# Biblbrox/ViT-Spectre-Experiments

Measured on AMD Instinct MI355X. Metric: images/sec training, Spectre-ViT-S CIFAR-100 bs512, higher is better.
Workload: dtype bf16; 1 GPU; Spectre-ViT-Small (E512 H16 F768 L4 P4 N65, 100 classes, dropout 0.001), fft mixer, train step fwd+CE+bwd+AdamW, bs 512/GPU; mixer=fft, global_batch=512, parallelism=dp1

## Files before the change

include/spv.h:

```cpp
#ifndef SPV_H
#define SPV_H

#include <stddef.h>
#include <stdint.h>

#ifdef __cplusplus
extern "C" {
#endif

#define SPV_F32 0
#define SPV_BF16 1

#define SPV_ABI_VERSION 1

int spv_version(void);
enum {
    SPV_PATH_GEMM_STRIP = 0,
    SPV_PATH_GEMM_STRIP_ACC = 1,
    SPV_PATH_GEMM_TN = 2,
    SPV_PATH_TAIL_LC = 3,
    SPV_PATH_TAIL_UP = 4,
    SPV_PATH_TAIL_LN = 5,
    SPV_PATH_FNET_MFMA = 6,
    SPV_PATH_GATHER_LDS = 7,
// ... 60 lines not shown
    int m, n, lda, ldb, ldc;
    int k;
} spv_tn_problem;
int spv_gemm_tn_batch(const spv_tn_problem* probs, int nprob, int K, int splits, void* workspace, const spv_fold_job* folds, int nfolds,
                      void* stream);
int spv_gemm_tn_batch_part(const spv_tn_problem* probs, int nprob, int K, int splits, void* workspace, const spv_fold_job* folds,
                           int nfolds, int part, void* stream);

int spv_spectre_tail_fwd(const void* h, const void* x, const float* gamma, const float* beta, void* out,
                         float* mean, float* rstd, int rows, int n, int k_in, int dtype, int out_dtype,
                         float p_drop, uint64_t seed, void* stream);

int spv_spectre_tail_bwd(const void* dout, const void* h, const float* mean, const float* rstd,
                         const float* gamma, const float* beta, void* dh, void* dx_pool, float* dgamma,
                         float* dbeta, float* dbias, float* partials, int rows, int n, int k_in, int dtype,
                         int dout_dtype, float p_drop, uint64_t seed, const void* dx_add, void* stream);
int64_t spv_rowop_partial_floats(int n);
int spv_tail_up_supported(int n, int k_in, int dtype);
int spv_spectre_tail_bwd_up(const void* dout, const void* h, const float* mean, const float* rstd, const float* gamma,
                            const float* beta, void* dh, void* dx_pool, float* dgamma, float* dbeta, float* dbias, float* partials,
                            int rows, int n, int k_in, int dtype, int dout_dtype, float p_drop, uint64_t seed, const void* dx_add,
                            const void* up_src, float up_p_drop, uint64_t up_seed, void* stream);
int spv_tail_ln_supported(int n, int k_in, int dtype);
int64_t spv_tail_ln_partial_floats(int n);
int spv_spectre_tail_ln_fwd(const void* h, const void* x, const float* gamma, const float* beta, void* out, float* mean, float* rstd,
                            const void* res, const float* gamma2, const float* beta2, void* out2, float* mean2, float* rstd2, int rows,
                            int n, int k_in, int dtype, float p_drop, uint64_t seed, void* stream);
int spv_spectre_tail_ln_bwd(const void* dout2, const void* f3, const void* res, const float* mean2, const float* rstd2,
                            const float* gamma2, void* ds, float* dgamma2, float* dbeta2, const void* h, const float* mean,
                            const float* rstd, const float* gamma, const float* beta, void* dh, void* dx_pool, float* dgamma,
                            float* dbeta, float* dbias, float* partials, int rows, int n, int k_in, int dtype, float p_drop,
                            uint64_t seed, void* stream);

int spv_haar_ln_supported(int dim, int dtype);
int spv_haar_ln_fwd(const void* x, const float* gamma, const float* beta, void* out, float* mean, float* rstd, int rows, int dim,
                    int dtype, void* stream);
int spv_haar_ln_bwd(const void* dout, const void* x, const float* mean, const float* rstd, const float* gamma, void* dx,
                    float* dgamma, float* dbeta, float* partials, int rows, int dim, int dtype, void* stream);
int spv_add_layernorm_fwd(const void* a, const void* b, const float* gamma, const float* beta, void* out,
                          float* mean, float* rstd, int rows, int n, int mode, int dtype, void* stream);
int spv_add_layernorm_bwd(const void* dout, const void* a, const void* b, const float* mean,
                          const float* rstd, const float* gamma, void* din, float* dgamma, float* dbeta,
                          float* partials, int rows, int n, int mode, int dtype, void* stream);

int64_t spv_permut_table_words(int heads, int d);
int spv_permut_pool_supported(int heads, int d, int pool_window, int dtype);
int spv_permut_pack(const int64_t* perms, const float* signs, uint32_t* idx, int heads, int d, void* stream);
int spv_permut_gather_fwd(const void* x, const uint32_t* idx, void* g, void* pooled, int pool_window, int batch,
                          int heads, int d, int dtype, void* stream);
int spv_permut_gather_bwd(const void* dg, const uint32_t* idx, void* dx, int batch, int heads, int d,
                          int dtype, void* stream);
int spv_permut_row0_fwd(const void* x, const uint32_t* idx, void* g0, void* x0, int batch, int d, int n, int embed, int dtype,
                        void* stream);
int spv_permut_row0_bwd(const void* dg0, const void* dx0, const uint32_t* idx, void* dx, int batch, int d, int n, int embed,
                        int dtype, void* stream);


int spv_fnet_mix(const void* x, void* y, const void* add_in, const float* twiddle, int batch, int tokens, int dim,
                 int dtype, float* workspace, void* stream);
int64_t spv_fnet_workspace_floats(int batch, int tokens, int dim);
int spv_fnet_ln_supported(int tokens, int dim, int dtype);
int spv_fnet_ln_fwd(const void* x, void* prenorm, void* out, const float* gamma, const float* beta, float* mean, float* rstd,
                    const float* twiddle, int batch, int tokens, int dim, int dtype, void* stream);
int spv_fnet_ln_bwd(const void* dout, const void* prenorm, const float* mean, const float* rstd, const float* gamma, void* dx,
                    float* dgamma, float* dbeta, float* partials, const float* twiddle, int batch, int tokens, int dim, int dtype,
                    void* stream);

int spv_fnet_cls_supported(int tokens, int dim, int dtype);
int spv_fnet_cls_fwd(const void* x, const float* gamma, const float* beta, void* out, float* m0, float* mean, float* rstd, int batch,
                     int tokens, int dim, int dtype, void* stream);
int spv_fnet_cls_bwd(const void* g1, const float* m0, const float* mean, const float* rstd, const float* gamma, void* dx,
                     float* partials, int batch, int tokens, int dim, int dtype, void* stream);
int64_t spv_fnet_twiddle_floats(int tokens);
int spv_fnet_make_twiddle(float* twiddle, int tokens, void* stream);

int spv_rfft_real(const void* x, void* y, int rows, int dim, int transpose, int dtype, void* stream);

int spv_haar_dwt(const void* x, void* y, int batch, int tokens, int dim, int axis, int levels, int inverse,
                 int dtype, void* scratch, void* stream);

int spv_set_seed_device_ptr(const void* seed_word);
int spv_seed_advance(void* seed_word, void* stream);

int spv_adamw_multi(const void* table, const int* chunk_tensor, const int* chunk_off, const int* sizes, int nchunks, float lr,
                    float beta1, float beta2, float one_minus_beta1, float one_minus_beta2, float eps, float weight_decay,
                    float bias_correction1, float bias_correction2, const float* step_dev, void* stream);

int spv_adamw_multi_ema(const void* table, const int* chunk_tensor, const int* chunk_off, const int* sizes, int nchunks, float lr,
                        float beta1, float beta2, float one_minus_beta1, float one_minus_beta2, float eps, float weight_decay,
                        float bias_correction1, float bias_correction2, const float* step_dev, float* const* ema_table, float ema_weight,
                        int ema_warmup, float ema_step, void* stream);

typedef struct spv_step_ctl {
    double a, b;
    float clip_coef;
    int apply;
    float grad_norm;
    int sched_step;
    int skipped;
    int reserved[7];
} spv_step_ctl;
#define SPV_CTL_SCHEDULE 1
#define SPV_CTL_CLIP 2
#define SPV_CTL_SKIP_NONFINITE 4

int spv_grad_sumsq(const void* table, const int* chunk_tensor, const int* chunk_off, const int* sizes, int nchunks, double* partials,
                   void* stream);

int spv_step_control(const double* partials, int npartials, float* const* step_ptrs, int nsteps, spv_step_ctl* ctl, int flags,
                     int warmup_steps, int total_steps, double eta_min, float max_norm, void* stream);

int spv_adamw_multi_ctl(const void* table, const int* chunk_tensor, const int* chunk_off, const int* sizes, int nchunks, double base_lr,
                        float beta1, float beta2, float one_minus_beta1, float one_minus_beta2, float eps, float weight_decay,
                        const float* step_dev, const spv_step_ctl* ctl, void* stream);

int spv_adamw_multi_ctl_ema(const void* table, const int* chunk_tensor, const int* chunk_off, const int* sizes, int nchunks, double base_lr,
                            float beta1, float beta2, float one_minus_beta1, float one_minus_beta2, float eps, float weight_decay,
                            const float* step_dev, const spv_step_ctl* ctl, float* const* ema_table, float ema_weight, int ema_warmup,
                            void* stream);

int spv_fwht(const void* x, void* y, const void* residual, int rows, int n_in, int n, int n_out, int mode, int repeat,
             float scale, int dtype, void* stream);

int spv_patchify(const float* img, void* out, int batch, int chans, int height, int width, int patch, int ld,
                 int transposed, int out_dtype, void* stream);
int spv_patchify_u8(const unsigned char* img_hwc, const float* mean, const float* inv_std, void* out, int batch, int chans,
                    int height, int width, int patch, int ld, int transposed, int out_dtype, void* stream);
int spv_embed_posbias(const float* pos, const float* bias, const float* cls, float* out, int patches, int embed, void* stream);
int spv_embed_cls_rows(const float* cls, const float* pos, void* tokens, int batch, int tokens_per_image, int embed,
                       int dtype, void* stream);
int spv_spectral_fold(const float* proj_w, const float* freq_h, const float* freq_w, float* w_full, int embed,
                      int chans, int patch, void* stream);
int spv_spectral_fold_bf16(const float* proj_w, const float* freq_h, const float* freq_w, float* w_full, void* w_full_bf16, int embed,
                           int chans, int patch, void* stream);
int spv_spectral_fold_bwd(const float* dw_full, const float* proj_w, const float* freq_h, const float* freq_w,
                          float* dproj_w, float* dfreq_h, float* dfreq_w, float* scratch, int embed, int chans,
                          int patch, void* stream);
int spv_dropout(const void* x, void* y, int64_t n, float p, uint64_t seed, int dtype, void* stream);
int spv_embed_bwd_groups(int batch);
int spv_embed_bwd(const void* g, const void* gcls, void* dtok, float* partials, float* dpos, float* dbias, float* dcls, int batch,
                  int tokens, int embed, float p_drop, uint64_t seed, int dtype, void* stream);

int spv_attention_fwd(const void* qkv, void* ctx, void* probs, int seqs, int len, int heads, int head_dim, int dtype,
                      float p_drop, uint64_t seed, void* stream);
int spv_attention_bwd(const void* dctx, const void* qkv, const void* probs, void* dscores, void* dqkv, int seqs, int len,
                      int heads, int head_dim, int dtype, float p_drop, uint64_t seed, void* stream);
int spv_attention_row0_fwd(const void* q0, const void* k, const void* v, int ldkv, void* ctx0, float* probs, int batch, int len,
                           int heads, int head_dim, int dtype, float p_drop, uint64_t seed, void* stream);
int spv_attention_row0_bwd(const void* dctx0, const void* q0, const void* k, const void* v, int ldkv, const float* probs, void* dq0,
                           void* dk, void* dv, int ldd, int batch, int len, int heads, int head_dim, int dtype, float p_drop,
                           uint64_t seed, void* stream);

int spv_gelu_fwd(const void* x, void* y, int64_t n, int dtype, void* stream);
int spv_gelu_bwd(const void* dy, const void* x, void* dx, int64_t n, int dtype, void* stream);
int spv_colsum(const void* x, float* out, float* partials, int rows, int n, int dtype, void* stream);
int spv_axpby(const void* x, const void* y, void* out, float a, float b, int64_t n, int dtype, void* stream);

int spv_small_sl_supported(int rows, int n, int k);
int64_t spv_small_sl_partial_floats(int rows, int n);
int spv_small_sl_fwd(const void* xa, int64_t lda, const void* xb, int64_t ldb, const float* W, const float* bias,
                     const float* gamma, const float* beta, float* out, float* h, float* xs, float* mean, float* rstd,
                     int rows, int n, int k, int dtype, void* stream);
int spv_small_sl_bwd(const float* dout, const float* h, const float* xs, const float* mean, const float* rstd,
                     const float* W, const float* gamma, const float* beta, float* dh, void* dx, float* dW,
                     float* dgamma, float* dbeta, float* dbias, float* partials, int rows, int n, int k, int dx_dtype,
                     void* stream);
int64_t spv_cross_entropy_workspace_floats(void);
int spv_cross_entropy_fwd(const float* logits, const int64_t* labels, float* lse, float* loss, float* workspace, int rows,
                          int classes, void* stream);
int spv_cross_entropy_bwd(const float* logits, const int64_t* labels, const float* lse, const float* grad_out,
                          float* dlogits, int rows, int classes, void* stream);

int spv_spectrum_floats(int H, int W);
int spv_spectrum_log1p(const float* img, void* out, int B, int C, int H, int W, int dtype, void* stream);
int spv_conv3x3_fwd(const void* x, const void* w, const float* bias, void* y, void* cols, int B, int H, int W, int Cin, int Cout,
                    int dtype, void* stream);
int spv_conv3x3_dgrad(const void* dy, const void* wd, void* dx, void* cols, int B, int H, int W, int Cin, int Cout, int dtype,
                      void* stream);
int spv_conv3x3_wgrad(const void* dy, const void* x, float* dw, void* dyt, void* colst, float* workspace, int splits, int B, int H,
                      int W, int Cin, int Cout, int dtype, void* stream);
int spv_token_pool_fwd(const void* y, void* out, int B, int L, int C, int T, int ldo, int dtype, void* stream);
int spv_token_pool_bwd(const void* dout, int ldo, const void* add, void* dy, int B, int L, int C, int T, int dtype, void* stream);

#define SPV_AUG_NPARAM 16
#define SPV_AUG_FLIP 0
#define SPV_AUG_BRIGHT 1
#define SPV_AUG_CONTRAST 2
#define SPV_AUG_SAT 3
#define SPV_AUG_HUE 4
#define SPV_AUG_ORDER 5
#define SPV_AUG_GRAY 6
#define SPV_AUG_ANGLE 7
#define SPV_AUG_BLUR 8
#define SPV_AUG_SIGMA 9
#define SPV_AUG_ERASE_I 10
#define SPV_AUG_ERASE_J 11
#define SPV_AUG_ERASE_H 12
#define SPV_AUG_ERASE_W 13
typedef struct spv_augment_cfg {
    float flip_p;
    float bright_lo, bright_hi, contrast_lo, contrast_hi, sat_lo, sat_hi, hue_lo, hue_hi;
    float gray_p;
    float degrees;
    float blur_p, sigma_lo, sigma_hi;
    float erase_p, scale_lo, scale_hi, ratio_lo, ratio_hi;
} spv_augment_cfg;
int spv_augment_params(float* params, int batch, int chans, int height, int width, const spv_augment_cfg* cfg, uint64_t seed,
                       uint64_t step, void* stream);
int spv_augment_supported(int chans, int height, int width);
int spv_augment_u8(const unsigned char* src_nhwc, const int64_t* index, const float* params, const float* mean, const float* inv_std,
                   float* out_nchw, int batch, int n_src, int chans, int height, int width, void* stream);
int spv_augment_plan(int chans, int height, int width);
size_t spv_augment_tiled_ws_bytes(int batch, int height, int width);
int spv_augment_tiled_u8(const unsigned char* src_nhwc, const int64_t* index, const float* params, const float* mean,
                         const float* inv_std, float* out_nchw, int batch, int n_src, int chans, int height, int width, void* workspace,
                         size_t workspace_bytes, void* stream);

int spv_teacher_view_supported(int chans, int n, int resize, int crop);
int spv_teacher_view_u8(const unsigned char* src_nhwc, const int64_t* index, const int* table, const float* lut, void* out_nchw, int batch,
                        int n_src, int chans, int n, int resize, int crop, int dtype, void* stream);
int64_t spv_distill_loss_workspace_floats(void);
int spv_distill_loss_fwd(const float* student, const float* teacher, const int64_t* labels, float* lse3, float* out3, float* workspace,
                         int rows, int classes, float T, float w_soft, float w_ce, void* stream);
int spv_distill_loss_bwd(const float* student, const float* teacher, const int64_t* labels, const float* lse3, const float* grad_out,
                         float* dlogits, int rows, int classes, float T, float w_soft, float w_ce, void* stream);
int spv_logit_cache_store(float* cache, const int64_t* index, const float* logits, int rows, int n_cache, int classes, void* stream);
int spv_distill_loss_idx_fwd(const float* student, const float* cache, const int64_t* index, const int64_t* labels, float* lse3, float* out3,
                             float* workspace, int rows, int n_cache, int classes, float T, float w_soft, float w_ce, void* stream);
int spv_distill_loss_idx_bwd(const float* student, const float* cache, const int64_t* index, const int64_t* labels, const float* lse3,
                             const float* grad_out, float* dlogits, int rows, int n_cache, int classes, float T, float w_soft, float w_ce,
                             void* stream);

int64_t spv_eval_head_stats_words(void);
int spv_eval_head(const void* logits, const int64_t* labels, const int* n_valid, int64_t* pred, void* stats, int rows, int classes, int k,
                  int dtype, void* stream);

#define SPV_TRAIN_METER_HEADER 16
#define SPV_TRAIN_METER_ROW 5
#define SPV_TRAIN_METER_MAX_CAPACITY (1 << 24)
int64_t spv_train_meter_words(int64_t capacity);
int64_t spv_cross_entropy_meter_workspace_floats(void);
int spv_cross_entropy_meter_fwd(const float* logits, const int64_t* labels, float* lse, float* loss, float* workspace, int rows,
                                int classes, void* meter, int k, void* stream);
int64_t spv_distill_loss_meter_workspace_floats(void);
int spv_distill_loss_meter_fwd(const float* student, const float* teacher, const int64_t* labels, float* lse3, float* out3, float* workspace,
                               int rows, int classes, float T, float w_soft, float w_ce, void* meter, int k, void* stream);
int spv_distill_loss_idx_meter_fwd(const float* student, const float* cache, const int64_t* index, const int64_t* labels, float* lse3,
                                   float* out3, float* workspace, int rows, int n_cache, int classes, float T, float w_soft, float w_ce,
                                   void* meter, int k, void* stream);
// ... 6 lines not shown
```

vit-spectre-experiments_amd/csrc/spv_head.hip:

```cpp
#include "spv_common.h"

namespace {

constexpr int HR = 4;
constexpr int HT = 1024;
constexpr int HW = HT / 64;
constexpr int MAXN = 128;
constexpr int MAXK = 1024;

template <typename T> __device__ __forceinline__ float ldx(const void* p, size_t i) { return io<T>::ld(static_cast<const T*>(p) + i); }

__device__ __forceinline__ int win_start(int i, int n, int k) { return (int)(((int64_t)i * k) / n); }
__device__ __forceinline__ int win_end(int i, int n, int k) { return (int)((((int64_t)(i + 1)) * k + n - 1) / n); }

template <typename T, int KJ>
__global__ __launch_bounds__(HT) void small_sl_fwd_kernel(const void* __restrict__ xa, int64_t lda, const void* __restrict__ xb, int64_t ldb,
                                                          const float* __restrict__ W, const float* __restrict__ bias,
                                                          const float* __restrict__ gamma, const float* __restrict__ beta,
                                                          float* __restrict__ out, float* __restrict__ h, float* __restrict__ xs_out,
                                                          float* __restrict__ mean, float* __restrict__ rstd, int rows, int n, int k) {
    __shared__ float xs[HR][MAXK];
    __shared__ float hs[HR][MAXN];
    const int tid = threadIdx.x, lane = tid & 63, wave = tid >> 6;
    const int r0 = blockIdx.x * HR;
// ... 124 lines not shown
            }
        }
        const float m1 = wave_sum(s1) / (float)n, m2 = wave_sum(s2) / (float)n;
#pragma unroll
        for (int j = 0; j < 2; ++j) {
            const int o = lane + 64 * j;
            if (o < n) {
                const float v = live ? rs * (t[j] - m1 - xh[j] * m2) : 0.0f;
                dhs[wave][o] = v;
                if (!live) dos[wave][o] = 0.0f;
                part[wave][0][o] = dl[j] * xh[j];
                part[wave][1][o] = dl[j];
                part[wave][2][o] = v;
                if (live) dh[(size_t)row * n + o] = v;
            }
        }
    }
    __syncthreads();
    for (int e = tid; e < 3 * n; e += HT) {
        const int w = e / n, o = e - w * n;
        float a = 0.0f;
#pragma unroll
        for (int r = 0; r < HR; ++r) a += part[r][w][o];
        partials[((size_t)blockIdx.x * 3 + w) * n + o] = a;
    }
    const int cols = min(k, HT);
    const int nq = HT / cols;
    const int c = tid % cols, qs = tid / cols;
    constexpr int LB = 32;
    float a[HR];
#pragma unroll
    for (int r = 0; r < HR; ++r) a[r] = 0.0f;
    if (qs < nq) {
        for (int o0 = qs; o0 < n; o0 += LB * nq) {
            float w[LB];
#pragma unroll
            for (int j = 0; j < LB; ++j) {
                w[j] = W[(size_t)min(o0 + j * nq, n - 1) * k + c];
            }
#pragma unroll
            for (int j = 0; j < LB; ++j) {
                const int o = o0 + j * nq;
                const float wv = o < n ? w[j] : 0.0f;
                const int oc = min(o, n - 1);
#pragma unroll
                for (int r = 0; r < HR; ++r) a[r] = fmaf(dhs[r][oc], wv, a[r]);
            }
        }
    }
    float* join = reinterpret_cast<float*>(joinbuf);
    if (qs < nq) {
#pragma unroll
        for (int r = 0; r < HR; ++r) join[((size_t)qs * HR + r) * cols + c] = a[r];
    }
    __syncthreads();
    if (tid < cols) {
        float o4[HR];
#pragma unroll
        for (int r = 0; r < HR; ++r) {
            float t = 0.0f;
            for (int q2 = 0; q2 < nq; ++q2) t += join[((size_t)q2 * HR + r) * cols + c];
            o4[r] = t;
        }
        if (n == k) {
#pragma unroll
            for (int r = 0; r < HR; ++r) o4[r] += dos[r][c];
        } else {
            const int i0 = (int)(((int64_t)c * n) / k);
            for (int i = max(i0 - 1, 0); i <= min(i0 + 1, n - 1); ++i) {
                const int s0 = win_start(i, n, k), e0 = win_end(i, n, k);
                if (c >= s0 && c < e0) {
                    const float inv = 1.0f / (float)(e0 - s0);
#pragma unroll
                    for (int r = 0; r < HR; ++r) o4[r] = fmaf(dos[r][i], inv, o4[r]);
                }
            }
        }
#pragma unroll
        for (int r = 0; r < HR; ++r)
            if (r0 + r < rows) io<T>::st(static_cast<T*>(dx) + (size_t)(r0 + r) * k + c, o4[r]);
    }
}

constexpr int WT = 1024, WCOLS = 128, WGRP = WT / WCOLS, WOUT = 2;
__global__ __launch_bounds__(WT) void small_sl_bwd_w_kernel(const float* __restrict__ dh, const float* __restrict__ xs,
                                                            const float* __restrict__ partials, float* __restrict__ dW,
                                                            float* __restrict__ dgamma, float* __restrict__ dbeta, float* __restrict__ dbias,
                                                            int rows, int n, int k, int nparts, int cblocks) {
    __shared__ float red[WGRP][WOUT][WCOLS];
    const int tid = threadIdx.x;
    const int njobs = ((n + WOUT - 1) / WOUT) * cblocks;
    if ((int)blockIdx.x == njobs) {
        constexpr int SL = 16;
        float* fold = &red[0][0][0];
        for (int e0 = 0; e0 < 3 * n; e0 += 64) {
            const int e = e0 + (tid & 63), q = tid >> 6;
            float a = 0.0f;
            if (e < 3 * n) {
                const int w = e / n, c = e - w * n;
                for (int p0 = q; p0 < nparts; p0 += SL * 8) {
                    float v[8];
#pragma unroll
                    for (int j = 0; j < 8; ++j) {
                        const int pp = p0 + j * SL;
                        v[j] = partials[((size_t)min(pp, nparts - 1) * 3 + w) * n + c] * (pp < nparts ? 1.0f : 0.0f);
                    }
#pragma unroll
                    for (int j = 0; j < 8; ++j) a += v[j];
                }
            }
            fold[q * 64 + (tid & 63)] = a;
            __syncthreads();
            if (tid < 64 && e < 3 * n) {
                float t = 0.0f;
#pragma unroll
                for (int j = 0; j < SL; ++j) t += fold[j * 64 + tid];
                const int w = e / n, c = e - w * n;
                (w == 0 ? dgamma : (w == 1 ? dbeta : dbias))[c] = t;
            }
            __syncthreads();
        }
        return;
    }
    const int o0 = ((int)blockIdx.x / cblocks) * WOUT, c = ((int)blockIdx.x % cblocks) * WCOLS + (tid & (WCOLS - 1));
    const int g = __builtin_amdgcn_readfirstlane(tid / WCOLS);
    const int o1 = min(o0 + 1, n - 1);
    const int cc = min(c, k - 1);
    float a0 = 0.0f, a1 = 0.0f;
    constexpr int RB = 32;
    for (int rb = g; rb < rows; rb += WGRP * RB) {
        float x[RB], d0[RB], d1[RB];
#pragma unroll
        for (int j = 0; j < RB; ++j) {
            const int r = rb + j * WGRP;
            const int rr = min(r, rows - 1);
            x[j] = xs[(size_t)rr * k + cc] * (r < rows ? 1.0f : 0.0f);
            d0[j] = dh[(size_t)rr * n + o0];
            d1[j] = dh[(size_t)rr * n + o1];
        }
#pragma unroll
        for (int j = 0; j < RB; ++j) {
            a0 = fmaf(d0[j], x[j], a0);
            a1 = fmaf(d1[j], x[j], a1);
        }
    }
    red[g][0][tid & (WCOLS - 1)] = a0;
    red[g][1][tid & (WCOLS - 1)] = a1;
    __syncthreads();
    if (tid < WOUT * WCOLS) {
        const int w = tid / WCOLS, cl = tid & (WCOLS - 1);
        const int o = o0 + w, col = ((int)blockIdx.x % cblocks) * WCOLS + cl;
        float t = 0.0f;
#pragma unroll
        for (int j = 0; j < WGRP; ++j) t += red[j][w][cl];
        if (o < n && col < k) dW[(size_t)o * k + col] = t;
    }
}

constexpr int CE_MAX_WG = 64;
constexpr int CE_HITS = CE_MAX_WG + 2;

template <bool METER>
__device__ __forceinline__ void ce_fwd_body(const float* __restrict__ z, const int64_t* __restrict__ labels, float* __restrict__ lse,
                                            float* __restrict__ loss, float* __restrict__ partial, unsigned* __restrict__ counter,
                                            int rows, int C, long long* meter, int k) {
    __shared__ float ws[HT / 64];
    __shared__ int hs[METER ? HT / 64 : 1][3];
    __shared__ bool last;
    const int tid = threadIdx.x, lane = tid & 63, wave = tid >> 6;
    float acc = 0.0f;
    int seen = 0, top1 = 0, topk = 0;
    for (int r = blockIdx.x * (HT / 64) + wave; r < rows; r += gridDim.x * (HT / 64)) {
        const float* zr = z + (size_t)r * C;
        float m = -INFINITY;
        int first = 0, above = 0;
        float s = 0.0f;
        if constexpr (METER) {
            const int64_t ym = labels[r];
            const float zy = zr[(ym >= 0 && ym < C) ? (int)ym : 0];
            float bm = -INFINITY;
            int am = C;
            for (int c = lane; c < C; c += 64) {
                const float x = zr[c];
                m = fmaxf(m, x);
                if (x > bm) { bm = x; am = c; }
            }
            m = wave_max(m);
            first = (int)(-wave_max(-(float)((bm == m && am < C) ? am : C)));
            if (first >= C) first = 0;
            float cnt = 0.0f;
            for (int c = lane; c < C; c += 64) {
                const float x = zr[c];
                s += __expf(x - m);
                cnt += (x > zy || (x == zy && c < ym)) ? 1.0f : 0.0f;
            }
            above = (int)wave_sum(cnt);
        } else {
            for (int c = lane; c < C; c += 64) m = fmaxf(m, zr[c]);
            m = wave_max(m);
            for (int c = lane; c < C; c += 64) s += __expf(zr[c] - m);
        }
        const float l = m + __logf(wave_sum(s));
        const int64_t y = labels[r];
        const bool ok = y >= 0 && y < C;
        if (lane == 0) {
            lse[r] = l;
            acc += ok ? l - zr[y] : __builtin_nanf("");
            if constexpr (METER) {
                if (ok) {
                    seen += 1;
                    top1 += first == (int)y ? 1 : 0;
                    topk += above < k ? 1 : 0;
// ... 25 lines not shown
            hits[0] = a0;
            hits[1] = a1;
            hits[2] = a2;
        }
        __threadfence();
        last = atomicAdd(counter, 1u) == gridDim.x - 1;
    }
    __syncthreads();
    if (last) {
        __threadfence();
        if (wave == 0) {
            const bool in = lane < (int)gridDim.x;
            const float t = wave_sum(in ? __builtin_nontemporal_load(partial + lane) : 0.0f);
            float h0 = 0.0f, h1 = 0.0f, h2 = 0.0f;
            if constexpr (METER) {
                const int* hits = reinterpret_cast<const int*>(partial + CE_HITS) + 3 * lane;
                h0 = wave_sum(in ? (float)__builtin_nontemporal_load(hits) : 0.0f);
                h1 = wave_sum(in ? (float)__builtin_nontemporal_load(hits + 1) : 0.0f);
                h2 = wave_sum(in ? (float)__builtin_nontemporal_load(hits + 2) : 0.0f);
            }
            if (lane == 0) {
                const float mean = t / (float)rows;
                *loss = mean;
                if constexpr (METER) train_meter_log(meter, mean, 0.0f, 0.0f, (int)h0, (int)h1, (int)h2);
                *counter = 0u;
            }
        }
    }
}

__global__ __launch_bounds__(HT) void ce_fwd_kernel(const float* __restrict__ z, const int64_t* __restrict__ labels, float* __restrict__ lse,
                                                    float* __restrict__ loss, float* __restrict__ partial, unsigned* __restrict__ counter,
                                                    int rows, int C) {
    ce_fwd_body<false>(z, labels, lse, loss, partial, counter, rows, C, nullptr, 0);
}

__global__ __launch_bounds__(HT) void ce_meter_fwd_kernel(const float* __restrict__ z, const int64_t* __restrict__ labels,
                                                          float* __restrict__ lse, float* __restrict__ loss, float* __restrict__ partial,
                                                          unsigned* __restrict__ counter, int rows, int C, long long* meter, int k) {
    ce_fwd_body<true>(z, labels, lse, loss, partial, counter, rows, C, meter, k);
}

__global__ __launch_bounds__(HT) void ce_bwd_kernel(const float* __restrict__ z, const int64_t* __restrict__ labels, const float* __restrict__ lse,
                                                    const float* __restrict__ go, float* __restrict__ dz, int rows, int C) {
    const float scale = go[0] / (float)rows;
    const int64_t total = (int64_t)rows * C;
    for (int64_t e = (int64_t)blockIdx.x * HT + threadIdx.x; e < total; e += (int64_t)gridDim.x * HT) {
        const int r = (int)(e / C), c = (int)(e - (int64_t)r * C);
        const float p = __expf(z[e] - lse[r]);
        dz[e] = (p - (labels[r] == c ? 1.0f : 0.0f)) * scale;
    }
}

}

extern "C" int spv_small_sl_supported(int rows, int n, int k) {
    return (rows > 0 && rows <= 4096 && n > 0 && n <= MAXN && k > 0 && k <= MAXK && n <= k) ? 1 : 0;
}
extern "C" int64_t spv_small_sl_partial_floats(int rows, int n) { return (int64_t)cdiv(rows, HR) * 3 * n; }

extern "C" int spv_small_sl_fwd(const void* xa, int64_t lda, const void* xb, int64_t ldb, const float* W, const float* bias, const float* gamma,
                                const float* beta, float* out, float* h, float* xs, float* mean, float* rstd, int rows, int n, int k,
                                int dtype, void* stream) {
    SPV_CHECK(spv_small_sl_supported(rows, n, k), "spv_small_sl_fwd: rows=%d n=%d k=%d outside the small-rows kernel", rows, n, k);
    SPV_CHECK(dtype == SPV_F32 || dtype == SPV_BF16, "spv_small_sl_fwd: bad dtype %d", dtype);
    SPV_CHECK(lda >= k && (xb == nullptr || ldb >= k), "spv_small_sl_fwd: row strides below k");
    hipStream_t st = static_cast<hipStream_t>(stream);
    const dim3 grid(cdiv(rows, HR));
#define SPV_HEAD_FWD(TY, KJV) hipLaunchKernelGGL((small_sl_fwd_kernel<TY, KJV>), grid, dim3(HT), 0, st, xa, lda, xb, ldb, W, bias, gamma, beta, out, h, xs, mean, rstd, rows, n, k)
    if (dtype == SPV_BF16) {
        if (k <= 512) SPV_HEAD_FWD(bf16_t, 8);
        else if (k <= 768) SPV_HEAD_FWD(bf16_t, 12);
        else SPV_HEAD_FWD(bf16_t, 16);
    } else {
        if (k <= 512) SPV_HEAD_FWD(float, 8);
        else if (k <= 768) SPV_HEAD_FWD(float, 12);
        else SPV_HEAD_FWD(float, 16);
    }
#undef SPV_HEAD_FWD
    SPV_LAUNCH_CHECK("spv_small_sl_fwd");
    return 0;
}

extern "C" int spv_small_sl_bwd(const float* dout, const float* h, const float* xs, const float* mean, const float* rstd, const float* W,
                                const float* gamma, const float* beta, float* dh, void* dx, float* dW, float* dgamma, float* dbeta,
                                float* dbias, float* partials, int rows, int n, int k, int dx_dtype, void* stream) {
    SPV_CHECK(spv_small_sl_supported(rows, n, k), "spv_small_sl_bwd: rows=%d n=%d k=%d outside the small-rows kernel", rows, n, k);
    SPV_CHECK(dx_dtype == SPV_F32 || dx_dtype == SPV_BF16, "spv_small_sl_bwd: bad dtype %d", dx_dtype);
    hipStream_t st = static_cast<hipStream_t>(stream);
    const int nparts = cdiv(rows, HR);
    if (dx_dtype == SPV_BF16)
        hipLaunchKernelGGL((small_sl_bwd_rows_kernel<bf16_t>), dim3(nparts), dim3(HT), 0, st, dout, h, mean, rstd, gamma, beta, W, dh, dx, partials, rows, n, k);
    else
        hipLaunchKernelGGL((small_sl_bwd_rows_kernel<float>), dim3(nparts), dim3(HT), 0, st, dout, h, mean, rstd, gamma, beta, W, dh, dx, partials, rows, n, k);
    SPV_LAUNCH_CHECK("spv_small_sl_bwd(rows)");
    const int cblocks = cdiv(k, WCOLS);
    hipLaunchKernelGGL(small_sl_bwd_w_kernel, dim3(cdiv(n, WOUT) * cblocks + 1), dim3(WT), 0, st, dh, xs, partials, dW, dgamma, dbeta, dbias, rows,
                       n, k, nparts, cblocks);
    SPV_LAUNCH_CHECK("spv_small_sl_bwd(weights)");
    return 0;
}

extern "C" int64_t spv_cross_entropy_workspace_floats() { return CE_MAX_WG + 1; }

extern "C" int spv_cross_entropy_fwd(const float* logits, const int64_t* labels, float* lse, float* loss, float* workspace, int rows, int classes,
                                     void* stream) {
    SPV_CHECK(rows > 0 && classes > 0, "spv_cross_entropy_fwd: empty");
    hipStream_t st = static_cast<hipStream_t>(stream);
    const int wgs = std::min(cdiv(rows, HT / 64), CE_MAX_WG);
    hipLaunchKernelGGL(ce_fwd_kernel, dim3(wgs), dim3(HT), 0, st, logits, labels, lse, loss, workspace, reinterpret_cast<unsigned*>(workspace + CE_MAX_WG),
                       rows, classes);
    SPV_LAUNCH_CHECK("spv_cross_entropy_fwd");
    return 0;
}

extern "C" int64_t spv_train_meter_words(int64_t capacity) {
    if (capacity < 1 || capacity > SPV_TRAIN_METER_MAX_CAPACITY) {
        spv_set_error("spv_train_meter_words: capacity=%lld outside 1..%lld", (long long)capacity, (long long)SPV_TRAIN_METER_MAX_CAPACITY);
        return 0;
    }
    return TM_HEADER + capacity * TM_ROW;
}

int spv_train_meter_check(const char* name, const void* meter, int k, int rows, int classes) {
    SPV_CHECK(meter != nullptr, "%s: meter missing", name);
    SPV_CHECK(((uintptr_t)meter & 7) == 0, "%s: the meter block must be 8-byte aligned", name);
    SPV_CHECK(k >= 1 && k <= 8, "%s: k=%d outside 1..8", name, k);
    SPV_CHECK(rows > 0 && rows <= (1 << 24) && classes > 0 && classes < (1 << 24), "%s: rows=%d classes=%d outside 1..2^24 rows, 1..2^24-1 classes",
              name, rows, classes);
    return 0;
}

extern "C" int64_t spv_cross_entropy_meter_workspace_floats() { return CE_HITS + 3 * CE_MAX_WG; }

extern "C" int spv_cross_entropy_meter_fwd(const float* logits, const int64_t* labels, float* lse, float* loss, float* workspace, int rows,
                                           int classes, void* meter, int k, void* stream) {
    if (int rc = spv_train_meter_check("spv_cross_entropy_meter_fwd", meter, k, rows, classes)) return rc;
    SPV_CHECK(logits != nullptr && labels != nullptr && lse != nullptr && loss != nullptr && workspace != nullptr,
              "spv_cross_entropy_meter_fwd: null pointer");
    hipStream_t st = static_cast<hipStream_t>(stream);
    const int wgs = std::min(cdiv(rows, HT / 64), CE_MAX_WG);
    hipLaunchKernelGGL(ce_meter_fwd_kernel, dim3(wgs), dim3(HT), 0, st, logits, labels, lse, loss, workspace,
                       reinterpret_cast<unsigned*>(workspace + CE_MAX_WG), rows, classes, static_cast<long long*>(meter), k);
    SPV_LAUNCH_CHECK("spv_cross_entropy_meter_fwd");
    return 0;
}

extern "C" int spv_cross_entropy_bwd(const float* logits, const int64_t* labels, const float* lse, const float* grad_out, float* dlogits, int rows,
                                     int classes, void* stream) {
    SPV_CHECK(rows > 0 && classes > 0, "spv_cross_entropy_bwd: empty");
    hipStream_t st = static_cast<hipStream_t>(stream);
    const int64_t total = (int64_t)rows * classes;
    hipLaunchKernelGGL(ce_bwd_kernel, dim3((unsigned)std::min<int64_t>((total + HT - 1) / HT, 1024)), dim3(HT), 0, st, logits, labels, lse, grad_out,
                       dlogits, rows, classes);
    SPV_LAUNCH_CHECK("spv_cross_entropy_bwd");
    return 0;
}
```

vit-spectre-experiments_amd/csrc/spv_misc.hip:

```cpp
#include "spv_common.h"
#include "spv_adamw_core.h"

#include <string.h>

static thread_local char g_err[512] = "";

int spv_set_error(const char* fmt, ...) {
    va_list ap;
    va_start(ap, fmt);
    vsnprintf(g_err, sizeof(g_err), fmt, ap);
    va_end(ap);
    return 1;
}

long long g_spv_path_counts[SPV_PATH_COUNT] = {0};
extern "C" long long spv_path_count(int which) {
    return (which >= 0 && which < SPV_PATH_COUNT) ? g_spv_path_counts[which] : -1;
}

extern "C" int spv_version(void) { return SPV_ABI_VERSION; }
extern "C" const char* spv_last_error(void) { return g_err; }

namespace {

template <typename TI, typename TO>
__global__ __launch_bounds__(256) void cast_kernel(const TI* __restrict__ src, TO* __restrict__ dst, int64_t n) {
    const int64_t n4 = n >> 2;
    for (int64_t i = (int64_t)blockIdx.x * blockDim.x + threadIdx.x; i < n4; i += (int64_t)gridDim.x * blockDim.x) {
        float v[4];
        io<TI>::ld4(src + 4 * i, v);
        io<TO>::st4(dst + 4 * i, v);
    }
    if (blockIdx.x == 0 && threadIdx.x < (n & 3)) {
        int64_t i = (n4 << 2) + threadIdx.x;
        io<TO>::st(dst + i, io<TI>::ld(src + i));
    }
}

template <typename TI, typename TO>
__global__ __launch_bounds__(256) void cast_transpose_kernel(const TI* __restrict__ src, TO* __restrict__ dst, int rows,
                                                             int cols, int ld, int rg, int gs, int roff) {
    __shared__ float tile[64][65];
    const int r0 = blockIdx.y * 64, c0 = blockIdx.x * 64;
    const int tx = threadIdx.x & 63, ty = threadIdx.x >> 6;
    for (int i = ty; i < 64; i += 4) {
        int r = r0 + i, c = c0 + tx;
        float v = 0.0f;
        if (r < rows && c < cols) {
            const size_t sr = rg > 0 ? (size_t)(r / rg) * gs + roff + (r % rg) : (size_t)r;
            v = io<TI>::ld(src + sr * cols + c);
        }
        tile[i][tx] = v;
    }
    __syncthreads();
    for (int i = ty; i < 64; i += 4) {
        int c = c0 + i, r = r0 + tx;
        if (c < cols && r < ld) io<TO>::st(dst + (size_t)c * ld + r, tile[tx][i]);
    }
}

template <typename TO>
__device__ __forceinline__ void weight_shadow_tile(const float* __restrict__ src, TO* __restrict__ plain, TO* __restrict__ tr, int rows,
                                                   int cols, int ld, int bx, int by, float (*tile)[65]) {
    const int r0 = by * 32, c0 = bx * 64;
    const int t = threadIdx.x;
    const bool vec = (cols & 3) == 0;
#pragma unroll
    for (int pass = 0; pass < 2; ++pass) {
        const int rl = pass * 16 + (t >> 4), c4 = (t & 15) * 4;
        const int r = r0 + rl, c = c0 + c4;
        float v[4] = {0.0f, 0.0f, 0.0f, 0.0f};
        if (r < rows) {
            if (vec && c + 3 < cols) {
                const float4 f = *reinterpret_cast<const float4*>(src + (size_t)r * cols + c);
                v[0] = f.x; v[1] = f.y; v[2] = f.z; v[3] = f.w;
                if (plain != nullptr) io<TO>::st4(plain + (size_t)r * cols + c, v);
            } else {
                for (int u = 0; u < 4; ++u)
                    if (c + u < cols) {
                        v[u] = src[(size_t)r * cols + c + u];
                        if (plain != nullptr) io<TO>::st(plain + (size_t)r * cols + c + u, v[u]);
                    }
            }
        }
#pragma unroll
        for (int u = 0; u < 4; ++u) tile[rl][c4 + u] = v[u];
    }
    __syncthreads();
    const int cl = t >> 2, r8 = (t & 3) * 8;
    const int c = c0 + cl;
    if (c < cols) {
        TO* o = tr + (size_t)c * ld + r0 + r8;
        if (r0 + r8 + 7 < ld && (ld & 7) == 0) {
            float a[4], b[4];
#pragma unroll
            for (int u = 0; u < 4; ++u) { a[u] = tile[r8 + u][cl]; b[u] = tile[r8 + 4 + u][cl]; }
            io<TO>::st4(o, a);
            io<TO>::st4(o + 4, b);
        } else {
            for (int u = 0; u < 8; ++u)
                if (r0 + r8 + u < ld) io<TO>::st(o + u, tile[r8 + u][cl]);
        }
    }
}

template <typename TO>
__global__ __launch_bounds__(256) void weight_shadow_kernel(const float* __restrict__ src, TO* __restrict__ plain, TO* __restrict__ tr,
                                                            int rows, int cols, int ld) {
    __shared__ float tile[32][65];
    weight_shadow_tile<TO>(src, plain, tr, rows, cols, ld, blockIdx.x, blockIdx.y, tile);
}

struct ShadowTensor { const float* src; void* plain; void* tr; int rows, cols, ld, pad; };
template <typename TO>
__global__ __launch_bounds__(256) void weight_shadow_multi_kernel(const ShadowTensor* __restrict__ tab, const int* __restrict__ tile_tensor,
                                                                  const int* __restrict__ tile_x, const int* __restrict__ tile_y) {
    __shared__ float tile[32][65];
    const ShadowTensor t = tab[tile_tensor[blockIdx.x]];
    weight_shadow_tile<TO>(t.src, static_cast<TO*>(t.plain), static_cast<TO*>(t.tr), t.rows, t.cols, t.ld, tile_x[blockIdx.x],
                           tile_y[blockIdx.x], tile);
}

template <typename T>
__global__ __launch_bounds__(256) void gelu_fwd_kernel(const T* __restrict__ x, T* __restrict__ y, int64_t n) {
    for (int64_t i = (int64_t)blockIdx.x * blockDim.x + threadIdx.x; i < n; i += (int64_t)gridDim.x * blockDim.x)
        io<T>::st(y + i, gelu_erf(io<T>::ld(x + i)));
}
template <typename T>
__global__ __launch_bounds__(256) void gelu_bwd_kernel(const T* __restrict__ dy, const T* __restrict__ x,
                                                       T* __restrict__ dx, int64_t n) {
    for (int64_t i = (int64_t)blockIdx.x * blockDim.x + threadIdx.x; i < n; i += (int64_t)gridDim.x * blockDim.x)
        io<T>::st(dx + i, io<T>::ld(dy + i) * gelu_erf_grad(io<T>::ld(x + i)));
}
template <typename T>
__global__ __launch_bounds__(256) void axpby_kernel(const T* __restrict__ x, const T* __restrict__ y, T* __restrict__ out,
                                                    float a, float b, int64_t n) {
    for (int64_t i = (int64_t)blockIdx.x * blockDim.x + threadIdx.x; i < n; i += (int64_t)gridDim.x * blockDim.x)
        io<T>::st(out + i, a * io<T>::ld(x + i) + b * io<T>::ld(y + i));
}

template <typename T, int VEC>
__global__ __launch_bounds__(256) void colsum_partial_kernel(const T* __restrict__ x, float* __restrict__ partials, int rows,
                                                             int n, int tx_log2) {
    __shared__ float red[256 * VEC];
    const int TX = 1 << tx_log2, TY = 256 >> tx_log2;
    const int tx = threadIdx.x & (TX - 1), ty = threadIdx.x >> tx_log2;
    const int c0 = (blockIdx.x * TX + tx) * VEC;
    float s[VEC];
#pragma unroll
    for (int k = 0; k < VEC; ++k) s[k] = 0.0f;
    if (c0 < n) {
        const int step = gridDim.y * TY;
        for (int r = blockIdx.y * TY + ty; r < rows; r += step) {
            if constexpr (VEC == 4) {
                float v[4];
                io<T>::ld4(x + (size_t)r * n + c0, v);
#pragma unroll
                for (int k = 0; k < 4; ++k) s[k] += v[k];
            } else {
                s[0] += io<T>::ld(x + (size_t)r * n + c0);
            }
        }
    }
#pragma unroll
    for (int k = 0; k < VEC; ++k) red[(ty * TX + tx) * VEC + k] = s[k];
    __syncthreads();
    if (ty == 0 && c0 < n) {
#pragma unroll
        for (int k = 0; k < VEC; ++k) {
            float t = s[k];
            for (int q = 1; q < TY; ++q) t += red[(q * TX + tx) * VEC + k];
            if (c0 + k < n) partials[(size_t)blockIdx.y * n + c0 + k] = t;
        }
    }
}
__global__ __launch_bounds__(256) void colsum_fold_kernel(const float* __restrict__ partials, float* __restrict__ out, int parts,
                                                          int n) {
    __shared__ float red[8][33];
    const int cx = threadIdx.x & 31, py = threadIdx.x >> 5;
    const int c = blockIdx.x * 32 + cx;
    float s = 0.0f;
    if (c < n)
        for (int p = py; p < parts; p += 8) s += partials[(size_t)p * n + c];
    red[py][cx] = s;
    __syncthreads();
    if (py == 0 && c < n) {
        float t = 0.0f;
#pragma unroll
        for (int q = 0; q < 8; ++q) t += red[q][cx];
        out[c] = t;
    }
}

inline int ew_blocks(int64_t n) { return (int)std::min<int64_t>((n + 255) / 256, 2048); }

}
// ... 68 lines not shown
    else
        return spv_set_error("spv_weight_shadows: bad dtype %d", dtype);
    SPV_LAUNCH_CHECK("spv_weight_shadows");
    return 0;
}

#define DISPATCH_T(dtype, name, ...)                                        \
    if (dtype == SPV_F32) { using T = float; __VA_ARGS__; }                 \
    else if (dtype == SPV_BF16) { using T = bf16_t; __VA_ARGS__; }          \
    else return spv_set_error("%s: bad dtype %d", name, dtype);

extern "C" int spv_gelu_fwd(const void* x, void* y, int64_t n, int dtype, void* stream) {
    if (n <= 0) return 0;
    hipStream_t st = static_cast<hipStream_t>(stream);
    DISPATCH_T(dtype, "spv_gelu_fwd",
               hipLaunchKernelGGL((gelu_fwd_kernel<T>), dim3(ew_blocks(n)), dim3(256), 0, st, (const T*)x, (T*)y, n));
    SPV_LAUNCH_CHECK("spv_gelu_fwd");
    return 0;
}
extern "C" int spv_gelu_bwd(const void* dy, const void* x, void* dx, int64_t n, int dtype, void* stream) {
    if (n <= 0) return 0;
    hipStream_t st = static_cast<hipStream_t>(stream);
    DISPATCH_T(dtype, "spv_gelu_bwd",
               hipLaunchKernelGGL((gelu_bwd_kernel<T>), dim3(ew_blocks(n)), dim3(256), 0, st, (const T*)dy, (const T*)x, (T*)dx, n));
    SPV_LAUNCH_CHECK("spv_gelu_bwd");
    return 0;
}
extern "C" int spv_axpby(const void* x, const void* y, void* out, float a, float b, int64_t n, int dtype, void* stream) {
    if (n <= 0) return 0;
    hipStream_t st = static_cast<hipStream_t>(stream);
    DISPATCH_T(dtype, "spv_axpby",
               hipLaunchKernelGGL((axpby_kernel<T>), dim3(ew_blocks(n)), dim3(256), 0, st, (const T*)x, (const T*)y, (T*)out, a, b, n));
    SPV_LAUNCH_CHECK("spv_axpby");
    return 0;
}

extern "C" int spv_colsum(const void* x, float* out, float* partials, int rows, int n, int dtype, void* stream) {
    SPV_CHECK(rows > 0 && n > 0, "spv_colsum: empty");
    hipStream_t st = static_cast<hipStream_t>(stream);
    const int vec = (n % 4 == 0 && ((uintptr_t)x & 15) == 0) ? 4 : 1;
    const int cthreads = cdiv(n, vec);
    int tx_log2 = 5;
    while (tx_log2 < 8 && (1 << tx_log2) < cthreads) ++tx_log2;
    const int ty = 256 >> tx_log2;
    const int gx = cdiv(cthreads, 1 << tx_log2);
    const int parts = std::max(1, std::min(std::min(cdiv(rows, ty), 512), std::max(1, 1024 / gx)));
    if (vec == 4) {
        DISPATCH_T(dtype, "spv_colsum",
                   hipLaunchKernelGGL((colsum_partial_kernel<T, 4>), dim3(gx, parts), dim3(256), 0, st, (const T*)x, partials, rows, n, tx_log2));
    } else {
        DISPATCH_T(dtype, "spv_colsum",
                   hipLaunchKernelGGL((colsum_partial_kernel<T, 1>), dim3(gx, parts), dim3(256), 0, st, (const T*)x, partials, rows, n, tx_log2));
    }
    SPV_LAUNCH_CHECK("spv_colsum");
    hipLaunchKernelGGL(colsum_fold_kernel, dim3(cdiv(n, 32)), dim3(256), 0, st, partials, out, parts, n);
    SPV_LAUNCH_CHECK("spv_colsum(fold)");
    return 0;
}

namespace {
__global__ __launch_bounds__(256) void adamw_multi_kernel(const AdamTensor* __restrict__ tab, const int* __restrict__ chunk_tensor,
                                                          const int* __restrict__ chunk_off, const int* __restrict__ sizes, float lr,
                                                          float beta1, float beta2, float omb1, float omb2, float eps, float wd,
                                                          float bc1, float bc2, const float* __restrict__ step_dev) {
    const int t = chunk_tensor[blockIdx.x];
    const int off = chunk_off[blockIdx.x];
    const AdamTensor a = tab[t];
    const int n = sizes[t];
    adamw_chunk<false>(a, n, off, lr, beta1, beta2, omb1, omb2, eps, wd, bc1, bc2, step_dev, 1.0f);
}

__global__ __launch_bounds__(256) void adamw_multi_ema_kernel(const AdamTensor* __restrict__ tab, const int* __restrict__ chunk_tensor,
                                                              const int* __restrict__ chunk_off, const int* __restrict__ sizes, float lr,
                                                              float beta1, float beta2, float omb1, float omb2, float eps, float wd,
                                                              float bc1, float bc2, const float* __restrict__ step_dev,
                                                              float* const* __restrict__ ema_tab, float ema_w, int ema_warmup, float ema_step) {
    const int t = chunk_tensor[blockIdx.x];
    const int off = chunk_off[blockIdx.x];
    const AdamTensor a = tab[t];
    const int n = sizes[t];
    adamw_chunk<false, true>(a, n, off, lr, beta1, beta2, omb1, omb2, eps, wd, bc1, bc2, step_dev, 1.0f, ema_tab[t], ema_w, ema_warmup,
                             ema_step);
}
}

extern "C" int spv_adamw_multi(const void* table, const int* chunk_tensor, const int* chunk_off, const int* sizes, int nchunks, float lr,
                               float beta1, float beta2, float one_minus_beta1, float one_minus_beta2, float eps, float weight_decay,
                               float bias_correction1, float bias_correction2, const float* step_dev, void* stream) {
    SPV_CHECK(nchunks >= 0, "spv_adamw_multi: nchunks = %d", nchunks);
    if (nchunks == 0) return 0;
    SPV_CHECK(table && chunk_tensor && chunk_off && sizes, "spv_adamw_multi: null table");
    SPV_CHECK(step_dev != nullptr || (bias_correction1 > 0.0f && bias_correction2 > 0.0f), "spv_adamw_multi: bias corrections must be > 0");
    hipLaunchKernelGGL(adamw_multi_kernel, dim3(nchunks), dim3(256), 0, static_cast<hipStream_t>(stream),
                       static_cast<const AdamTensor*>(table), chunk_tensor, chunk_off, sizes, lr, beta1, beta2, one_minus_beta1,
                       one_minus_beta2, eps, weight_decay, bias_correction1, bias_correction2, step_dev);
    SPV_LAUNCH_CHECK("spv_adamw_multi");
    return 0;
}

extern "C" int spv_adamw_multi_ema(const void* table, const int* chunk_tensor, const int* chunk_off, const int* sizes, int nchunks, float lr,
                                   float beta1, float beta2, float one_minus_beta1, float one_minus_beta2, float eps, float weight_decay,
                                   float bias_correction1, float bias_correction2, const float* step_dev, float* const* ema_table,
                                   float ema_weight, int ema_warmup, float ema_step, void* stream) {
    SPV_CHECK(nchunks >= 0, "spv_adamw_multi_ema: nchunks = %d", nchunks);
    SPV_CHECK(table && chunk_tensor && chunk_off && sizes, "spv_adamw_multi_ema: null table");
    SPV_CHECK(ema_table, "spv_adamw_multi_ema: null ema_table (use spv_adamw_multi for a group that is not averaged)");
    SPV_CHECK(step_dev != nullptr || (bias_correction1 > 0.0f && bias_correction2 > 0.0f), "spv_adamw_multi_ema: bias corrections must be > 0");
    SPV_CHECK(ema_weight > 0.0f && ema_weight <= 1.0f, "spv_adamw_multi_ema: ema_weight = %g must be in (0, 1]", (double)ema_weight);
    SPV_CHECK(!ema_warmup || step_dev != nullptr || ema_step >= 1.0f, "spv_adamw_multi_ema: ema_step = %g must be >= 1 (the step count of this step)",
              (double)ema_step);
    if (nchunks == 0) return 0;
    hipLaunchKernelGGL(adamw_multi_ema_kernel, dim3(nchunks), dim3(256), 0, static_cast<hipStream_t>(stream),
                       static_cast<const AdamTensor*>(table), chunk_tensor, chunk_off, sizes, lr, beta1, beta2, one_minus_beta1,
                       one_minus_beta2, eps, weight_decay, bias_correction1, bias_correction2, step_dev, ema_table, ema_weight, ema_warmup,
                       ema_step);
    SPV_LAUNCH_CHECK("spv_adamw_multi_ema");
    return 0;
}

int spv_seed_ptr_set_rowops(const unsigned long long* p);
int spv_seed_ptr_set_patch(const unsigned long long* p);
int spv_seed_ptr_set_attn(const unsigned long long* p);
int spv_seed_ptr_set_gemm(const unsigned long long* p);
namespace {
__global__ void seed_advance_kernel(unsigned long long* p) { *p += 0x9e3779b97f4a7c15ull; }
}
extern "C" int spv_set_seed_device_ptr(const void* seed_word) {
    const unsigned long long* p = static_cast<const unsigned long long*>(seed_word);
    SPV_CHECK(spv_seed_ptr_set_rowops(p) == 0 && spv_seed_ptr_set_patch(p) == 0 && spv_seed_ptr_set_attn(p) == 0 && spv_seed_ptr_set_gemm(p) == 0,
              "spv_set_seed_device_ptr: hipMemcpyToSymbol failed");
    return 0;
}
extern "C" int spv_seed_advance(void* seed_word, void* stream) {
    SPV_CHECK(seed_word != nullptr, "spv_seed_advance: null pointer");
    hipLaunchKernelGGL(seed_advance_kernel, dim3(1), dim3(1), 0, static_cast<hipStream_t>(stream), static_cast<unsigned long long*>(seed_word));
    SPV_LAUNCH_CHECK("spv_seed_advance");
    return 0;
}
```

vit-spectre-experiments_amd/csrc/spv_patch.hip:

```cpp
#define SPV_USES_SEED
#include "spv_common.h"

namespace {

__device__ __forceinline__ void st_any(void* base, size_t off, int bf, float v) {
    if (bf) static_cast<bf16_t*>(base)[off] = f2bf(v);
    else static_cast<float*>(base)[off] = v;
}
__device__ __forceinline__ float ld_any(const void* base, size_t off, int bf) {
    return bf ? bf2f(static_cast<const bf16_t*>(base)[off]) : static_cast<const float*>(base)[off];
}

__global__ __launch_bounds__(256) void patchify_kernel(const float* __restrict__ img, void* __restrict__ out, int B, int C, int H,
                                                       int W, int P, int ld, int transposed, int bf) {
    const int nH = H / P, nW = W / P, Np = nH * nW, K = C * P * P;
    const int64_t rows = (int64_t)B * Np;
    const int64_t total = transposed == 1 ? (int64_t)K * ld : (transposed == 2 ? (int64_t)B * (Np + 1) * ld : rows * ld);
    for (int64_t e = (int64_t)blockIdx.x * blockDim.x + threadIdx.x; e < total; e += (int64_t)gridDim.x * blockDim.x) {
        int64_t row;
        int k;
        if (transposed == 1) { k = (int)(e / ld); row = e % ld; }
        else { row = e / ld; k = (int)(e % ld); }
        if (transposed == 2) {
            const int64_t b2 = row / (Np + 1);
            const int t2 = (int)(row % (Np + 1));
            row = t2 == 0 ? rows : b2 * Np + t2 - 1;
        }
        float v = 0.0f;
        if (row < rows && k < K) {
            const int b = (int)(row / Np), n = (int)(row % Np);
            const int ih = n / nW, iw = n % nW;
            const int c = k / (P * P), p = (k / P) % P, q = k % P;
            v = img[(((size_t)b * C + c) * H + ih * P + p) * W + iw * P + q];
        }
        st_any(out, (size_t)e, bf, v);
    }
}

template <typename T>
__global__ __launch_bounds__(256) void patchify_vec4_kernel(const float* __restrict__ img, T* __restrict__ out, int B, int C, int H, int W,
                                                            int P, int ld, int token_rows) {
    const int nH = H / P, nW = W / P, Np = nH * nW, K = C * P * P;
    const int T1 = token_rows ? Np + 1 : Np;
    const int ld4 = ld >> 2, P4 = P >> 2;
    const int64_t total = (int64_t)B * T1 * ld4;
    for (int64_t e = (int64_t)blockIdx.x * blockDim.x + threadIdx.x; e < total; e += (int64_t)gridDim.x * blockDim.x) {
        const int64_t row = e / ld4;
        const int k = (int)(e - row * ld4) * 4;
        const int b = (int)(row / T1), t = (int)(row - (int64_t)b * T1);
        const int n = token_rows ? t - 1 : t;
        float v[4] = {0.0f, 0.0f, 0.0f, 0.0f};
        if (n >= 0 && k < K) {
            const int ih = n / nW, iw = n - ih * nW;
            const int c = k / (P * P), r = k - c * P * P, pr = r / P, q = r - pr * P;
            const float4 px = *reinterpret_cast<const float4*>(img + (((size_t)b * C + c) * H + ih * P + pr) * W + iw * P + q);
            v[0] = px.x; v[1] = px.y; v[2] = px.z; v[3] = px.w;
        }
        (void)P4;
        io<T>::st4(out + (size_t)row * ld + k, v);
    }
}

__global__ __launch_bounds__(256) void patchify_u8_kernel(const unsigned char* __restrict__ img, const float* __restrict__ mean,
                                                          const float* __restrict__ inv_std, void* __restrict__ out, int B, int C,
                                                          int H, int W, int P, int ld, int transposed, int bf) {
    const int nH = H / P, nW = W / P, Np = nH * nW, K = C * P * P;
    const int64_t rows = (int64_t)B * Np;
    const int64_t total = transposed == 1 ? (int64_t)K * ld : (transposed == 2 ? (int64_t)B * (Np + 1) * ld : rows * ld);
    for (int64_t e = (int64_t)blockIdx.x * blockDim.x + threadIdx.x; e < total; e += (int64_t)gridDim.x * blockDim.x) {
        int64_t row;
        int k;
        if (transposed == 1) { k = (int)(e / ld); row = e % ld; }
        else { row = e / ld; k = (int)(e % ld); }
        if (transposed == 2) {
            const int64_t b2 = row / (Np + 1);
            const int t2 = (int)(row % (Np + 1));
            row = t2 == 0 ? rows : b2 * Np + t2 - 1;
        }
        float v = 0.0f;
        if (row < rows && k < K) {
            const int b = (int)(row / Np), n = (int)(row % Np);
            const int ih = n / nW, iw = n % nW;
            const int c = k / (P * P), p = (k / P) % P, q = k % P;
            const float px = (float)img[(((size_t)b * H + ih * P + p) * W + iw * P + q) * C + c];
            v = (px * (1.0f / 255.0f) - mean[c]) * inv_std[c];
        }
        st_any(out, (size_t)e, bf, v);
    }
}

__global__ __launch_bounds__(256) void posbias_kernel(const float* __restrict__ pos, const float* __restrict__ bias,
                                                      const float* __restrict__ cls, float* __restrict__ out, int Np, int E) {
    const int lead = cls != nullptr ? E : 0;
    const int total = Np * E + lead;
    for (int i = blockIdx.x * blockDim.x + threadIdx.x; i < total; i += gridDim.x * blockDim.x)
        out[i] = i < lead ? cls[i] + pos[i] : pos[E + i - lead] + bias[(i - lead) % E];
}

__global__ __launch_bounds__(256) void cls_rows_kernel(const float* __restrict__ cls, const float* __restrict__ pos,
                                                       void* __restrict__ tokens, int B, int T, int E, int bf) {
    const int total = B * E;
    for (int i = blockIdx.x * blockDim.x + threadIdx.x; i < total; i += gridDim.x * blockDim.x) {
        const int b = i / E, e = i % E;
        st_any(tokens, ((size_t)b * T) * E + e, bf, cls[e] + pos[e]);
    }
}

__global__ __launch_bounds__(256) void dropout_kernel(const void* __restrict__ x, void* __restrict__ y, int64_t n, float p,
                                                      uint64_t seed, int bf) {
    const float inv_keep = 1.0f / (1.0f - p);
    const int64_t n8 = n >> 3;
    for (int64_t v = (int64_t)blockIdx.x * blockDim.x + threadIdx.x; v < n8; v += (int64_t)gridDim.x * blockDim.x) {
        const int64_t i = v << 3;
        const unsigned key = dropout_row_key(live_seed(seed), (uint64_t)i >> 12);
        const unsigned c0 = (unsigned)(i & 4095);
        float sc[8];
#pragma unroll
        for (int u = 0; u < 8; ++u) sc[u] = dropout_scale(key, c0 + u, p, inv_keep);
        if (bf) {
            const uint4 t = *reinterpret_cast<const uint4*>(static_cast<const bf16_t*>(x) + i);
            const unsigned w[4] = {t.x, t.y, t.z, t.w};
            unsigned o[4];
#pragma unroll
            for (int u = 0; u < 4; ++u)
                o[u] = pack_bf16x2(__uint_as_float(w[u] << 16) * sc[2 * u], __uint_as_float(w[u] & 0xffff0000u) * sc[2 * u + 1]);
            *reinterpret_cast<uint4*>(static_cast<bf16_t*>(y) + i) = make_uint4(o[0], o[1], o[2], o[3]);
        } else {
            const float4 a = *reinterpret_cast<const float4*>(static_cast<const float*>(x) + i);
            const float4 b = *reinterpret_cast<const float4*>(static_cast<const float*>(x) + i + 4);
            *reinterpret_cast<float4*>(static_cast<float*>(y) + i) = make_float4(a.x * sc[0], a.y * sc[1], a.z * sc[2], a.w * sc[3]);
            *reinterpret_cast<float4*>(static_cast<float*>(y) + i + 4) = make_float4(b.x * sc[4], b.y * sc[5], b.z * sc[6], b.w * sc[7]);
        }
    }
    for (int64_t i = (n8 << 3) + (int64_t)blockIdx.x * blockDim.x + threadIdx.x; i < n; i += (int64_t)gridDim.x * blockDim.x)
        st_any(y, (size_t)i, bf, ld_any(x, (size_t)i, bf) *
                                     dropout_scale(dropout_row_key(live_seed(seed), (uint64_t)i >> 12), (unsigned)(i & 4095), p, inv_keep));
}

__device__ __forceinline__ float rcoef(int u, int v, int p, int q, int P) {
    return cospif(2.0f * (float)((u * p + v * q) % P) / (float)P) / (float)P;
}

__global__ __launch_bounds__(256) void spectral_fold_kernel(const float* __restrict__ w, const float* __restrict__ fh,
                                                            const float* __restrict__ fw, float* __restrict__ wf, int E, int C, int P,
                                                            bf16_t* __restrict__ wf_bf = nullptr) {
    const int Pv = P / 2 + 1;
    const int total = E * C * P * P;
    for (int i = blockIdx.x * blockDim.x + threadIdx.x; i < total; i += gridDim.x * blockDim.x) {
        const int q = i % P, p = (i / P) % P, c = (i / (P * P)) % C, e = i / (P * P * C);
        const float* wr = w + ((size_t)e * C + c) * P * Pv;
        float a = 0.0f;
        for (int u = 0; u < P; ++u)
            for (int v = 0; v < Pv; ++v) a = fmaf(wr[u * Pv + v] * fh[u] * fw[v], rcoef(u, v, p, q, P), a);
        wf[i] = a;
        if (wf_bf != nullptr) wf_bf[i] = f2bf(a);
    }
}

__global__ __launch_bounds__(256) void spectral_fold_bwd_kernel(const float* __restrict__ dwf, const float* __restrict__ w,
                                                                const float* __restrict__ fh, const float* __restrict__ fw,
                                                                float* __restrict__ dw, float* __restrict__ gw, int E, int C, int P) {
    const int Pv = P / 2 + 1;
    const int total = E * C * P * Pv;
    for (int i = blockIdx.x * blockDim.x + threadIdx.x; i < total; i += gridDim.x * blockDim.x) {
        const int v = i % Pv, u = (i / Pv) % P, ec = i / (Pv * P);
        const float* dr = dwf + (size_t)ec * P * P;
        float g = 0.0f;
        for (int p = 0; p < P; ++p)
            for (int q = 0; q < P; ++q) g = fmaf(dr[p * P + q], rcoef(u, v, p, q, P), g);
        dw[i] = g * fh[u] * fw[v];
        gw[i] = g * w[i];
    }
}
__global__ __launch_bounds__(1024) void freq_weight_grad_kernel(const float* __restrict__ gw, const float* __restrict__ fh,
                                                                const float* __restrict__ fw, float* __restrict__ dfh,
                                                                float* __restrict__ dfw, int EC, int P) {
    extern __shared__ float lds[];
    const int Pv = P / 2 + 1, S = P + Pv;
    const int nt = blockDim.x;
    float* mine = lds + threadIdx.x * S;
    for (int j = 0; j < S; ++j) mine[j] = 0.0f;
    for (int ec = threadIdx.x; ec < EC; ec += nt) {
        const float* g = gw + (size_t)ec * P * Pv;
        for (int u = 0; u < P; ++u)
            for (int v = 0; v < Pv; ++v) {
                const float t = g[u * Pv + v];
                mine[u] += t * fw[v];
                mine[P + v] += t * fh[u];
            }
    }
    for (int stride = nt >> 1; stride >= 1; stride >>= 1) {
        __syncthreads();
        if ((int)threadIdx.x < stride) {
            const float* other = lds + (threadIdx.x + stride) * S;
            for (int j = 0; j < S; ++j) mine[j] += other[j];
        }
    }
    if (threadIdx.x == 0) {
        for (int j = 0; j < P; ++j) dfh[j] = mine[j];
        for (int j = 0; j < Pv; ++j) dfw[j] = mine[P + j];
    }
}

inline int ew_blocks(int64_t n) { return (int)std::min<int64_t>((n + 255) / 256, 4096); }

}

extern "C" int spv_patchify(const float* img, void* out, int batch, int chans, int height, int width, int patch, int ld,
                            int transposed, int out_dtype, void* stream) {
    SPV_CHECK(batch > 0 && chans > 0 && patch > 0 && height >= patch && width >= patch, "spv_patchify: bad shape");
    SPV_CHECK(out_dtype == SPV_F32 || out_dtype == SPV_BF16, "spv_patchify: bad dtype");
    const int Np = (height / patch) * (width / patch), K = chans * patch * patch;
    const int64_t rows = (int64_t)batch * Np;
    SPV_CHECK(transposed >= 0 && transposed <= 2 && (transposed == 1 ? ld >= rows : ld >= K), "spv_patchify: ld=%d too small", ld);
    const int64_t total = transposed == 1 ? (int64_t)K * ld : (transposed == 2 ? (int64_t)batch * (Np + 1) * ld : rows * ld);
    if (transposed != 1 && patch % 4 == 0 && width % 4 == 0 && ld % 4 == 0 && ((uintptr_t)img & 15) == 0 && ((uintptr_t)out & 15) == 0) {
        const int64_t vecs = (int64_t)batch * (Np + (transposed == 2 ? 1 : 0)) * (ld / 4);
        if (out_dtype == SPV_BF16)
            hipLaunchKernelGGL((patchify_vec4_kernel<bf16_t>), dim3(ew_blocks(vecs)), dim3(256), 0, static_cast<hipStream_t>(stream), img, (bf16_t*)out,
                               batch, chans, height, width, patch, ld, transposed == 2);
        else
            hipLaunchKernelGGL((patchify_vec4_kernel<float>), dim3(ew_blocks(vecs)), dim3(256), 0, static_cast<hipStream_t>(stream), img, (float*)out,
                               batch, chans, height, width, patch, ld, transposed == 2);
        SPV_LAUNCH_CHECK("spv_patchify(vec4)");
        return 0;
    }
    hipLaunchKernelGGL(patchify_kernel, dim3(ew_blocks(total)), dim3(256), 0, static_cast<hipStream_t>(stream), img, out, batch,
                       chans, height, width, patch, ld, transposed, out_dtype == SPV_BF16);
    SPV_LAUNCH_CHECK("spv_patchify");
    return 0;
}

extern "C" int spv_patchify_u8(const unsigned char* img_hwc, const float* mean, const float* inv_std, void* out, int batch,
                               int chans, int height, int width, int patch, int ld, int transposed, int out_dtype, void* stream) {
    SPV_CHECK(batch > 0 && chans > 0 && patch > 0 && height >= patch && width >= patch, "spv_patchify_u8: bad shape");
    SPV_CHECK(out_dtype == SPV_F32 || out_dtype == SPV_BF16, "spv_patchify_u8: bad dtype");
    SPV_CHECK(mean != nullptr && inv_std != nullptr, "spv_patchify_u8: mean / inv_std missing");
    const int Np = (height / patch) * (width / patch), K = chans * patch * patch;
    const int64_t rows = (int64_t)batch * Np;
    SPV_CHECK(transposed >= 0 && transposed <= 2 && (transposed == 1 ? ld >= rows : ld >= K), "spv_patchify_u8: ld=%d too small", ld);
    const int64_t total = transposed == 1 ? (int64_t)K * ld : (transposed == 2 ? (int64_t)batch * (Np + 1) * ld : rows * ld);
    hipLaunchKernelGGL(patchify_u8_kernel, dim3(ew_blocks(total)), dim3(256), 0, static_cast<hipStream_t>(stream), img_hwc, mean,
                       inv_std, out, batch, chans, height, width, patch, ld, transposed, out_dtype == SPV_BF16);
    SPV_LAUNCH_CHECK("spv_patchify_u8");
    return 0;
}

extern "C" int spv_embed_posbias(const float* pos, const float* bias, const float* cls, float* out, int patches, int embed, void* stream) {
    SPV_CHECK(patches > 0 && embed > 0, "spv_embed_posbias: empty");
    hipLaunchKernelGGL(posbias_kernel, dim3(ew_blocks((int64_t)(patches + 1) * embed)), dim3(256), 0, static_cast<hipStream_t>(stream), pos,
                       bias, cls, out, patches, embed);
    SPV_LAUNCH_CHECK("spv_embed_posbias");
    return 0;
}

extern "C" int spv_embed_cls_rows(const float* cls, const float* pos, void* tokens, int batch, int tokens_per_image, int embed,
                                  int dtype, void* stream) {
    SPV_CHECK(batch > 0 && tokens_per_image > 0 && embed > 0, "spv_embed_cls_rows: empty");
    SPV_CHECK(dtype == SPV_F32 || dtype == SPV_BF16, "spv_embed_cls_rows: bad dtype");
    hipLaunchKernelGGL(cls_rows_kernel, dim3(ew_blocks((int64_t)batch * embed)), dim3(256), 0, static_cast<hipStream_t>(stream), cls,
                       pos, tokens, batch, tokens_per_image, embed, dtype == SPV_BF16);
    SPV_LAUNCH_CHECK("spv_embed_cls_rows");
    return 0;
}

constexpr int EB_GS = 16, EB_HB = 8;
template <typename T>
__global__ __launch_bounds__(256) void embed_bwd_rows_kernel(const T* __restrict__ g, const T* __restrict__ gcls, T* __restrict__ dtok,
                                                            float* __restrict__ partials, int B, int TE, int E, float p, uint64_t seed) {
    const int v = blockIdx.x * 256 + threadIdx.x;
    if (v * 8 >= TE) return;
    const int col = v * 8;
    const int b0 = blockIdx.y * EB_GS;
    const float inv_keep = 1.0f / (1.0f - p);
    const uint64_t sd = live_seed(seed);
    float acc[8];
#pragma unroll
    for (int u = 0; u < 8; ++u) acc[u] = 0.0f;
    const bool cls_row = gcls != nullptr && col < E;
    if constexpr (sizeof(T) == 2) {
        typedef unsigned raw4 __attribute__((ext_vector_type(4)));
        for (int h0 = 0; h0 < EB_GS; h0 += EB_HB) {
            raw4 xr[EB_HB], cr[EB_HB];
#pragma unroll
            for (int s = 0; s < EB_HB; ++s) xr[s] = *reinterpret_cast<const raw4*>(g + (size_t)min(b0 + h0 + s, B - 1) * TE + col);
            if (cls_row) {
#pragma unroll
// ... 190 lines not shown
```

vit-spectre-experiments_amd/spectre_vit/_native.py:

```python
import ctypes
import os

import torch

_HERE = os.path.dirname(os.path.abspath(__file__))
LIB_PATH = os.environ.get("SPV_LIB_PATH") or os.path.join(os.path.dirname(_HERE), "lib", "libspv_hip.so")

c_vp, c_i, c_i64, c_u64, c_f, c_d = ctypes.c_void_p, ctypes.c_int, ctypes.c_int64, ctypes.c_uint64, ctypes.c_float, ctypes.c_double

PATH = dict(gemm_strip=0, gemm_strip_acc=1, gemm_tn=2, tail_lc=3, tail_up=4, tail_ln=5, fnet_mfma=6, gather_lds=7, distill_cached=8, gemm_tn_wide=9,
            gemm_tn_batch=10, gemm_strip_pool=11, permut_row0=12, gemm_rows=13,
            spectrum=14, conv_fwd=15, conv_dgrad=16, conv_wgrad=17, token_pool=18, token_unpool=19, attn_row0_fwd=20, attn_row0_bwd=21, augment=22, teacher_view=23,
            attn_v1=24, attn_v2=25, attn_v3=26)

SIGNATURES = {
    "spv_version": [],
    "spv_last_error": [],
    "spv_path_count": [c_i],
    "spv_cast": [c_vp, c_i, c_vp, c_i, c_i64, c_vp],
    "spv_cast_transpose": [c_vp, c_i, c_vp, c_i, c_i, c_i, c_i, c_i, c_i, c_i, c_vp],
    "spv_weight_shadows": [c_vp, c_vp, c_vp, c_i, c_i, c_i, c_i, c_vp],
    "spv_weight_shadows_multi": [c_vp, c_vp, c_vp, c_vp, c_i, c_i, c_vp],
    "spv_gemm_nt": [c_vp, c_vp, c_vp, c_vp, c_i, c_i, c_i, c_i, c_i, c_i, c_i, c_i, c_i, c_i, c_vp, c_vp],
    "spv_gemm_nt_grouped_rows": [c_vp, c_vp, c_vp, c_vp, c_vp, c_i, c_i, c_i, c_i, c_i, c_i, c_i, c_i, c_i, c_i, c_i, c_vp],
    "spv_gemm_nt_grouped_rows_drop": [c_vp, c_vp, c_vp, c_vp, c_vp, c_i, c_i, c_i, c_i, c_i, c_i, c_i, c_i, c_i, c_i, c_i, c_f, c_u64, c_vp],
    "spv_set_reserved_cus": [c_i],
    "spv_gemm_tn": [c_vp, c_vp, c_vp, c_i, c_i, c_i, c_i, c_i, c_i, c_i, c_i, c_i, c_vp, c_vp],
    "spv_spectre_tail_fwd": [c_vp, c_vp, c_vp, c_vp, c_vp, c_vp, c_vp, c_i, c_i, c_i, c_i, c_i, c_f, c_u64, c_vp],
    "spv_spectre_tail_bwd": [c_vp, c_vp, c_vp, c_vp, c_vp, c_vp, c_vp, c_vp, c_vp, c_vp, c_vp, c_vp, c_i, c_i, c_i, c_i,
                             c_i, c_f, c_u64, c_vp, c_vp],
    "spv_rowop_partial_floats": [c_i],
    "spv_tail_up_supported": [c_i, c_i, c_i],
    "spv_spectre_tail_bwd_up": [c_vp] * 12 + [c_i, c_i, c_i, c_i, c_i, c_f, c_u64, c_vp, c_vp, c_f, c_u64, c_vp],
    "spv_tail_ln_supported": [c_i, c_i, c_i],
    "spv_tail_ln_partial_floats": [c_i],
    "spv_spectre_tail_ln_fwd": [c_vp] * 13 + [c_i, c_i, c_i, c_i, c_f, c_u64, c_vp],
    "spv_spectre_tail_ln_bwd": [c_vp] * 20 + [c_i, c_i, c_i, c_i, c_f, c_u64, c_vp],
    "spv_add_layernorm_fwd": [c_vp, c_vp, c_vp, c_vp, c_vp, c_vp, c_vp, c_i, c_i, c_i, c_i, c_vp],
    "spv_add_layernorm_bwd": [c_vp, c_vp, c_vp, c_vp, c_vp, c_vp, c_vp, c_vp, c_vp, c_vp, c_i, c_i, c_i, c_i, c_vp],
    "spv_permut_pack": [c_vp, c_vp, c_vp, c_i, c_i, c_vp],
    "spv_permut_row0_fwd": [c_vp, c_vp, c_vp, c_vp, c_i, c_i, c_i, c_i, c_i, c_vp],
    "spv_permut_row0_bwd": [c_vp, c_vp, c_vp, c_vp, c_i, c_i, c_i, c_i, c_i, c_vp],
    "spv_permut_table_words": [c_i, c_i],
    "spv_permut_pool_supported": [c_i, c_i, c_i, c_i],
    "spv_tail_bwd_parts": [c_i],
    "spv_haar_ln_supported": [c_i, c_i],
    "spv_haar_ln_fwd": [c_vp, c_vp, c_vp, c_vp, c_vp, c_vp, c_i, c_i, c_i, c_vp],
    "spv_haar_ln_bwd": [c_vp, c_vp, c_vp, c_vp, c_vp, c_vp, c_vp, c_vp, c_vp, c_i, c_i, c_i, c_vp],
    "spv_embed_bwd_groups": [c_i],
    "spv_embed_bwd": [c_vp, c_vp, c_vp, c_vp, c_vp, c_vp, c_vp, c_i, c_i, c_i, c_f, c_u64, c_i, c_vp],
    "spv_fold_multi": [c_vp, c_i, c_vp],
    "spv_gemm_tn_fold": [c_vp, c_vp, c_vp, c_i, c_i, c_i, c_i, c_i, c_i, c_i, c_i, c_i, c_vp, c_vp, c_i, c_vp],
    "spv_gemm_tn_batch": [c_vp, c_i, c_i, c_i, c_vp, c_vp, c_i, c_vp],
    "spv_gemm_tn_batch_part": [c_vp, c_i, c_i, c_i, c_vp, c_vp, c_i, c_i, c_vp],
    "spv_small_sl_supported": [c_i, c_i, c_i],
    "spv_small_sl_partial_floats": [c_i, c_i],
    "spv_small_sl_fwd": [c_vp, c_i64, c_vp, c_i64, c_vp, c_vp, c_vp, c_vp, c_vp, c_vp, c_vp, c_vp, c_vp, c_i, c_i, c_i, c_i, c_vp],
    "spv_small_sl_bwd": [c_vp] * 15 + [c_i, c_i, c_i, c_i, c_vp],
    "spv_cross_entropy_workspace_floats": [],
    "spv_cross_entropy_fwd": [c_vp, c_vp, c_vp, c_vp, c_vp, c_i, c_i, c_vp],
    "spv_cross_entropy_bwd": [c_vp, c_vp, c_vp, c_vp, c_vp, c_i, c_i, c_vp],
    "spv_permut_gather_fwd": [c_vp, c_vp, c_vp, c_vp, c_i, c_i, c_i, c_i, c_i, c_vp],
    "spv_gemm_nt_pool_bwd": [c_vp, c_vp, c_vp, c_vp, c_i, c_i, c_i, c_i, c_i, c_i, c_i, c_i, c_i, c_i, c_vp],
    "spv_permut_gather_bwd": [c_vp, c_vp, c_vp, c_i, c_i, c_i, c_i, c_vp],
    "spv_fnet_mix": [c_vp, c_vp, c_vp, c_vp, c_i, c_i, c_i, c_i, c_vp, c_vp],
    "spv_fnet_workspace_floats": [c_i, c_i, c_i],
    "spv_fnet_twiddle_floats": [c_i],
    "spv_fnet_make_twiddle": [c_vp, c_i, c_vp],
    "spv_fnet_ln_supported": [c_i, c_i, c_i],
    "spv_fnet_cls_supported": [c_i, c_i, c_i],
    "spv_fnet_cls_fwd": [c_vp, c_vp, c_vp, c_vp, c_vp, c_vp, c_vp, c_i, c_i, c_i, c_i, c_vp],
    "spv_fnet_cls_bwd": [c_vp, c_vp, c_vp, c_vp, c_vp, c_vp, c_vp, c_i, c_i, c_i, c_i, c_vp],
    "spv_fnet_ln_fwd": [c_vp, c_vp, c_vp, c_vp, c_vp, c_vp, c_vp, c_vp, c_i, c_i, c_i, c_i, c_vp],
    "spv_fnet_ln_bwd": [c_vp, c_vp, c_vp, c_vp, c_vp, c_vp, c_vp, c_vp, c_vp, c_vp, c_i, c_i, c_i, c_i, c_vp],
    "spv_rfft_real": [c_vp, c_vp, c_i, c_i, c_i, c_i, c_vp],
    "spv_haar_dwt": [c_vp, c_vp, c_i, c_i, c_i, c_i, c_i, c_i, c_i, c_vp, c_vp],
    "spv_patchify": [c_vp, c_vp, c_i, c_i, c_i, c_i, c_i, c_i, c_i, c_i, c_vp],
    "spv_patchify_u8": [c_vp, c_vp, c_vp, c_vp, c_i, c_i, c_i, c_i, c_i, c_i, c_i, c_i, c_vp],
    "spv_embed_posbias": [c_vp, c_vp, c_vp, c_vp, c_i, c_i, c_vp],
    "spv_embed_cls_rows": [c_vp, c_vp, c_vp, c_i, c_i, c_i, c_i, c_vp],
    "spv_spectral_fold": [c_vp, c_vp, c_vp, c_vp, c_i, c_i, c_i, c_vp],
    "spv_spectral_fold_bf16": [c_vp, c_vp, c_vp, c_vp, c_vp, c_i, c_i, c_i, c_vp],
    "spv_spectral_fold_bwd": [c_vp, c_vp, c_vp, c_vp, c_vp, c_vp, c_vp, c_vp, c_i, c_i, c_i, c_vp],
    "spv_dropout": [c_vp, c_vp, c_i64, c_f, c_u64, c_i, c_vp],
    "spv_attention_fwd": [c_vp, c_vp, c_vp, c_i, c_i, c_i, c_i, c_i, c_f, c_u64, c_vp],
    "spv_attention_bwd": [c_vp, c_vp, c_vp, c_vp, c_vp, c_i, c_i, c_i, c_i, c_i, c_f, c_u64, c_vp],
    "spv_attention_row0_fwd": [c_vp, c_vp, c_vp, c_i, c_vp, c_vp, c_i, c_i, c_i, c_i, c_i, c_f, c_u64, c_vp],
    "spv_attention_row0_bwd": [c_vp, c_vp, c_vp, c_vp, c_i, c_vp, c_vp, c_vp, c_vp, c_i, c_i, c_i, c_i, c_i, c_i, c_f, c_u64, c_vp],
    "spv_gelu_fwd": [c_vp, c_vp, c_i64, c_i, c_vp],
    "spv_gelu_bwd": [c_vp, c_vp, c_vp, c_i64, c_i, c_vp],
    "spv_colsum": [c_vp, c_vp, c_vp, c_i, c_i, c_i, c_vp],
    "spv_set_seed_device_ptr": [c_vp],
    "spv_seed_advance": [c_vp, c_vp],
    "spv_adamw_multi": [c_vp, c_vp, c_vp, c_vp, c_i, c_f, c_f, c_f, c_f, c_f, c_f, c_f, c_f, c_f, c_vp, c_vp],
    "spv_adamw_multi_ema": [c_vp, c_vp, c_vp, c_vp, c_i, c_f, c_f, c_f, c_f, c_f, c_f, c_f, c_f, c_f, c_vp, c_vp, c_f, c_i, c_f, c_vp],
    "spv_grad_sumsq": [c_vp, c_vp, c_vp, c_vp, c_i, c_vp, c_vp],
    "spv_step_control": [c_vp, c_i, c_vp, c_i, c_vp, c_i, c_i, c_i, c_d, c_f, c_vp],
    "spv_adamw_multi_ctl": [c_vp, c_vp, c_vp, c_vp, c_i, c_d, c_f, c_f, c_f, c_f, c_f, c_f, c_vp, c_vp, c_vp],
    "spv_adamw_multi_ctl_ema": [c_vp, c_vp, c_vp, c_vp, c_i, c_d, c_f, c_f, c_f, c_f, c_f, c_f, c_vp, c_vp, c_vp, c_f, c_i, c_vp],
    "spv_fwht": [c_vp, c_vp, c_vp, c_i, c_i, c_i, c_i, c_i, c_i, c_f, c_i, c_vp],
    "spv_axpby": [c_vp, c_vp, c_vp, c_f, c_f, c_i64, c_i, c_vp],
    "spv_spectrum_floats": [c_i, c_i],
    "spv_spectrum_log1p": [c_vp, c_vp, c_i, c_i, c_i, c_i, c_i, c_vp],
    "spv_conv3x3_fwd": [c_vp, c_vp, c_vp, c_vp, c_vp, c_i, c_i, c_i, c_i, c_i, c_i, c_vp],
    "spv_conv3x3_dgrad": [c_vp, c_vp, c_vp, c_vp, c_i, c_i, c_i, c_i, c_i, c_i, c_vp],
    "spv_conv3x3_wgrad": [c_vp, c_vp, c_vp, c_vp, c_vp, c_vp, c_i, c_i, c_i, c_i, c_i, c_i, c_i, c_vp],
    "spv_token_pool_fwd": [c_vp, c_vp, c_i, c_i, c_i, c_i, c_i, c_i, c_vp],
    "spv_token_pool_bwd": [c_vp, c_i, c_vp, c_vp, c_i, c_i, c_i, c_i, c_i, c_vp],
    "spv_augment_params": [c_vp, c_i, c_i, c_i, c_i, c_vp, c_u64, c_u64, c_vp],
    "spv_augment_supported": [c_i, c_i, c_i],
    "spv_augment_u8": [c_vp, c_vp, c_vp, c_vp, c_vp, c_vp, c_i, c_i, c_i, c_i, c_i, c_vp],
    "spv_augment_plan": [c_i, c_i, c_i],
    "spv_augment_tiled_ws_bytes": [c_i, c_i, c_i],
    "spv_augment_tiled_u8": [c_vp, c_vp, c_vp, c_vp, c_vp, c_vp, c_i, c_i, c_i, c_i, c_i, c_vp, ctypes.c_size_t, c_vp],
    "spv_teacher_view_supported": [c_i, c_i, c_i, c_i],
    "spv_teacher_view_u8": [c_vp, c_vp, c_vp, c_vp, c_vp, c_i, c_i, c_i, c_i, c_i, c_i, c_i, c_vp],
    "spv_distill_loss_workspace_floats": [],
    "spv_distill_loss_fwd": [c_vp, c_vp, c_vp, c_vp, c_vp, c_vp, c_i, c_i, c_f, c_f, c_f, c_vp],
    "spv_distill_loss_bwd": [c_vp, c_vp, c_vp, c_vp, c_vp, c_vp, c_i, c_i, c_f, c_f, c_f, c_vp],
    "spv_logit_cache_store": [c_vp, c_vp, c_vp, c_i, c_i, c_i, c_vp],
    "spv_distill_loss_idx_fwd": [c_vp, c_vp, c_vp, c_vp, c_vp, c_vp, c_vp, c_i, c_i, c_i, c_f, c_f, c_f, c_vp],
    "spv_distill_loss_idx_bwd": [c_vp, c_vp, c_vp, c_vp, c_vp, c_vp, c_vp, c_i, c_i, c_i, c_f, c_f, c_f, c_vp],
    "spv_eval_head_stats_words": [],
    "spv_eval_head": [c_vp, c_vp, c_vp, c_vp, c_vp, c_i, c_i, c_i, c_i, c_vp],
    "spv_train_meter_words": [c_i64],
    "spv_cross_entropy_meter_workspace_floats": [],
    "spv_cross_entropy_meter_fwd": [c_vp, c_vp, c_vp, c_vp, c_vp, c_i, c_i, c_vp, c_i, c_vp],
    "spv_distill_loss_meter_workspace_floats": [],
    "spv_distill_loss_meter_fwd": [c_vp, c_vp, c_vp, c_vp, c_vp, c_vp, c_i, c_i, c_f, c_f, c_f, c_vp, c_i, c_vp],
    "spv_distill_loss_idx_meter_fwd": [c_vp, c_vp, c_vp, c_vp, c_vp, c_vp, c_vp, c_i, c_i, c_i, c_f, c_f, c_f, c_vp, c_i, c_vp],
}
_RESTYPES = {"spv_last_error": ctypes.c_char_p, "spv_path_count": ctypes.c_longlong, "spv_rowop_partial_floats": c_i64, "spv_fnet_workspace_floats": c_i64,
             "spv_fnet_twiddle_floats": c_i64, "spv_tail_ln_partial_floats": c_i64, "spv_permut_table_words": c_i64, "spv_small_sl_partial_floats": c_i64,
             "spv_cross_entropy_workspace_floats": c_i64, "spv_distill_loss_workspace_floats": c_i64,
             "spv_eval_head_stats_words": c_i64, "spv_augment_tiled_ws_bytes": ctypes.c_size_t, "spv_train_meter_words": c_i64,
             "spv_cross_entropy_meter_workspace_floats": c_i64, "spv_distill_loss_meter_workspace_floats": c_i64}
_NO_STATUS = set(_RESTYPES) | {"spv_version", "spv_fnet_ln_supported", "spv_fnet_cls_supported", "spv_tail_ln_supported", "spv_tail_up_supported", "spv_small_sl_supported", "spv_tail_bwd_parts", "spv_embed_bwd_groups", "spv_haar_ln_supported", "spv_permut_pool_supported", "spv_spectrum_floats", "spv_augment_supported", "spv_augment_plan", "spv_teacher_view_supported"}

class FoldJob(ctypes.Structure):
    _fields_ = [("partials", c_vp), ("out", c_vp * 5), ("parts", c_i), ("nsum", c_i), ("n", c_i)]


class AugmentCfg(ctypes.Structure):
    _fields_ = [(n, c_f) for n in ("flip_p", "bright_lo", "bright_hi", "contrast_lo", "contrast_hi", "sat_lo", "sat_hi", "hue_lo", "hue_hi",
                                   "gray_p", "degrees", "blur_p", "sigma_lo", "sigma_hi", "erase_p", "scale_lo", "scale_hi", "ratio_lo",
                                   "ratio_hi")]


class TnProblem(ctypes.Structure):
    _fields_ = [("a", c_vp), ("b", c_vp), ("c", c_vp), ("m", c_i), ("n", c_i), ("lda", c_i), ("ldb", c_i), ("ldc", c_i), ("k", c_i)]


_lib = None
timer = None
hint = 0
_LAUNCHERS = {}


def load():
    global _lib
    if _lib is None:
        if not os.path.exists(LIB_PATH):
            raise RuntimeError(
                f"libspv_hip.so not found at {LIB_PATH}: build it with `python -c 'import __graft_entry__ as g; g.build()'` "
                "or `make -C vit-spectre-experiments_amd/csrc` (there is no CPU/PyTorch fallback for the Spectre-ViT kernels)")
        lib = ctypes.CDLL(LIB_PATH)
        for name, argtypes in SIGNATURES.items():
            fn = getattr(lib, name)
            fn.argtypes = argtypes
            fn.restype = _RESTYPES.get(name, c_i)
            if argtypes and argtypes[-1] is c_vp and name not in _NO_STATUS and name != "spv_fnet_make_twiddle":
                _LAUNCHERS[name] = ([i for i, t in enumerate(argtypes) if t in (c_i, c_i64)],
                                    [i for i, t in enumerate(argtypes[:-1]) if t is c_vp])
        if lib.spv_version() != 1:
            raise RuntimeError(f"libspv_hip.so ABI version {lib.spv_version()} != 1")
        _lib = lib
    return _lib


def call(name, *args):
    lib = load()
    if timer is not None and name in _LAUNCHERS:
        global hint
        ii, pi = _LAUNCHERS[name]
        ints = tuple(int(args[i]) for i in ii) + (sum(1 << b for b, i in enumerate(pi) if not args[i]), hint)
        hint = 0
        box = []
        timer.bracket(name, ints, lambda: box.append(getattr(lib, name)(*args)))
        rc = box[0]
    else:
        rc = getattr(lib, name)(*args)
    if name in _NO_STATUS:
        return rc
    if rc != 0:
        raise RuntimeError(f"{name} failed: {lib.spv_last_error().decode()}")
    return 0
```

vit-spectre-experiments_amd/spectre_vit/graph.py:

```python
from __future__ import annotations

import contextlib
import weakref

import torch

from spectre_vit import _native, hip_ops, shadows
from spectre_vit.dp import GradReducer

_seed_owner = None


def _claim_seed_word(obj):
    global _seed_owner
    cur = _seed_owner() if _seed_owner is not None else None
    if cur is not None and cur is not obj and not cur._closed:
        raise RuntimeError("a graph-replayed training step is already live in this process: the dropout seed word is one device "
                           "symbol of libspv_hip.so, so two live steps would share (or steal) each other's masks -- call .close() "
                           "on the old step first")
    _native.call("spv_set_seed_device_ptr", obj.seed_word.data_ptr())
    _seed_owner = weakref.ref(obj)


def _release_seed_word(obj):
    global _seed_owner
    cur = _seed_owner() if _seed_owner is not None else None
    if cur is obj or cur is None:
        if _seed_owner is not None:
            _native.call("spv_set_seed_device_ptr", 0)
        _seed_owner = None


class GraphedTrainStep:
    _dp = False

    def __init__(self, model, optimizer, criterion, example_img, example_labels, autocast_dtype=torch.bfloat16, warmup=3,
                 return_features=False, process_group=None, force_collective=False):
        if not example_img.is_cuda:
            raise RuntimeError(f"{type(self).__name__} needs the example batch on the GPU")
        for g in optimizer.param_groups:
            if not g.get("capturable", False):
                raise ValueError(f"{type(self).__name__}: build the optimizer with capturable=True (its step count must live on the device)")
        self._closed = True
        self.model, self.optimizer, self.criterion = model, optimizer, criterion
        self.autocast_dtype = autocast_dtype
        self.img = example_img.clone()
        self.labels = example_labels.clone()
        dev = self.img.device
        self.force_collective = bool(force_collective)
        self.reducer = GradReducer(model, always=True, process_group=process_group, overlap=not self._dp)
        if not self._dp and self.reducer.world > 1:
            raise RuntimeError("GraphedTrainStep is the single-process step; a rank of a torch.distributed job uses GraphedDPStep")
        self.seed_word = torch.zeros(1, dtype=torch.int64, device=dev)
        _claim_seed_word(self)
        self._closed = False
        self._one = torch.ones((), dtype=torch.float32, device=dev)
        self.replays = 0
        try:
            self._build(max(1, warmup))
        except BaseException:
            self.close()
            raise

    def _forward_backward(self):
        _native.call("spv_seed_advance", self.seed_word.data_ptr(), torch.cuda.current_stream().cuda_stream)
        self.reducer.zero_grad()
        with torch.autocast("cuda", dtype=self.autocast_dtype, enabled=self.autocast_dtype is not None):
            out = self.model(self.img)
        loss = self.criterion(out, self.labels)
        loss.backward(self._one)
        return loss, out

    def _eager_step(self):
        loss, out = self._forward_backward()
        self.reducer.finish()
        self.optimizer.step()
        return loss, out

    @contextlib.contextmanager
    def _hold(self):
        prev = hip_ops.HOLD_UNDER_DP
        hip_ops.HOLD_UNDER_DP = prev or self._dp
        try:
            yield
        finally:
            hip_ops.HOLD_UNDER_DP = prev

    def _warm(self, warmup):
        side = torch.cuda.Stream(device=self.img.device)
        side.wait_stream(torch.cuda.current_stream())
        with torch.cuda.stream(side), self._hold():
            for _ in range(warmup):
                loss, out = self._eager_step()
        torch.cuda.current_stream().wait_stream(side)
        self.warm_loss, self.warm_out = loss.detach(), out.detach()
        shadows.reset_shadow_cache()

    def _build(self, warmup):
        self._warm(warmup)
        self.graph = torch.cuda.CUDAGraph()
        with torch.cuda.graph(self.graph), self._hold():
            self.loss, self.out = self._eager_step()

    def _replay(self):
        self.graph.replay()

    def __call__(self, img=None, labels=None):
        if self._closed:
            raise RuntimeError("this graph-replayed step was closed")
        if img is not None:
            self.img.copy_(img, non_blocking=True)
        if labels is not None:
            self.labels.copy_(labels, non_blocking=True)
        self._replay()
        self.replays += 1
        shadows.invalidate_weight_shadows()
        return self.loss

    def close(self):
        if not self._closed:
            self._closed = True
            _release_seed_word(self)

    def __del__(self):
        try:
            self.close()
        except Exception:
            pass


class GraphedDPStep(GraphedTrainStep):
    _dp = True

    def _eager_step(self):
        loss, out = self._forward_backward()
        self.reducer.allreduce_flat(force=self.force_collective)
        self.optimizer.step()
        return loss, out

    def _build(self, warmup):
        self._warm(warmup)
        torch.cuda.synchronize()
        pool = torch.cuda.graph_pool_handle()
        mode = dict(capture_error_mode="thread_local")
        self.graph = torch.cuda.CUDAGraph()
        with torch.cuda.graph(self.graph, pool=pool, **mode), self._hold():
            self.loss, self.out = self._forward_backward()
        self.graph_opt = torch.cuda.CUDAGraph()
# ... 65 lines not shown
```

vit-spectre-experiments_amd/spectre_vit/hip_ops.py:

```python
from __future__ import annotations

import collections
import ctypes
import os
import warnings
import weakref
from typing import NamedTuple

import torch

from . import _native, shadows
from ._launch import _DT, BF16, F32, _dt, _p, _require_gpu, _stream
from .shadows import invalidate_weight_shadows
from .timing import KernelTimer, _timing, set_kernel_timer


_warned_fp16 = False


def compute_dtype(x: torch.Tensor) -> torch.dtype:
    global _warned_fp16
    if torch.is_autocast_enabled("cuda"):
        dt = torch.get_autocast_dtype("cuda")
        if dt == torch.float16:
            if not _warned_fp16:
                warnings.warn("spectre_vit (MI355X): fp16 autocast is served by the bf16 kernels")
                _warned_fp16 = True
            return torch.bfloat16
        if dt == torch.bfloat16:
            return torch.bfloat16
    if x.dtype in (torch.float32, torch.bfloat16):
        return x.dtype
    return torch.float32


def cast(x: torch.Tensor, dtype: torch.dtype) -> torch.Tensor:
    if x.dtype == dtype:
        return x
    return _Cast.apply(x, dtype)


def _raw_cast(x, dtype):
    x = x.contiguous()
    out = torch.empty(x.shape, dtype=dtype, device=x.device)
    _native.call("spv_cast", _p(x), _dt(x), _p(out), _DT[dtype], x.numel(), _stream())
    return out


class _Cast(torch.autograd.Function):
    @staticmethod
    def forward(ctx, x, dtype):
        _require_gpu(x)
        ctx.src = x.dtype
        return _raw_cast(x, dtype)

    @staticmethod
    def backward(ctx, g):
        return _raw_cast(g, ctx.src), None


def _gemm(a, b, bias, c, M, N, K, lda, ldb, ldc, accumulate=0, splits=1, workspace=None):
    if splits == 1 and K >= 256:
        tiles = ((M + 127) // 128) * ((N + 127) // 128)
        rows_kernel = (a.dtype == torch.bfloat16 and M <= 2048 and K <= 1536 and K % 16 == 0 and lda % 8 == 0 and ldb % 8 == 0
                       and 64 <= ((M + 31) // 32) * ((N + 31) // 32) <= 1024)
        if tiles <= 32 and not rows_kernel:
            splits = max(1, min(K // 64, 256 // tiles))
            if splits > 1:
                workspace = torch.empty((splits * M * N,), dtype=torch.float32, device=c.device)
    _gemm_launch(a, b, bias, c, M, N, K, lda, ldb, ldc, accumulate, splits, workspace)


def _gemm_launch(a, b, bias, c, M, N, K, lda, ldb, ldc, accumulate=0, splits=1, workspace=None):
    _native.call("spv_gemm_nt", _p(a), _p(b), _p(bias), _p(c), M, N, K, lda, ldb, ldc, _dt(a), _dt(c), accumulate, splits,
                 _p(workspace), _stream())


_SIDE_MIN_FLOPS = 1e11
_side_streams = {}
_side_keep = []


def _side_stream(dev):
    s = _side_streams.get(dev)
    if s is None:
        s = _side_streams[dev] = torch.cuda.Stream(device=dev)
    return s


def join_side_stream():
    if _side_keep:
        dev = _side_keep[0][0].device
        torch.cuda.current_stream().wait_stream(_side_streams[dev])
        _side_keep.clear()


PATH_COUNTS = collections.Counter()
_held_folds = []
_held_task = -2
FOLD_RIDERS = 6
_held_wgrads = []
WGRAD_BATCH = 8
BATCH_FOLDS = 16
_WGRAD_HOLD = True
FOLD_RIDE = True


HOLD_UNDER_DP = False
TIME_HELD = False


_task_id_fn = getattr(torch._C, "_current_graph_task_id", None)
_engine = getattr(getattr(torch.autograd, "Variable", None), "_execution_engine", None)
_HOLD_API = _task_id_fn is not None and hasattr(_engine, "queue_callback")


def _graph_task_id():
    return _task_id_fn() if _task_id_fn is not None else -1


def _hold_ok():
    if not _HOLD_API:
        return False
    if _timing() and not TIME_HELD:
        return False
    if HOLD_UNDER_DP:
        return True
    import torch.distributed as dist
    return not (dist.is_available() and dist.is_initialized() and dist.get_world_size() > 1)


_T = torch.Tensor
_Fold = NamedTuple("_Fold", [("partials", _T), ("outs", tuple), ("parts", int), ("n", int)])
_HeldWgrad = NamedTuple("_HeldWgrad", [("dh", _T), ("x", _T), ("dw", int), ("rows", int), ("n", int), ("k", int), ("fold", object)])


def _addrs(tensors):
    return tuple(t.data_ptr() for t in tensors)


def _fold_array(folds):
    arr = (_native.FoldJob * len(folds))()
    for j, f in zip(arr, folds):
        j.partials = _p(f.partials)
        for i, o in enumerate(f.outs):
            j.out[i] = o
        j.parts, j.nsum, j.n = f.parts, len(f.outs), f.n
    return arr


def _batch_splits(tiles):
    if 160 <= tiles <= 224:
        return 7
    best, best_score = 1, -1.0
    for sp in range(1, 11):
        rounds = tiles * sp / 512.0
        score = rounds / max(1.0, float(-(-tiles * sp // 512))) - 0.01 * sp
        if rounds >= 0.7 and score > best_score:
            best, best_score = sp, score
    return best


def _flush_held_wgrads():
    used = []
    while _held_wgrads:
        rows = max(w.rows for w in _held_wgrads)
        group = sorted(_held_wgrads, key=lambda w: -w.rows)[:WGRAD_BATCH]
        taken = {id(w) for w in group}
        _held_wgrads[:] = [w for w in _held_wgrads if id(w) not in taken]
        probs = (_native.TnProblem * len(group))()
        tiles = floats = 0
        flops = 0.0
        folds = []
        for q, w in zip(probs, group):
            n, k = w.n, w.k
            q.a, q.b, q.c, q.m, q.n, q.lda, q.ldb, q.ldc, q.k = _p(w.dh), _p(w.x), w.dw, n, k, n, k, k, w.rows
            if w.rows == rows:
                tiles += ((n + 127) // 128) * ((k + 127) // 128)
                floats += n * k
            flops += 2.0 * w.rows * n * k
            used += [w.dh, w.x]
            if w.fold is not None:
                folds.append(w.fold)
        while _held_folds and len(folds) < BATCH_FOLDS:
            folds.append(_held_folds.pop(0))
        splits = max(1, min(_batch_splits(tiles), rows // 256))
        ws = torch.empty((splits * floats,), dtype=torch.float32, device=group[0].dh.device)
        used.append(ws)
        used += [f.partials for f in folds]
        arr = _fold_array(folds) if folds else None
        batch = (ctypes.addressof(probs), len(group), rows, splits, _p(ws), ctypes.addressof(arr) if folds else 0, len(folds))
        if _timing():
            for part, work in ((1, flops), (2, 4.0 * floats * (splits + 1))):
                _native.hint = int(work)
                _native.call("spv_gemm_tn_batch_part", *batch, part, _stream())
        else:
            _native.call("spv_gemm_tn_batch", *batch, _stream())
        PATH_COUNTS["wgrad_batch"] += 1
        PATH_COUNTS["wgrad_batch_problems"] += len(group)
    return used


def start_held_wgrads():
    if not (_held_wgrads and _held_task == _graph_task_id()) or _timing():
        return False
    side = _side_stream(_held_wgrads[0].dh.device)
    side.wait_stream(torch.cuda.current_stream())
    with torch.cuda.stream(side):
        used = _flush_held_wgrads()
    if used:
        _side_keep.append(tuple(used))
    PATH_COUNTS["wgrad_side_start"] += 1
    return True


def _begin_pass(task):
    global _held_task
    if _held_task != task:
        _held_folds.clear()
        _held_wgrads.clear()
        _engine.queue_callback(flush_held_folds)
        _held_task = task


def _hold_wgrad(dh, x, dw, sink, rows, n, k, fold, fold_sunk):
    if not (_WGRAD_HOLD and _hold_ok() and _in_sink(dw, sink) and (fold is None or fold_sunk)):
        return False
    task = _graph_task_id()
    if task < 0:
        return False
    _begin_pass(task)
    _held_wgrads.append(_HeldWgrad(dh, x, dw.data_ptr(), rows, n, k, fold))
    return True


def _in_sink(dw, sink):
    if sink is None:
        return False
    base = sink.view.data_ptr()
    return base <= dw.data_ptr() and dw.data_ptr() + dw.numel() * dw.element_size() <= base + sink.view.numel() * sink.view.element_size()


def flush_held_folds():
    global _held_task
    _flush_held_wgrads()
    if _held_folds:
        arr = _fold_array(_held_folds)
        _native.call("spv_fold_multi", ctypes.addressof(arr), len(_held_folds), _stream())
        _held_folds.clear()
    _held_task = -2
    join_side_stream()


def _hold_fold(partials, outs, sinks, parts, n):
    if not _hold_ok() or not _sunk(outs, sinks):
        return False
    task = _graph_task_id()
    if task < 0:
        return False
    _begin_pass(task)
    _held_folds.append(_Fold(partials, _addrs(outs), parts, n))
    return True


def _fold_rides(dtype, rows, n, k):
    return (dtype == torch.bfloat16 and n % 8 == 0 and k % 8 == 0 and FOLD_RIDE
            and not (not _timing() and 2.0 * rows * n * k >= _SIDE_MIN_FLOPS))


def _fold_job(partials, outs, rows, n):
    return _Fold(partials, _addrs(outs), _native.call("spv_tail_bwd_parts", rows), n)


def _sunk(outs, sinks):
    return all(sk is not None and o.data_ptr() == sk.view.data_ptr() for o, sk in zip(outs, sinks))


def _weight_grad(dh, x, rows, n, k, sink=None, fold=None, fold_sunk=False, out=None):
    dev = dh.device
    dw = out if out is not None else _grad_buf(sink, (n, k), dev)
    tiles = ((n + 127) // 128) * ((k + 127) // 128)
    splits = max(1, min(512 // tiles, (rows + 511) // 512 if tiles >= 8 else (rows + 63) // 64))
    if tiles < 8:
        splits = min(splits, 64)
    elif n == 512 and k % 128 == 0 and k >= 1024 and rows >= 8192:
        splits = max(1, min(256 // (k // 128), rows // 2048))
    ws = None
    if dh.dtype == torch.bfloat16 and n % 8 == 0 and k % 8 == 0:
        if tiles >= 8 and 2.0 * rows * n * k < _SIDE_MIN_FLOPS and _hold_wgrad(dh, x, dw, sink, rows, n, k, fold, fold_sunk):
            return dw
        def launch(riders=True):
            nonlocal ws
            if ws is None and splits > 1:
                ws = torch.empty((splits * n * k,), dtype=torch.float32, device=dev)
            folds = [fold] if fold is not None else []
            if riders and _held_task == _graph_task_id():
                while _held_folds and len(folds) < FOLD_RIDERS:
                    folds.append(_held_folds.pop(0))
            if folds:
                arr = _fold_array(folds)
                _native.call("spv_gemm_tn_fold", _p(dh), _p(x), _p(dw), n, k, rows, n, k, k, F32, 0, splits, _p(ws), ctypes.addressof(arr),
                             len(folds), _stream())
            else:
                _native.call("spv_gemm_tn", _p(dh), _p(x), _p(dw), n, k, rows, n, k, k, F32, 0, splits, _p(ws), _stream())
        if not _timing() and 2.0 * rows * n * k >= _SIDE_MIN_FLOPS:
            side = _side_stream(dev)
            side.wait_stream(torch.cuda.current_stream())
            with torch.cuda.stream(side):
                launch(False)
            _side_keep.append((dh, x, ws, dw))
        else:
            launch()
        return dw
    ws = torch.empty((splits * n * k,), dtype=torch.float32, device=dev) if splits > 1 else None
    ld = (rows + 7) // 8 * 8
    dht = torch.empty((n, ld), dtype=dh.dtype, device=dev)
    xt = torch.empty((k, ld), dtype=x.dtype, device=dev)
    st = _stream()
    _native.call("spv_cast_transpose", _p(dh), _dt(dh), _p(dht), _dt(dht), rows, n, ld, 0, 0, 0, st)
    _native.call("spv_cast_transpose", _p(x), _dt(x), _p(xt), _dt(xt), rows, k, ld, 0, 0, 0, st)
    _gemm(dht, xt, None, dw, n, k, ld, ld, ld, k, 0, splits, ws)
    return dw


class GradSink:
    __slots__ = ("view", "used")

    def __init__(self, view):
# ... 209 lines not shown
def _fnet_twiddle(tokens, device):
    key = (tokens, device)
    t = _twiddles.get(key)
    if t is None:
        t = torch.empty((_native.call("spv_fnet_twiddle_floats", tokens),), dtype=torch.float32, device=device)
        _native.call("spv_fnet_make_twiddle", _p(t), tokens, _stream())
        _twiddles[key] = t
    return t


def _fnet_raw(x, add_in=None):
    B, N, D = x.shape
    xc = x.contiguous()
    y = torch.empty_like(xc)
    wsn = _native.call("spv_fnet_workspace_floats", B, N, D)
    ws = torch.empty((wsn,), dtype=torch.float32, device=x.device) if wsn else None
    tw = _fnet_twiddle(N, x.device)

    _native.call("spv_fnet_mix", _p(xc), _p(y), _p(add_in), _p(tw), B, N, D, _dt(xc), _p(ws), _stream())
    return y


class FNetMixFn(torch.autograd.Function):

    @staticmethod
    def forward(ctx, x):
        _require_gpu(x)
        return _fnet_raw(x)

    @staticmethod
    def backward(ctx, dy):
        return _fnet_raw(dy)


class RfftRealFn(torch.autograd.Function):

    @staticmethod
    def forward(ctx, x):
        _require_gpu(x)
        D = x.shape[-1]
        xc = _rows2d(x, D)
        y = torch.empty((xc.shape[0], D // 2 + 1), dtype=x.dtype, device=x.device)
        _native.call("spv_rfft_real", _p(xc), _p(y), xc.shape[0], D, 0, _dt(xc), _stream())
        ctx.meta = (x.shape, D)
        return y.reshape(*x.shape[:-1], D // 2 + 1)

    @staticmethod
    def backward(ctx, dy):
        shape, D = ctx.meta
        dyc = _rows2d(dy, D // 2 + 1)
        dx = torch.empty((dyc.shape[0], D), dtype=dy.dtype, device=dy.device)
        _native.call("spv_rfft_real", _p(dyc), _p(dx), dyc.shape[0], D, 1, _dt(dyc), _stream())
        return dx.reshape(shape)


def _haar_raw(x, axis, levels, inverse, zero_mode=False):
    B, N, D = x.shape
    xc = x.contiguous()
    y = torch.empty_like(xc)
    scratch = torch.empty_like(xc) if levels > 1 else None
    _native.call("spv_haar_dwt", _p(xc), _p(y), B, N, D, axis, levels, inverse | (2 if zero_mode else 0), _dt(xc), _p(scratch), _stream())
    return y


class HaarDWTFn(torch.autograd.Function):
    @staticmethod
    def forward(ctx, x, axis, levels, zero_mode=False):
        _require_gpu(x)
        ctx.meta = (axis, levels, bool(zero_mode))
        return _haar_raw(x, axis, levels, 0, zero_mode)

    @staticmethod
    def backward(ctx, dy):
        axis, levels, zero_mode = ctx.meta
        return _haar_raw(dy, axis, levels, 1, zero_mode), None, None, None


class SpectralFoldFn(torch.autograd.Function):

    @staticmethod
    def forward(ctx, proj_w, fh, fw, chans, patch):
        _require_gpu(proj_w)
        E = proj_w.shape[0]
        wf = torch.empty((E, chans * patch * patch), dtype=torch.float32, device=proj_w.device)
        if torch.is_autocast_enabled("cuda"):
            wb = torch.empty(wf.shape, dtype=torch.bfloat16, device=proj_w.device)
            _native.call("spv_spectral_fold_bf16", _p(proj_w), _p(fh), _p(fw), _p(wf), _p(wb), E, chans, patch, _stream())
            wf._spv_bf16 = wb
        else:
            _native.call("spv_spectral_fold", _p(proj_w), _p(fh), _p(fw), _p(wf), E, chans, patch, _stream())
        ctx.save_for_backward(proj_w, fh, fw)
        ctx.sinks = (_sink(proj_w), _sink(fh), _sink(fw))
        ctx.meta = (E, chans, patch)
        return wf

    @staticmethod
    def backward(ctx, dwf):
        proj_w, fh, fw = ctx.saved_tensors
        E, chans, patch = ctx.meta
        dwf = dwf.contiguous()
        dw = _grad_buf(ctx.sinks[0], proj_w.shape, proj_w.device)
        dfh = _grad_buf(ctx.sinks[1], fh.shape, fh.device)
        dfw = _grad_buf(ctx.sinks[2], fw.shape, fw.device)
        scratch = torch.empty_like(proj_w)
        _native.call("spv_spectral_fold_bwd", _p(dwf), _p(proj_w), _p(fh), _p(fw), _p(dw), _p(dfh), _p(dfw), _p(scratch), E,
                     chans, patch, _stream())
        return dw, dfh, dfw, None, None


class _EmbedKey:
    __slots__ = ("__weakref__",)


_cls_grad_stash = weakref.WeakKeyDictionary()


class PatchEmbedFn(torch.autograd.Function):

    @staticmethod
    def forward(ctx, img, w_full, bias, cls, pos, patch, dtype, norm=None, p_drop=0.0):
        _require_gpu(img, w_full)
        u8 = img.dtype == torch.uint8
        if u8:
            if norm is None:
                raise ValueError("uint8 images need the (mean, inv_std) normalisation tensors")
            B, H, W, C = img.shape
        else:
            B, C, H, W = img.shape
        E, K = w_full.shape
        Np = (H // patch) * (W // patch)
        T = Np + 1
        dev = img.device
        img = img.contiguous() if u8 else img.contiguous().float()
        _check_channels("patch embedding", E, K, dtype)
        st = _stream()
        patches = torch.empty((B * T, K), dtype=dtype, device=dev)
        if u8:
            _native.call("spv_patchify_u8", _p(img), _p(norm[0]), _p(norm[1]), _p(patches), B, C, H, W, patch, K, 2, _DT[dtype], st)
        else:
            _native.call("spv_patchify", _p(img), _p(patches), B, C, H, W, patch, K, 2, _DT[dtype], st)
        wc = w_full if dtype == torch.float32 else (getattr(w_full, "_spv_bf16", None) if dtype == torch.bfloat16 else None)
        if wc is None:
            wc = _raw_cast(w_full, dtype)
        posbias = torch.empty((T, E), dtype=torch.float32, device=dev)
        _native.call("spv_embed_posbias", _p(pos), _p(bias), _p(cls), _p(posbias), Np, E, st)
        tokens = torch.empty((B, T, E), dtype=dtype, device=dev)
        seed = _new_seed() if p_drop > 0.0 else 0
        _native.call("spv_gemm_nt_grouped_rows_drop", _p(patches), _p(wc), 0, _p(posbias), _p(tokens), B * T, E, K, K, K, E,
                     _DT[dtype], _DT[dtype], T, T, 0, float(p_drop), seed, st)
        ctx.save_for_backward(None if u8 else img, patches if (dtype == torch.bfloat16 or u8) else None)
        ctx.meta = (B, C, H, W, patch, E, K, Np, T, dtype, cls.shape, pos.shape, float(p_drop), seed)
        ctx.sinks = (_sink(bias), _sink(cls), _sink(pos))
        ctx.key = _EmbedKey()
        tokens._spv_embed_key = ctx.key
        return tokens

    @staticmethod
    def backward(ctx, dtok):
        img, patches = ctx.saved_tensors
        B, C, H, W, patch, E, K, Np, T, dtype, cls_shape, pos_shape, p_drop, seed = ctx.meta
        dev = dtok.device
        st = _stream()
        dtok = dtok.contiguous()
        early = start_held_wgrads()
        gcls = _cls_grad_stash.pop(ctx.key, None)
        if gcls is not None:
            gcls = gcls.to(dtok.dtype).contiguous()
        s_bias, s_cls, s_pos = ctx.sinks
        dpos_full = _grad_buf(s_pos, pos_shape, dev)
        dbias = _grad_buf(s_bias, (E,), dev)
        dcls = _grad_buf(s_cls, cls_shape, dev)
        part = torch.empty((_native.call("spv_embed_bwd_groups", B) * T * E,), dtype=torch.float32, device=dev)
        masked = torch.empty_like(dtok) if (gcls is not None or p_drop > 0.0) else None
        _native.call("spv_embed_bwd", _p(dtok), _p(gcls), _p(masked), _p(part), _p(dpos_full), _p(dbias), _p(dcls), B, T, E, p_drop, seed,
                     _dt(dtok), st)
        if masked is not None:
            dtok = masked
        if patches is not None and dtok.dtype == torch.bfloat16:
            dwf = _weight_grad(dtok.view(B * T, E), patches, B * T, E, K)
            if not early:
                join_side_stream()
            return None, dwf, dbias, dcls, dpos_full, None, None, None, None
        rows = B * Np
        ld = (rows + 7) // 8 * 8
        dyt = torch.empty((E, ld), dtype=dtok.dtype, device=dev)
        _native.call("spv_cast_transpose", _p(dtok), _dt(dtok), _p(dyt), _dt(dyt), rows, E, ld, Np, T, 1, st)
        pt = torch.empty((K, ld), dtype=dtok.dtype, device=dev)
        if img is None:
            _native.call("spv_cast_transpose", _p(patches), _dt(patches), _p(pt), _dt(pt), rows, K, ld, Np, T, 1, st)
        else:
            _native.call("spv_patchify", _p(img), _p(pt), B, C, H, W, patch, ld, 1, _dt(pt), st)
        dwf = torch.empty((E, K), dtype=torch.float32, device=dev)
        tiles = ((E + 127) // 128) * ((K + 127) // 128)
        splits = max(1, min(1024 // tiles, (ld + 511) // 512))
        ws = torch.empty((splits * E * K,), dtype=torch.float32, device=dev) if splits > 1 else None
        _gemm(dyt, pt, None, dwf, E, K, ld, ld, ld, K, 0, splits, ws)
        return None, dwf, dbias, dcls, dpos_full, None, None, None, None


CIFAR100_MEAN = (0.5071, 0.4867, 0.4408)
CIFAR100_STD = (0.2675, 0.2565, 0.2761)


class PixelNorm:

    def __init__(self, mean=CIFAR100_MEAN, std=CIFAR100_STD):
        self.mean = tuple(float(m) for m in mean)
        self.std = tuple(float(v) for v in std)
        self._cache = {}

    def tensors(self, device, channels):
        if len(self.mean) != channels or len(self.std) != channels:
            raise ValueError(f"pixel normalisation has {len(self.mean)} channels, the image has {channels}")
        t = self._cache.get(device)
        if t is None:
            t = (torch.tensor(self.mean, dtype=torch.float32, device=device),
                 torch.tensor([1.0 / v for v in self.std], dtype=torch.float32, device=device))
            self._cache[device] = t
        return t

    def __deepcopy__(self, memo):
        return PixelNorm(self.mean, self.std)


def patch_embed(x, w_full, bias, cls, pos, patch, pixel_norm, p_drop=0.0):
    if x.dtype == torch.uint8:
        dt = torch.bfloat16 if torch.is_autocast_enabled("cuda") else torch.float32
        norm = pixel_norm.tensors(x.device, x.shape[-1])
        return PatchEmbedFn.apply(x, w_full, bias, cls, pos, patch, dt, norm, float(p_drop))
    return PatchEmbedFn.apply(x, w_full, bias, cls, pos, patch, compute_dtype(x), None, float(p_drop))


class DropoutFn(torch.autograd.Function):
    @staticmethod
    def forward(ctx, x, p):
        _require_gpu(x)
        xc = x.contiguous()
        seed = _new_seed()
        y = torch.empty_like(xc)
        _native.call("spv_dropout", _p(xc), _p(y), xc.numel(), float(p), seed, _dt(xc), _stream())
        ctx.meta = (float(p), seed)
        return y

    @staticmethod
    def backward(ctx, dy):
        p, seed = ctx.meta
        dyc = dy.contiguous()
        dx = torch.empty_like(dyc)
        _native.call("spv_dropout", _p(dyc), _p(dx), dyc.numel(), p, seed, _dt(dyc), _stream())
        return dx, None


def dropout(x, p, training):
    if not training or p <= 0.0:
        return x
    return DropoutFn.apply(x, p)


class AddFn(torch.autograd.Function):

    @staticmethod
    def forward(ctx, a, b):
# ... 20 lines not shown
    def backward(ctx, gx, gcls):
        if gcls is None:
            return gx
        if gx is None:
            raise RuntimeError("TapClsFn: the layer stack produced no input gradient")
        if ctx.key is not None:
            _cls_grad_stash[ctx.key] = gcls
            return gx
        if not gx.is_contiguous():
            gx = gx.contiguous()
        gx[:, 0, :] += gcls.to(gx.dtype)
        return gx


_cls_grad_bufs = {}
LAST_LAYER_CLS_ONLY = os.environ.get("SPV_FULL_LAST_LAYER", "0") == "0"


class TakeClsFn(torch.autograd.Function):

    @staticmethod
    def forward(ctx, x):
        _require_gpu(x)
        ctx.meta = (x.shape, x.dtype)
        return x[:, 0, :].contiguous()

    @staticmethod
    def backward(ctx, g):
        shape, dtype = ctx.meta
        return _cls_row_gradient(shape, dtype, g.device, g)


class PermutClsFn(torch.autograd.Function):

    @staticmethod
    def forward(ctx, x, table, n):
        _require_gpu(x)
        B, N, E = x.shape
        xc = x.contiguous()
        g0 = torch.empty((B, n), dtype=xc.dtype, device=xc.device)
        x0 = torch.empty((B, E), dtype=xc.dtype, device=xc.device)
        _native.call("spv_permut_row0_fwd", _p(xc), _p(table), _p(g0), _p(x0), B, N * E, n, E, _dt(xc), _stream())
        ctx.table = table
        ctx.meta = (B, N, E, n, xc.dtype)
        return g0, x0

    @staticmethod
    def backward(ctx, dg0, dx0):
        B, N, E, n, dtype = ctx.meta
        dev = ctx.table.device
        dg0 = torch.zeros((B, n), dtype=dtype, device=dev) if dg0 is None else dg0.to(dtype).contiguous()
        dx0 = torch.zeros((B, E), dtype=dtype, device=dev) if dx0 is None else dx0.to(dtype).contiguous()
        dx = torch.empty((B, N, E), dtype=dtype, device=dev)
        _native.call("spv_permut_row0_bwd", _p(dg0), _p(dx0), _p(ctx.table), _p(dx), B, N * E, n, E, _DT[dtype], _stream())
        return dx, None, None


def _cls_row_gradient(shape, dtype, dev, rows):
    if shape[1] == 1:
        return rows.to(dtype).reshape(shape)
    key = (tuple(shape), dtype, dev.index)
    full = _cls_grad_bufs.get(key)
    if full is None:
        if len(_cls_grad_bufs) > 8:
            _cls_grad_bufs.clear()
        full = torch.zeros(shape, dtype=dtype, device=dev)
        _cls_grad_bufs[key] = full
    full[:, 0, :] = rows
    return full


class ClsAddFn(torch.autograd.Function):

    @staticmethod
    def forward(ctx, out, src_cls):
        _require_gpu(out, src_cls)
        ctx.meta = (out.shape, out.dtype)
        return out[:, 0, :] + src_cls

    @staticmethod
    def backward(ctx, g):
        shape, dtype = ctx.meta
        return _cls_row_gradient(shape, dtype, g.device, g), g


def small_head_ok(rows: int, n: int, k: int) -> bool:
    return bool(_native.call("spv_small_sl_supported", int(rows), int(n), int(k)))


class ClsHeadFn(torch.autograd.Function):

    @staticmethod
    def forward(ctx, out, src_cls, weight, bias, gamma, beta):
        _require_gpu(out, src_cls, weight)
        B, N, E = out.shape
        n = weight.shape[0]
        if not out.is_contiguous():
            out = out.contiguous()
        if src_cls.stride(-1) != 1:
            src_cls = src_cls.contiguous()
        if src_cls.dtype != out.dtype or weight.dtype != torch.float32 or not weight.is_contiguous():
            raise ValueError("ClsHeadFn: src_cls must have the stack's dtype and the head weight must be contiguous fp32")
        dev = out.device
        logits = torch.empty((B, n), dtype=torch.float32, device=dev)
        h = torch.empty((B, n), dtype=torch.float32, device=dev)
        xs = torch.empty((B, E), dtype=torch.float32, device=dev)
        mean, rstd = _row_stats(B, dev)
        _native.call("spv_small_sl_fwd", _p(out), N * E, _p(src_cls), src_cls.stride(0), _p(weight), _p(bias), _p(gamma), _p(beta), _p(logits), _p(h),
                     _p(xs), _p(mean), _p(rstd), B, n, E, _dt(out), _stream())
        ctx.save_for_backward(h, xs, mean, rstd, weight, gamma, beta)
        ctx.meta = (out.shape, out.dtype)
        ctx.sinks = (_sink(weight), _sink(bias), _sink(gamma), _sink(beta))
        ctx.set_materialize_grads(False)
        return logits, xs

    @staticmethod
    def backward(ctx, dlogits, dfeats):
        h, xs, mean, rstd, weight, gamma, beta = ctx.saved_tensors
        shape, dtype = ctx.meta
        B, n = h.shape
        E = xs.shape[1]
        dev = h.device
        if dlogits is None:
            dlogits = torch.zeros_like(h)
        dlogits = dlogits.contiguous().float()
        s_w, s_b, s_g, s_be = ctx.sinks
        dh = torch.empty_like(h)
        dx = torch.empty((B, E), dtype=dtype, device=dev)
        dw = _grad_buf(s_w, (n, E), dev)
        dbias = _grad_buf(s_b, (n,), dev)
        dgamma = _grad_buf(s_g, (n,), dev)
        dbeta = _grad_buf(s_be, (n,), dev)
        partials = torch.empty((_native.call("spv_small_sl_partial_floats", B, n),), dtype=torch.float32, device=dev)
        _native.call("spv_small_sl_bwd", _p(dlogits), _p(h), _p(xs), _p(mean), _p(rstd), _p(weight), _p(gamma), _p(beta), _p(dh), _p(dx),
                     _p(dw), _p(dgamma), _p(dbeta), _p(dbias), _p(partials), B, n, E, _DT[dtype], _stream())
        if dfeats is not None:
            dx = dx + dfeats.to(dx.dtype)
        return _cls_row_gradient(shape, dtype, dev, dx), dx, dw, dbias, dgamma, dbeta


_ce_workspaces = {}


class CrossEntropyFn(torch.autograd.Function):

    @staticmethod
    def forward(ctx, logits, labels):
        _require_gpu(logits, labels)
        if logits.dim() != 2 or logits.dtype != torch.float32 or labels.dtype != torch.int64 or labels.shape != logits.shape[:1]:
            raise ValueError("cross_entropy: fp32 logits [rows, classes] and int64 labels [rows] expected")
        z = logits.contiguous()
        y = labels.contiguous()
        rows, C = z.shape
        lse = torch.empty((rows,), dtype=torch.float32, device=z.device)
        loss = torch.empty((), dtype=torch.float32, device=z.device)
        _native.call("spv_cross_entropy_fwd", _p(z), _p(y), _p(lse), _p(loss), _p(_zero_workspace(_ce_workspaces, z.device, "spv_cross_entropy_workspace_floats")), rows, C, _stream())
        ctx.save_for_backward(z, y, lse)
        return loss

    @staticmethod
    def backward(ctx, go):
        z, y, lse = ctx.saved_tensors
        go = go.reshape(1).float().contiguous()
        dz = torch.empty_like(z)
        _native.call("spv_cross_entropy_bwd", _p(z), _p(y), _p(lse), _p(go), _p(dz), z.shape[0], z.shape[1], _stream())
        return dz, None


def _meter_block(meter, dev, what):
    block = meter.tensor()
    if block.dtype != torch.int64 or not block.is_contiguous() or block.device != dev:
        raise ValueError(f"{what}: the meter's block is a contiguous int64 tensor on the logits' device ({dev}), got {block.dtype} on {block.device}")
    return block, int(meter.topk)


_ce_meter_workspaces = {}


class CrossEntropyMeterFn(torch.autograd.Function):

    @staticmethod
    def forward(ctx, logits, labels, meter):
        _require_gpu(logits, labels)
        if logits.dim() != 2 or logits.dtype != torch.float32 or labels.dtype != torch.int64 or labels.shape != logits.shape[:1]:
            raise ValueError("cross_entropy: fp32 logits [rows, classes] and int64 labels [rows] expected")
        block, k = _meter_block(meter, logits.device, "cross_entropy")
        z = logits.contiguous()
        y = labels.contiguous()
        rows, C = z.shape
        lse = torch.empty((rows,), dtype=torch.float32, device=z.device)
        loss = torch.empty((), dtype=torch.float32, device=z.device)
        _native.call("spv_cross_entropy_meter_fwd", _p(z), _p(y), _p(lse), _p(loss),
                     _p(_zero_workspace(_ce_meter_workspaces, z.device, "spv_cross_entropy_meter_workspace_floats")), rows, C, _p(block), k, _stream())
        ctx.save_for_backward(z, y, lse)
        return loss

    @staticmethod
    def backward(ctx, go):
        return CrossEntropyFn.backward(ctx, go) + (None,)


def cross_entropy(logits, labels, meter=None):
    if meter is not None:
        return CrossEntropyMeterFn.apply(logits, labels, meter)
    return CrossEntropyFn.apply(logits, labels)


def eval_head_stats(device):
    return torch.zeros((_native.call("spv_eval_head_stats_words"),), dtype=torch.int64, device=device)


def eval_head(logits, labels, n_valid, pred, stats, k=5):
    _require_gpu(logits, labels, n_valid, pred, stats)
    if logits.dim() != 2 or not logits.is_contiguous():
        raise ValueError("eval_head: contiguous logits [rows, classes] expected")
    rows, C = logits.shape
    if (labels.dtype != torch.int64 or pred.dtype != torch.int64 or n_valid.dtype != torch.int32 or stats.dtype != torch.int64
            or labels.numel() < rows or pred.numel() < rows or n_valid.numel() < 1
# ... 605 lines not shown
```

vit-spectre-experiments_amd/spectre_vit/models/spectre/spectre.py:

```python
import torch
import torch.nn as nn
from torch.nn.modules.transformer import _get_activation_fn, _get_clones

from spectre_vit import hip_ops, shadows
from spectre_vit.models.spectre.layers import MHPermutMix, SpectreLinear
from spectre_vit.modules.mixers import FNetMixer, HaarDWTMixer, SelfAttentionMixer

MIXERS = ("permut", "fft", "dwt_embed", "dwt_token", "attention")


class Transpose(nn.Module):

    def __init__(self, dims=(-2, -1)):
        super(Transpose, self).__init__()
        self.dims = dims

    def forward(self, x):
        return x.transpose(self.dims[0], self.dims[1])


def _make_mixer(mixer, d_model, seq_length, nhead, dwt_levels, dwt_mode="passthrough", dropout=0.0):
    if mixer == "permut":
        return MHPermutMix(d_model, seq_length, nhead, d_model)
    if mixer == "fft":
# ... 56 lines not shown
        if self.mixer == "fft":
            x = hip_ops.FNetResidualFn.apply(x, self.norm1.weight, self.norm1.bias)
        elif self.mixer == "dwt_embed" and hip_ops.haar_ln_ok(x, self.mix_layer.axis, self.mix_layer.levels):
            x = hip_ops.HaarResidualFn.apply(x, self.norm1.weight, self.norm1.bias)
        else:
            x = hip_ops.add_layernorm(self.mix_layer(x), x, self.norm1.weight, self.norm1.bias, 0)
        return x

    def _ff(self, x):
        l1, l3 = self.linear1.local_head, self.linear3.local_head
        mult = 8 if x.dtype == torch.bfloat16 else 4
        if (l1[0].in_features % mult == 0 and l1[0].out_features % mult == 0):
            p = self.linear1.drop_p if self.training else 0.0
            return hip_ops.FFResidualFn.apply(x, l1[0].weight, l1[0].bias, l1[1].weight, l1[1].bias, l3[0].weight, l3[0].bias,
                                              l3[1].weight, l3[1].bias, self.norm2.weight, self.norm2.bias, p)
        return hip_ops.add_layernorm(self._ff_block(x), x, self.norm2.weight, self.norm2.bias, 1)

    def _ff_block(self, x: torch.Tensor) -> torch.Tensor:
        return self.linear3(self.linear1(x))


class SpectreEncoder(nn.Module):

    __constants__ = ["norm"]

    def __init__(self, encoder_layer, num_layers: int, norm=None) -> None:
        super().__init__()
        self.layers = _get_clones(encoder_layer, num_layers)
        self.num_layers = num_layers
        self.norm = norm

    def forward(self, src: torch.Tensor):
        src = hip_ops.cast(src, hip_ops.compute_dtype(src))
        output = src
        for mod in self.layers:
            output = mod(output)
        if self.norm is not None:
            output = self.norm(output)
        return hip_ops.AddFn.apply(output, src)

    def forward_cls(self, src: torch.Tensor):
        src = hip_ops.cast(src, hip_ops.compute_dtype(src))
        output, src_cls = hip_ops.TapClsFn.apply(src)
        output = self._stack_cls(output)
        return hip_ops.ClsAddFn.apply(output, src_cls)

    def _stack_cls(self, output):
        layers = list(self.layers)
        cls_only = hip_ops.LAST_LAYER_CLS_ONLY and len(layers) > 0 and output.is_cuda
        for mod in (layers[:-1] if cls_only else layers):
            output = mod(output)
        if cls_only:
            output = layers[-1].forward_cls(output).unsqueeze(1)
        if self.norm is not None:
            output = self.norm(output)
        return output

    def forward_cls_parts(self, src: torch.Tensor):
        src = hip_ops.cast(src, hip_ops.compute_dtype(src))
        output, src_cls = hip_ops.TapClsFn.apply(src)
        return self._stack_cls(output), src_cls


class SpectralPatchEmbed(nn.Module):

    def __init__(self, embed_dim, patch_size, num_patches, dropout, in_channels):
        super().__init__()
        self.P = patch_size
        self.embed_dim = embed_dim
        self.in_channels = in_channels
        self.freq_weight_h = nn.Parameter(torch.ones(self.P))
        self.freq_weight_w = nn.Parameter(torch.ones(self.P // 2 + 1))
        self.proj = nn.Linear(in_channels * self.P * (self.P // 2 + 1), embed_dim)
        self.cls_token = nn.Parameter(torch.randn(1, 1, embed_dim))
        self.position_embeddings = nn.Parameter(torch.randn(1, num_patches + 1, embed_dim))
        self.dropout = nn.Dropout(dropout)
        self.pixel_norm = hip_ops.PixelNorm()

    def forward(self, x):
        C = x.shape[-1] if x.dtype == torch.uint8 else x.shape[1]
        w_full = hip_ops.SpectralFoldFn.apply(self.proj.weight, self.freq_weight_h, self.freq_weight_w, C, self.P)
        return hip_ops.patch_embed(x, w_full, self.proj.bias, self.cls_token, self.position_embeddings, self.P, self.pixel_norm,
                                   self.dropout.p if self.training else 0.0)


class SpectreViT(nn.Module):

    def __init__(self, img_size=32, patch_size=4, in_channels=3, num_classes=10, embed_dim=768, num_encoders=12,
                 num_heads=12, hidden_dim=3072, dropout=0.1, activation="gelu", mixer="permut", dwt_levels=1, dwt_mode="passthrough"):
        super().__init__()
        num_patches = (img_size // patch_size) ** 2
        self.embeddings_block = SpectralPatchEmbed(embed_dim, patch_size, num_patches, dropout, in_channels)
        encoder_layer = SpectreEncoderLayer(seq_length=num_patches + 1, d_model=embed_dim, nhead=num_heads,
                                            dim_feedforward=hidden_dim, dropout=dropout, activation=activation,
                                            mixer=mixer, dwt_levels=dwt_levels, dwt_mode=dwt_mode)
        self.encoder_blocks = SpectreEncoder(encoder_layer, num_layers=num_encoders)
        self.mlp_head = nn.Sequential(SpectreLinear(embed_dim, num_classes))
        self.mlp_head[0].out_fp32 = True

    def _shadow_weights(self):
        cand = self.__dict__.get("_shadow_candidates")
        if cand is None or cand[0] != len(self.encoder_blocks.layers):
            mods = [mod for layer in self.encoder_blocks.layers for mod in layer.modules() if isinstance(mod, (SpectreLinear, SelfAttentionMixer))]
            cand = self.__dict__["_shadow_candidates"] = (len(self.encoder_blocks.layers), mods)
        ws = []
        for mod in cand[1]:
            for w in ((mod.in_proj_weight, mod.out_proj.weight) if isinstance(mod, SelfAttentionMixer) else (mod.local_head[0].weight,)):
                if w.requires_grad and w.shape[0] % 8 == 0 and w.shape[1] % 8 == 0:
                    ws.append(w)
        return ws

    def _observed(self):
        from torch.nn.modules import module as _m
        if _m._global_forward_hooks or _m._global_forward_pre_hooks:
            return True
        watched = [self.encoder_blocks, *self.encoder_blocks.layers, self.mlp_head, *self.mlp_head]
        if self.encoder_blocks.layers:
            watched += list(self.encoder_blocks.layers[-1].children())
        return any(w._forward_hooks or w._forward_pre_hooks for w in watched)

    def forward(self, x, return_features=False):
        if torch.is_grad_enabled() and x.is_cuda and torch.is_autocast_enabled("cuda"):
            shadows.refresh_weight_shadows(self, self._shadow_weights)
        x = self.embeddings_block(x)
        if self._observed():
            x = self.encoder_blocks(x)
            cls_token = x[:, 0, :]
            x = self.mlp_head(cls_token)
            return (x, cls_token) if return_features else x
        head = self.mlp_head[0] if len(self.mlp_head) == 1 and isinstance(self.mlp_head[0], SpectreLinear) else None
        if (head is not None and (head.drop_p == 0.0 or not self.training) and x.is_cuda
                and hip_ops.small_head_ok(x.shape[0], head.out_channels, head.in_channels)):
            output, src_cls = self.encoder_blocks.forward_cls_parts(x)
            lin, ln = head.local_head[0], head.local_head[1]
            x, cls_token = hip_ops.ClsHeadFn.apply(output, src_cls, lin.weight, lin.bias, ln.weight, ln.bias)
        else:
            cls_token = self.encoder_blocks.forward_cls(x)
            x = self.mlp_head(cls_token)
        if return_features:
            return x, cls_token
        return x
```

vit-spectre-experiments_amd/spectre_vit/shadows.py:

```python
from __future__ import annotations

import contextlib
import weakref

import torch

from . import _native
from ._launch import _DT, _p, _stream


def _pair(w, dtype):
    n, k = w.shape
    wd = w.detach()
    wc = wd if dtype == torch.float32 else torch.empty((n, k), dtype=dtype, device=w.device)
    ldt = (n + 7) // 8 * 8
    wt = torch.empty((k, ldt), dtype=dtype, device=w.device)
    _native.call("spv_weight_shadows", _p(wd), 0 if wc is wd else _p(wc), _p(wt), n, k, ldt, _DT[dtype], _stream())
    return wc, wt


def _multi_table(ents):
    dev = ents[0][0].device
    rows, tt, tx, ty = [], [], [], []
    for i, (w, wc, wt) in enumerate(ents):
        n, k = w.shape
        ld = wt.shape[1]
        rows += [w.data_ptr(), 0 if wc.data_ptr() == w.data_ptr() else wc.data_ptr(), wt.data_ptr(), n | (k << 32), ld]
        for by in range((ld + 31) // 32):
            for bx in range((k + 63) // 64):
                tt.append(i)
                tx.append(bx)
                ty.append(by)
    return (torch.tensor(rows, dtype=torch.int64).to(dev), torch.tensor(tt, dtype=torch.int32).to(dev),
            torch.tensor(tx, dtype=torch.int32).to(dev), torch.tensor(ty, dtype=torch.int32).to(dev), len(tt))


def _refresh_multi(tables, dtype):
    table, tt, tx, ty, ntiles = tables
    _native.call("spv_weight_shadows_multi", table.data_ptr(), tt.data_ptr(), tx.data_ptr(), ty.data_ptr(), ntiles, _DT[dtype], _stream())


class _ShadowCache:

    def __init__(self):
        self._d = {}
        self._fresh = {}
        self.epoch = 0

    def get(self, w: torch.Tensor, dtype: torch.dtype):
        if _pinned is not None:
            return _pinned.get(w, dtype)
        key = (id(w), dtype)
        ent = self._d.get(key)
        ver = (w.data_ptr(), w._version, tuple(w.shape), self.epoch)
        training = torch.is_grad_enabled() and w.requires_grad
        if not training and ent is not None and ent[0]() is w and ent[1] == ver:
            return ent[2], ent[3]
        fresh = self._fresh.pop(key, None)
        if fresh is not None and fresh[0]() is w and fresh[3] == (w._version, self.epoch):
            return fresh[1], fresh[2]
        wc, wt = _pair(w, dtype)
        if len(self._d) > 1024:
            self._d = {kk: e for kk, e in self._d.items() if e[0]() is not None}
        self._d[key] = (weakref.ref(w), ver, wc, wt)
        return wc, wt

    def reset(self):
        self._d = {}
        self._fresh = {}


_shadows = _ShadowCache()
get = _shadows.get


def reset_shadow_cache():
    _shadows.reset()


class ShadowSet:

    def __init__(self, weights, dtype=torch.bfloat16):
        self.weights = [weakref.ref(w) for w in weights]
        self.dtype = dtype
        self.key = tuple((w.data_ptr(), tuple(w.shape)) for w in weights)
        dev = weights[0].device
        self.bufs = [(torch.empty(tuple(w.shape), dtype=dtype, device=dev),
                      torch.empty((w.shape[1], (w.shape[0] + 7) // 8 * 8), dtype=dtype, device=dev)) for w in weights]
        self._tables = _multi_table([(w, wc, wt) for w, (wc, wt) in zip(weights, self.bufs)])

    def refresh(self):
        _refresh_multi(self._tables, self.dtype)
        for wr, (wc, wt) in zip(self.weights, self.bufs):
            w = wr()
            if w is not None:
                _shadows._fresh[(id(w), self.dtype)] = (wr, wc, wt, (w._version, _shadows.epoch))


class PinnedShadows:

    def __init__(self):
        self.ent = {}
        self._tables = {}

    def get(self, w, dtype):
        key = (id(w), dtype)
        e = self.ent.get(key)
        if e is not None and e[0] is w:
            return e[1], e[2]
        if torch.cuda.is_current_stream_capturing():
            raise RuntimeError("a weight asked for its compute-dtype copies for the first time inside a graph capture: the warm-up "
                               "forward must run the very launch sequence that is captured")
        wc, wt = _pair(w, dtype)
        self.ent[key] = (w, wc, wt)
        return wc, wt

    def refresh(self):
        for dtype in {dt for _, dt in self.ent}:
            ents = [e for (_, dt), e in self.ent.items() if dt == dtype]
            t = self._tables.get(dtype)
            if t is None or t[0] != len(ents):
                t = self._tables[dtype] = (len(ents), _multi_table(ents))
            _refresh_multi(t[1], dtype)


_pinned = None


@contextlib.contextmanager
def pinned_shadows(p):
    global _pinned
    prev, _pinned = _pinned, p
    try:
        yield p
    finally:
        _pinned = prev


def refresh_weight_shadows(module, weights_fn):
    weights = weights_fn()
    if not weights:
        return
    ss = getattr(module, "_spv_shadow_set", None)
    key = tuple((w.data_ptr(), tuple(w.shape)) for w in weights)
    if ss is None or ss.key != key:
        if torch.cuda.is_current_stream_capturing():
            return
        ss = ShadowSet(weights)
        object.__setattr__(module, "_spv_shadow_set", ss)
    ss.refresh()


def invalidate_weight_shadows(*_args, **_kwargs):
    _shadows.epoch += 1


from torch.optim.optimizer import register_optimizer_step_post_hook as _register_post_step

_register_post_step(invalidate_weight_shadows)
```

vit-spectre-experiments_amd/spectre_vit/timing.py:

```python
from __future__ import annotations

import torch

from . import _native
from ._launch import BF16, F32

PEAK_TFLOPS = {BF16: 2500.0, F32: 157.3}
PEAK_HBM_GBS = 8000.0


def _es(dt):
    return 2 if dt == BF16 else 4


_WORK_MODELS = {
    "spv_small_sl_fwd": lambda i: ("head_fwd", i[2:5], i[5], "mfma", 2.0 * i[2] * i[3] * i[4]),
    "spv_small_sl_bwd": lambda i: ("head_bwd", i[0:3], i[3], "mfma", 4.0 * i[0] * i[1] * i[2]),
    "spv_cross_entropy_fwd": lambda i: ("cross_entropy_fwd", i[0:2], F32, "hbm", i[0] * i[1] * 4.0),
    "spv_cross_entropy_bwd": lambda i: ("cross_entropy_bwd", i[0:2], F32, "hbm", i[0] * i[1] * 8.0),
    "spv_distill_loss_fwd": lambda i: ("distill_loss_fwd", i[0:2], F32, "hbm", i[0] * i[1] * 8.0),
    "spv_distill_loss_bwd": lambda i: ("distill_loss_bwd", i[0:2], F32, "hbm", i[0] * i[1] * 12.0),
    "spv_distill_loss_idx_fwd": lambda i: ("distill_loss_idx_fwd", (i[0], i[2]), F32, "hbm", i[0] * (i[2] * 8.0 + 8.0)),
    "spv_distill_loss_idx_bwd": lambda i: ("distill_loss_idx_bwd", (i[0], i[2]), F32, "hbm", i[0] * (i[2] * 12.0 + 8.0)),
    "spv_cross_entropy_meter_fwd": lambda i: ("cross_entropy_meter_fwd", i[0:2], F32, "hbm", i[0] * i[1] * 4.0),
    "spv_distill_loss_meter_fwd": lambda i: ("distill_loss_meter_fwd", i[0:2], F32, "hbm", i[0] * i[1] * 8.0),
    "spv_distill_loss_idx_meter_fwd": lambda i: ("distill_loss_idx_meter_fwd", (i[0], i[2]), F32, "hbm", i[0] * (i[2] * 8.0 + 8.0)),
    "spv_logit_cache_store": lambda i: ("logit_cache_store", (i[0], i[2]), F32, "hbm", i[0] * (i[2] * 8.0 + 8.0)),
    "spv_teacher_view_u8": lambda i: ("teacher_view", (i[0], i[2], i[3], i[5]), i[6], "hbm",
                                      1.0 * i[0] * i[2] * (i[3] * i[3] + i[5] * i[5] * _es(i[6]))),
    "spv_gemm_nt": lambda i: ("gemm_acc" if i[8] else "gemm", i[0:3], i[6], "mfma", 2.0 * i[0] * i[1] * i[2]),
    "spv_gemm_nt_grouped_rows": lambda i: ("gemm_grouped_rows", i[0:3], i[6], "mfma", 2.0 * i[0] * i[1] * i[2]),
    "spv_gemm_nt_grouped_rows_drop": lambda i: ("gemm_grouped_rows", i[0:3], i[6], "mfma", 2.0 * i[0] * i[1] * i[2]),
    "spv_gemm_nt_pool_bwd": lambda i: ("gemm_pool_bwd", i[1:4], i[7], "mfma", 2.0 * i[1] * i[2] * i[3]),
    "spv_gemm_tn": lambda i: ("gemm_tn", i[0:3], BF16, "mfma", 2.0 * i[0] * i[1] * i[2]),
    "spv_gemm_tn_fold": lambda i: ("gemm_tn", i[0:3], BF16, "mfma", 2.0 * i[0] * i[1] * i[2]),
    "spv_gemm_tn_batch_part": lambda i: (("gemm_tn_batch", i[0:3], BF16, "mfma", float(i[-1])) if i[4] == 1 else
                                         ("splitk_reduce_batch", i[0:4], F32, "hbm", float(i[-1]))),
    "spv_embed_bwd": lambda i: ("embed_bwd", i[0:3], i[3], "hbm", 1.0 * i[0] * i[1] * i[2] * _es(i[3]) * (1 if (i[-2] >> 2) & 1 else 2)),
    "spv_fnet_cls_fwd": lambda i: ("fnet_cls_fwd", i[0:3], i[3], "hbm", 1.0 * i[0] * (i[1] + 1) * i[2] * _es(i[3])),
    "spv_fnet_cls_bwd": lambda i: ("fnet_cls_bwd", i[0:3], i[3], "hbm", 1.0 * i[0] * (i[1] + 1) * i[2] * _es(i[3])),
    "spv_permut_row0_fwd": lambda i: ("permut_row0_fwd", i[0:4], i[4], "hbm", 2.0 * i[0] * (i[2] + i[3]) * _es(i[4])),
    "spv_permut_row0_bwd": lambda i: ("permut_row0_bwd", i[0:4], i[4], "hbm", 1.0 * i[0] * (i[1] + i[2] + i[3]) * _es(i[4])),
    "spv_patchify": lambda i: ("patchify", i[0:5], i[7], "hbm",
                               1.0 * i[0] * i[1] * i[2] * i[3] * 4 + 1.0 * i[0] * ((i[2] // i[4]) * (i[3] // i[4]) + (i[6] == 2)) * i[5] * _es(i[7])),
    "spv_weight_shadows_multi": lambda i: ("weight_shadows_multi", i[0:1], i[1], "hbm", 2048.0 * i[0] * (4 + 2 * _es(i[1]))),
    "spv_spectre_tail_fwd": lambda i: ("tail_fwd", i[0:3], i[3], "hbm", i[0] * (2.0 * i[1] + i[2]) * _es(i[3])),
    "spv_spectre_tail_bwd": lambda i: ("tail_bwd" if not (i[-2] >> 7) & 1 else "tail_bwd_nodx", i[0:3], i[3], "hbm",
                                       i[0] * (3.0 * i[1] + (0 if (i[-2] >> 7) & 1 else i[2])) * _es(i[3])),
    "spv_spectre_tail_bwd_up": lambda i: ("tail_bwd_up", i[0:3], i[3], "hbm", i[0] * (3.0 * i[1] + 3.0 * i[2]) * _es(i[3])),
    "spv_spectre_tail_ln_fwd": lambda i: ("tail_ln_fwd", i[0:3], i[3], "hbm", i[0] * (4.0 * i[1] + i[2]) * _es(i[3])),
    "spv_spectre_tail_ln_bwd": lambda i: ("tail_ln_bwd", i[0:3], i[3], "hbm", i[0] * 6.0 * i[1] * _es(i[3])),
    "spv_add_layernorm_fwd": lambda i: ("addln_fwd", i[0:2], i[3], "hbm", 3.0 * i[0] * i[1] * _es(i[3])),
    "spv_add_layernorm_bwd": lambda i: ("addln_bwd", i[0:2], i[3], "hbm", (3.0 + (i[2] == 1)) * i[0] * i[1] * _es(i[3])),
    "spv_permut_gather_fwd": lambda i: ("gather_fwd", i[1:4], i[4], "hbm", i[1] * i[3] * (1.0 + i[2]) * _es(i[4])),
    "spv_permut_gather_bwd": lambda i: ("gather_bwd", i[0:3], i[3], "hbm", i[0] * i[2] * (1.0 + i[1]) * _es(i[3])),
    "spv_fnet_mix": lambda i: ("fnet_mix", i[0:3], i[3], "hbm", 2.0 * i[0] * i[1] * i[2] * _es(i[3])),
    "spv_fnet_ln_fwd": lambda i: ("fnet_ln_fwd", i[0:3], i[3], "hbm", 3.0 * i[0] * i[1] * i[2] * _es(i[3])),
    "spv_fnet_ln_bwd": lambda i: ("fnet_ln_bwd", i[0:3], i[3], "hbm", 3.0 * i[0] * i[1] * i[2] * _es(i[3])),
    "spv_haar_ln_fwd": lambda i: ("haar_ln_fwd", i[0:2], i[2], "hbm", 2.0 * i[0] * i[1] * _es(i[2])),
    "spv_haar_ln_bwd": lambda i: ("haar_ln_bwd", i[0:2], i[2], "hbm", 3.0 * i[0] * i[1] * _es(i[2])),
    "spv_haar_dwt": lambda i: ("haar_dwt", i[0:3], i[6], "hbm", 2.0 * i[0] * i[1] * i[2] * _es(i[6])),
    "spv_adamw_multi": lambda i: ("adamw_multi", i[0:1], F32, "hbm", 7.0 * 4 * 2048 * i[0]),
    "spv_adamw_multi_ema": lambda i: ("adamw_multi_ema", i[0:1], F32, "hbm", 9.0 * 4 * 2048 * i[0]),
    "spv_adamw_multi_ctl_ema": lambda i: ("adamw_multi_ctl_ema", i[0:1], F32, "hbm", 9.0 * 4 * 2048 * i[0]),
    "spv_grad_sumsq": lambda i: ("grad_sumsq", i[0:1], F32, "hbm", 4.0 * 2048 * i[0]),
    "spv_step_control": lambda i: ("step_control", i[0:2], F32, "hbm", 8.0 * i[0] + 64),
    "spv_adamw_multi_ctl": lambda i: ("adamw_multi_ctl", i[0:1], F32, "hbm", 7.0 * 4 * 2048 * i[0]),
    "spv_weight_shadows": lambda i: ("weight_shadows", i[0:2], i[3], "hbm", i[0] * i[1] * (4.0 + 2 * _es(i[3]))),
    "spv_dropout": lambda i: ("dropout", i[0:1], i[1], "hbm", 2.0 * i[0] * _es(i[1])),
    "spv_axpby": lambda i: ("axpby", i[0:1], i[1], "hbm", 3.0 * i[0] * _es(i[1])),
    "spv_colsum": lambda i: ("colsum", i[0:2], i[2], "hbm", 1.0 * i[0] * i[1] * _es(i[2])),
    "spv_cast": lambda i: ("cast", i[2:3], i[1], "hbm", 1.0 * i[2] * (_es(i[0]) + _es(i[1]))),
}


class KernelTimer:
    def __init__(self):
        self.records = []
        self.empties = []
        self.overhead_s = 0.0
        self.passes = 0

    def bracket(self, name, key, launch):
        e0 = torch.cuda.Event(enable_timing=True)
        e1 = torch.cuda.Event(enable_timing=True)
        e0.record()
        launch()
        e1.record()
        self.records.append((name, key, e0, e1))
        if len(self.records) % 8 == 0:
            z0, z1 = torch.cuda.Event(enable_timing=True), torch.cuda.Event(enable_timing=True)
            z0.record()
            z1.record()
            self.empties.append((z0, z1))

    def _groups(self):
        torch.cuda.synchronize()
        if self.empties:
            self.overhead_s = sorted(a.elapsed_time(b) for a, b in self.empties)[len(self.empties) // 2] * 1e-3
            self.empties = []
        groups = {}
        for name, key, e0, e1 in self.records:
            g = groups.setdefault((name, key), [0, 0.0])
            g[0] += 1
            g[1] += max(e0.elapsed_time(e1) * 1e-3, 1e-7)
        return groups

    @staticmethod
    def _work(name, key):
        model = _WORK_MODELS.get(name)
        if model is not None:
            label, shape, dt, bound, work = model(key)
            peak = PEAK_TFLOPS[dt] * 1e12 if bound == "mfma" else PEAK_HBM_GBS * 1e9
            return label, list(shape), "bf16" if dt == BF16 else "f32", bound, work, peak
        if name.startswith("torch:") and key and key[0] > 0:
            return name, [], "f32", "hbm", float(key[0]), PEAK_HBM_GBS * 1e9
        return name.replace("spv_", ""), list(key[:4]), "-", None, 0.0, 1.0

    def summary(self):
        out = []
        for (name, key), (cnt, tot) in sorted(self._groups().items(), key=lambda kv: -kv[1][1]):
            label, shape, dt, bound, work, peak = self._work(name, key)
            d = dict(kernel=label, shape=shape, dtype=dt, launches=cnt, avg_us=round(tot / cnt * 1e6, 2), total_ms=round(tot * 1e3, 3))
            if bound is not None:
                ach = work * cnt / tot
                d.update(bound=bound, achieved=round(ach / (1e12 if bound == "mfma" else 1e9), 2),
                         unit="TFLOP/s" if bound == "mfma" else "GB/s", frac=round(ach / peak, 4), algorithmic=int(work))
            out.append(d)
        return out

    def roofline(self):
        s = [d for d in self.summary() if "bound" in d]
        if not s:
            return None
        d = s[0]
        peak = (PEAK_TFLOPS[BF16 if d["dtype"] == "bf16" else F32]) if d["bound"] == "mfma" else PEAK_HBM_GBS
        return dict(bound=d["bound"], achieved=d["achieved"], peak=peak, unit=d["unit"], frac=d["frac"], traffic=None,
                    kernel=d["kernel"], shape=d["shape"], avg_us=d["avg_us"], launches=d["launches"],
                    event_overhead_us=round(self.overhead_s * 1e6, 2))


def set_kernel_timer(t):
    _native.timer = t


def _timing():
    return _native.timer is not None
```

Measured before the change: 329,800 images/sec.

## Fuse per-step prologue kernels into one launch and split head weight-grad

Adds a single step-prologue kernel that does the seed advance, weight-shadow refresh, spectral fold, patchify and position-bias work in one launch. Its results are deposited in a keyed cache that the later forward ops take instead of launching their own kernels. The small-head backward is split into separate row and weight-gradient entry points so the weight gradient can be deferred, and the weight-grad kernel is retuned to 256 threads with smaller tiles. The aim is to cut launch count and host overhead per step, at the cost of pointer-identity cache bookkeeping and a risk of stale or mismatched deposits.

Measured after the change: 334,700 images/sec, median of 6. 1.01x the previous value.

```diff
diff --git a/include/spv.h b/include/spv.h
--- a/include/spv.h
+++ b/include/spv.h
@@ -166,6 +166,30 @@
 int spv_set_seed_device_ptr(const void* seed_word);
 int spv_seed_advance(void* seed_word, void* stream);
 
+typedef struct spv_prologue_jobs {
+    void* seed_word;
+    const void* shadow_table;
+    const int* tile_tensor;
+    const int* tile_x;
+    const int* tile_y;
+    int ntiles, shadow_dtype;
+    const float* fold_w;
+    const float* fold_fh;
+    const float* fold_fw;
+    float* fold_out;
+    void* fold_out_bf16;
+    int fold_embed, fold_chans, fold_patch, pad0;
+    const float* patch_img;
+    void* patch_out;
+    int patch_batch, patch_chans, patch_height, patch_width, patch_size, patch_ld, patch_dtype, pad1;
+    const float* pos_pos;
+    const float* pos_bias;
+    const float* pos_cls;
+    float* pos_out;
+    int pos_patches, pos_embed;
+} spv_prologue_jobs;
+int spv_step_prologue(const spv_prologue_jobs* jobs, void* stream);
+
 int spv_adamw_multi(const void* table, const int* chunk_tensor, const int* chunk_off, const int* sizes, int nchunks, float lr,
                     float beta1, float beta2, float one_minus_beta1, float one_minus_beta2, float eps, float weight_decay,
                     float bias_correction1, float bias_correction2, const float* step_dev, void* stream);
@@ -249,6 +273,11 @@
                      const float* W, const float* gamma, const float* beta, float* dh, void* dx, float* dW,
                      float* dgamma, float* dbeta, float* dbias, float* partials, int rows, int n, int k, int dx_dtype,
                      void* stream);
+int spv_small_sl_bwd_rows(const float* dout, const float* h, const float* mean, const float* rstd, const float* W,
+                          const float* gamma, const float* beta, float* dh, void* dx, float* partials, int rows, int n, int k,
+                          int dx_dtype, void* stream);
+int spv_small_sl_bwd_w(const float* dh, const float* xs, const float* partials, float* dW, float* dgamma, float* dbeta,
+                       float* dbias, int rows, int n, int k, void* stream);
 int64_t spv_cross_entropy_workspace_floats(void);
 int spv_cross_entropy_fwd(const float* logits, const int64_t* labels, float* lse, float* loss, float* workspace, int rows,
                           int classes, void* stream);
diff --git a/vit-spectre-experiments_amd/csrc/spv_head.hip b/vit-spectre-experiments_amd/csrc/spv_head.hip
--- a/vit-spectre-experiments_amd/csrc/spv_head.hip
+++ b/vit-spectre-experiments_amd/csrc/spv_head.hip
@@ -230,39 +230,42 @@
     }
 }
 
-constexpr int WT = 1024, WCOLS = 128, WGRP = WT / WCOLS, WOUT = 2;
+constexpr int WT = 256, WCOLS = 32, WGRP = WT / WCOLS, WOUT = 2;
 __global__ __launch_bounds__(WT) void small_sl_bwd_w_kernel(const float* __restrict__ dh, const float* __restrict__ xs,
                                                             const float* __restrict__ partials, float* __restrict__ dW,
                                                             float* __restrict__ dgamma, float* __restrict__ dbeta, float* __restrict__ dbias,
                                                             int rows, int n, int k, int nparts, int cblocks) {
-    __shared__ float red[WGRP][WOUT][WCOLS];
+    constexpr int SL = 16;
+    __shared__ float smem[SL * 64];
     const int tid = threadIdx.x;
     const int njobs = ((n + WOUT - 1) / WOUT) * cblocks;
     if ((int)blockIdx.x == njobs) {
-        constexpr int SL = 16;
-        float* fold = &red[0][0][0];
         for (int e0 = 0; e0 < 3 * n; e0 += 64) {
-            const int e = e0 + (tid & 63), q = tid >> 6;
-            float a = 0.0f;
-            if (e < 3 * n) {
-                const int w = e / n, c = e - w * n;
-                for (int p0 = q; p0 < nparts; p0 += SL * 8) {
-                    float v[8];
-#pragma unroll
-                    for (int j = 0; j < 8; ++j) {
-                        const int pp = p0 + j * SL;
-                        v[j] = partials[((size_t)min(pp, nparts - 1) * 3 + w) * n + c] * (pp < nparts ? 1.0f : 0.0f);
+            const int e = e0 + (tid & 63);
+#pragma unroll
+            for (int u = 0; u < SL / (WT / 64); ++u) {
+                const int q = (tid >> 6) + u * (WT / 64);
+                float a = 0.0f;
+                if (e < 3 * n) {
+                    const int w = e / n, c = e - w * n;
+                    for (int p0 = q; p0 < nparts; p0 += SL * 8) {
+                        float v[8];
+#pragma unroll
+                        for (int j = 0; j < 8; ++j) {
+                            const int pp = p0 + j * SL;
+                            v[j] = partials[((size_t)min(pp, nparts - 1) * 3 + w) * n + c] * (pp < nparts ? 1.0f : 0.0f);
+                        }
+#pragma unroll
+                        for (int j = 0; j < 8; ++j) a += v[j];
                     }
-#pragma unroll
-                    for (int j = 0; j < 8; ++j) a += v[j];
                 }
-            }
-            fold[q * 64 + (tid & 63)] = a;
+                smem[q * 64 + (tid & 63)] = a;
+            }
             __syncthreads();
             if (tid < 64 && e < 3 * n) {
                 float t = 0.0f;
 #pragma unroll
-                for (int j = 0; j < SL; ++j) t += fold[j * 64 + tid];
+                for (int j = 0; j < SL; ++j) t += smem[j * 64 + tid];
                 const int w = e / n, c = e - w * n;
                 (w == 0 ? dgamma : (w == 1 ? dbeta : dbias))[c] = t;
             }
@@ -270,12 +273,13 @@
         }
         return;
     }
+    float (*red)[WOUT][WCOLS] = reinterpret_cast<float (*)[WOUT][WCOLS]>(smem);
     const int o0 = ((int)blockIdx.x / cblocks) * WOUT, c = ((int)blockIdx.x % cblocks) * WCOLS + (tid & (WCOLS - 1));
-    const int g = __builtin_amdgcn_readfirstlane(tid / WCOLS);
+    const int g = tid / WCOLS;
     const int o1 = min(o0 + 1, n - 1);
     const int cc = min(c, k - 1);
     float a0 = 0.0f, a1 = 0.0f;
-    constexpr int RB = 32;
+    constexpr int RB = 16;
     for (int rb = g; rb < rows; rb += WGRP * RB) {
         float x[RB], d0[RB], d1[RB];
 #pragma unroll
@@ -467,23 +471,36 @@
     return 0;
 }
 
-extern "C" int spv_small_sl_bwd(const float* dout, const float* h, const float* xs, const float* mean, const float* rstd, const float* W,
-                                const float* gamma, const float* beta, float* dh, void* dx, float* dW, float* dgamma, float* dbeta,
-                                float* dbias, float* partials, int rows, int n, int k, int dx_dtype, void* stream) {
-    SPV_CHECK(spv_small_sl_supported(rows, n, k), "spv_small_sl_bwd: rows=%d n=%d k=%d outside the small-rows kernel", rows, n, k);
-    SPV_CHECK(dx_dtype == SPV_F32 || dx_dtype == SPV_BF16, "spv_small_sl_bwd: bad dtype %d", dx_dtype);
+extern "C" int spv_small_sl_bwd_rows(const float* dout, const float* h, const float* mean, const float* rstd, const float* W, const float* gamma,
+                                     const float* beta, float* dh, void* dx, float* partials, int rows, int n, int k, int dx_dtype, void* stream) {
+    SPV_CHECK(spv_small_sl_supported(rows, n, k), "spv_small_sl_bwd_rows: rows=%d n=%d k=%d outside the small-rows kernel", rows, n, k);
+    SPV_CHECK(dx_dtype == SPV_F32 || dx_dtype == SPV_BF16, "spv_small_sl_bwd_rows: bad dtype %d", dx_dtype);
     hipStream_t st = static_cast<hipStream_t>(stream);
     const int nparts = cdiv(rows, HR);
     if (dx_dtype == SPV_BF16)
         hipLaunchKernelGGL((small_sl_bwd_rows_kernel<bf16_t>), dim3(nparts), dim3(HT), 0, st, dout, h, mean, rstd, gamma, beta, W, dh, dx, partials, rows, n, k);
     else
         hipLaunchKernelGGL((small_sl_bwd_rows_kernel<float>), dim3(nparts), dim3(HT), 0, st, dout, h, mean, rstd, gamma, beta, W, dh, dx, partials, rows, n, k);
-    SPV_LAUNCH_CHECK("spv_small_sl_bwd(rows)");
+    SPV_LAUNCH_CHECK("spv_small_sl_bwd_rows");
+    return 0;
+}
+
+extern "C" int spv_small_sl_bwd_w(const float* dh, const float* xs, const float* partials, float* dW, float* dgamma, float* dbeta, float* dbias,
+                                  int rows, int n, int k, void* stream) {
+    SPV_CHECK(spv_small_sl_supported(rows, n, k), "spv_small_sl_bwd_w: rows=%d n=%d k=%d outside the small-rows kernel", rows, n, k);
+    SPV_CHECK(dh && xs && partials && dW && dgamma && dbeta && dbias, "spv_small_sl_bwd_w: null pointer");
     const int cblocks = cdiv(k, WCOLS);
-    hipLaunchKernelGGL(small_sl_bwd_w_kernel, dim3(cdiv(n, WOUT) * cblocks + 1), dim3(WT), 0, st, dh, xs, partials, dW, dgamma, dbeta, dbias, rows,
-                       n, k, nparts, cblocks);
-    SPV_LAUNCH_CHECK("spv_small_sl_bwd(weights)");
-    return 0;
+    hipLaunchKernelGGL(small_sl_bwd_w_kernel, dim3(cdiv(n, WOUT) * cblocks + 1), dim3(WT), 0, static_cast<hipStream_t>(stream), dh, xs, partials,
+                       dW, dgamma, dbeta, dbias, rows, n, k, cdiv(rows, HR), cblocks);
+    SPV_LAUNCH_CHECK("spv_small_sl_bwd_w");
+    return 0;
+}
+
+extern "C" int spv_small_sl_bwd(const float* dout, const float* h, const float* xs, const float* mean, const float* rstd, const float* W,
+                                const float* gamma, const float* beta, float* dh, void* dx, float* dW, float* dgamma, float* dbeta,
+                                float* dbias, float* partials, int rows, int n, int k, int dx_dtype, void* stream) {
+    if (int rc = spv_small_sl_bwd_rows(dout, h, mean, rstd, W, gamma, beta, dh, dx, partials, rows, n, k, dx_dtype, stream)) return rc;
+    return spv_small_sl_bwd_w(dh, xs, partials, dW, dgamma, dbeta, dbias, rows, n, k, stream);
 }
 
 extern "C" int64_t spv_cross_entropy_workspace_floats() { return CE_MAX_WG + 1; }
diff --git a/vit-spectre-experiments_amd/csrc/spv_misc.hip b/vit-spectre-experiments_amd/csrc/spv_misc.hip
--- a/vit-spectre-experiments_amd/csrc/spv_misc.hip
+++ b/vit-spectre-experiments_amd/csrc/spv_misc.hip
@@ -1,5 +1,6 @@
 #include "spv_common.h"
 #include "spv_adamw_core.h"
+#include "spv_prologue_core.h"
 
 #include <string.h>
 
@@ -60,58 +61,12 @@
 }
 
 template <typename TO>
-__device__ __forceinline__ void weight_shadow_tile(const float* __restrict__ src, TO* __restrict__ plain, TO* __restrict__ tr, int rows,
-                                                   int cols, int ld, int bx, int by, float (*tile)[65]) {
-    const int r0 = by * 32, c0 = bx * 64;
-    const int t = threadIdx.x;
-    const bool vec = (cols & 3) == 0;
-#pragma unroll
-    for (int pass = 0; pass < 2; ++pass) {
-        const int rl = pass * 16 + (t >> 4), c4 = (t & 15) * 4;
-        const int r = r0 + rl, c = c0 + c4;
-        float v[4] = {0.0f, 0.0f, 0.0f, 0.0f};
-        if (r < rows) {
-            if (vec && c + 3 < cols) {
-                const float4 f = *reinterpret_cast<const float4*>(src + (size_t)r * cols + c);
-                v[0] = f.x; v[1] = f.y; v[2] = f.z; v[3] = f.w;
-                if (plain != nullptr) io<TO>::st4(plain + (size_t)r * cols + c, v);
-            } else {
-                for (int u = 0; u < 4; ++u)
-                    if (c + u < cols) {
-                        v[u] = src[(size_t)r * cols + c + u];
-                        if (plain != nullptr) io<TO>::st(plain + (size_t)r * cols + c + u, v[u]);
-                    }
-            }
-        }
-#pragma unroll
-        for (int u = 0; u < 4; ++u) tile[rl][c4 + u] = v[u];
-    }
-    __syncthreads();
-    const int cl = t >> 2, r8 = (t & 3) * 8;
-    const int c = c0 + cl;
-    if (c < cols) {
-        TO* o = tr + (size_t)c * ld + r0 + r8;
-        if (r0 + r8 + 7 < ld && (ld & 7) == 0) {
-            float a[4], b[4];
-#pragma unroll
-            for (int u = 0; u < 4; ++u) { a[u] = tile[r8 + u][cl]; b[u] = tile[r8 + 4 + u][cl]; }
-            io<TO>::st4(o, a);
-            io<TO>::st4(o + 4, b);
-        } else {
-            for (int u = 0; u < 8; ++u)
-                if (r0 + r8 + u < ld) io<TO>::st(o + u, tile[r8 + u][cl]);
-        }
-    }
-}
-
-template <typename TO>
 __global__ __launch_bounds__(256) void weight_shadow_kernel(const float* __restrict__ src, TO* __restrict__ plain, TO* __restrict__ tr,
                                                             int rows, int cols, int ld) {
     __shared__ float tile[32][65];
     weight_shadow_tile<TO>(src, plain, tr, rows, cols, ld, blockIdx.x, blockIdx.y, tile);
 }
 
-struct ShadowTensor { const float* src; void* plain; void* tr; int rows, cols, ld, pad; };
 template <typename TO>
 __global__ __launch_bounds__(256) void weight_shadow_multi_kernel(const ShadowTensor* __restrict__ tab, const int* __restrict__ tile_tensor,
                                                                   const int* __restrict__ tile_x, const int* __restrict__ tile_y) {
@@ -346,6 +301,7 @@
     adamw_chunk<false, true>(a, n, off, lr, beta1, beta2, omb1, omb2, eps, wd, bc1, bc2, step_dev, 1.0f, ema_tab[t], ema_w, ema_warmup,
                              ema_step);
 }
+
 }
 
 extern "C" int spv_adamw_multi(const void* table, const int* chunk_tensor, const int* chunk_off, const int* sizes, int nchunks, float lr,
@@ -387,7 +343,55 @@
 int spv_seed_ptr_set_attn(const unsigned long long* p);
 int spv_seed_ptr_set_gemm(const unsigned long long* p);
 namespace {
-__global__ void seed_advance_kernel(unsigned long long* p) { *p += 0x9e3779b97f4a7c15ull; }
+__global__ void seed_advance_kernel(unsigned long long* p) { *p += SEED_STEP; }
+
+struct PrologueArgs {
+    spv_prologue_jobs j;
+    int n_seed, n_shadow, n_fold, n_patch, n_pos;
+    int patch_vec4;
+};
+
+__global__ __launch_bounds__(256) void step_prologue_kernel(const PrologueArgs a) {
+    __shared__ float tile[32][65];
+    int bid = blockIdx.x;
+    if (bid < a.n_seed) {
+        if (threadIdx.x == 0) *static_cast<unsigned long long*>(a.j.seed_word) += SEED_STEP;
+        return;
+    }
+    bid -= a.n_seed;
+    if (bid < a.n_shadow) {
+        const ShadowTensor t = static_cast<const ShadowTensor*>(a.j.shadow_table)[a.j.tile_tensor[bid]];
+        if (a.j.shadow_dtype == SPV_BF16)
+            weight_shadow_tile<bf16_t>(t.src, static_cast<bf16_t*>(t.plain), static_cast<bf16_t*>(t.tr), t.rows, t.cols, t.ld, a.j.tile_x[bid],
+                                       a.j.tile_y[bid], tile);
+        else
+            weight_shadow_tile<float>(t.src, static_cast<float*>(t.plain), static_cast<float*>(t.tr), t.rows, t.cols, t.ld, a.j.tile_x[bid],
+                                      a.j.tile_y[bid], tile);
+        return;
+    }
+    bid -= a.n_shadow;
+    if (bid < a.n_fold) {
+        spectral_fold_body(a.j.fold_w, a.j.fold_fh, a.j.fold_fw, a.j.fold_out, a.j.fold_embed, a.j.fold_chans, a.j.fold_patch,
+                           static_cast<bf16_t*>(a.j.fold_out_bf16), bid, a.n_fold);
+        return;
+    }
+    bid -= a.n_fold;
+    if (bid < a.n_patch) {
+        const bool bf = a.j.patch_dtype == SPV_BF16;
+        if (!a.patch_vec4)
+            patchify_body(a.j.patch_img, a.j.patch_out, a.j.patch_batch, a.j.patch_chans, a.j.patch_height, a.j.patch_width, a.j.patch_size,
+                          a.j.patch_ld, 2, bf, bid, a.n_patch);
+        else if (bf)
+            patchify_vec4_body<bf16_t>(a.j.patch_img, static_cast<bf16_t*>(a.j.patch_out), a.j.patch_batch, a.j.patch_chans, a.j.patch_height,
+                                       a.j.patch_width, a.j.patch_size, a.j.patch_ld, 1, bid, a.n_patch);
+        else
+            patchify_vec4_body<float>(a.j.patch_img, static_cast<float*>(a.j.patch_out), a.j.patch_batch, a.j.patch_chans, a.j.patch_height,
+                                      a.j.patch_width, a.j.patch_size, a.j.patch_ld, 1, bid, a.n_patch);
+        return;
+    }
+    bid -= a.n_patch;
+    if (bid < a.n_pos) posbias_body(a.j.pos_pos, a.j.pos_bias, a.j.pos_cls, a.j.pos_out, a.j.pos_patches, a.j.pos_embed, bid, a.n_pos);
+}
 }
 extern "C" int spv_set_seed_device_ptr(const void* seed_word) {
     const unsigned long long* p = static_cast<const unsigned long long*>(seed_word);
@@ -401,3 +405,48 @@
     SPV_LAUNCH_CHECK("spv_seed_advance");
     return 0;
 }
+
+extern "C" int spv_step_prologue(const spv_prologue_jobs* jobs, void* stream) {
+    SPV_CHECK(jobs != nullptr, "spv_step_prologue: null jobs");
+    PrologueArgs a;
+    a.j = *jobs;
+    const spv_prologue_jobs& j = a.j;
+    a.n_seed = j.seed_word != nullptr ? 1 : 0;
+    SPV_CHECK(j.ntiles >= 0, "spv_step_prologue: ntiles = %d", j.ntiles);
+    a.n_shadow = (j.shadow_table != nullptr && j.ntiles > 0) ? j.ntiles : 0;
+    if (a.n_shadow) {
+        SPV_CHECK(j.tile_tensor && j.tile_x && j.tile_y, "spv_step_prologue: null tile lists");
+        SPV_CHECK(j.shadow_dtype == SPV_BF16 || j.shadow_dtype == SPV_F32, "spv_step_prologue: bad shadow dtype %d", j.shadow_dtype);
+    }
+    a.n_fold = 0;
+    if (j.fold_w != nullptr && j.fold_embed > 0) {
+        SPV_CHECK(j.fold_fh && j.fold_fw && j.fold_out && j.fold_chans > 0 && j.fold_patch > 0, "spv_step_prologue: bad spectral-fold arguments");
+        a.n_fold = patch_ew_blocks((int64_t)j.fold_embed * j.fold_chans * j.fold_patch * j.fold_patch);
+    }
+    a.n_patch = a.patch_vec4 = 0;
+    if (j.patch_img != nullptr && j.patch_batch > 0) {
+        SPV_CHECK(j.patch_out && j.patch_chans > 0 && j.patch_size > 0 && j.patch_height >= j.patch_size && j.patch_width >= j.patch_size,
+                  "spv_step_prologue: bad patch shape");
+        SPV_CHECK(j.patch_dtype == SPV_F32 || j.patch_dtype == SPV_BF16, "spv_step_prologue: bad patch dtype");
+        const int Np = (j.patch_height / j.patch_size) * (j.patch_width / j.patch_size), K = j.patch_chans * j.patch_size * j.patch_size;
+        SPV_CHECK(j.patch_ld >= K, "spv_step_prologue: patch ld=%d too small", j.patch_ld);
+        if (j.patch_size % 4 == 0 && j.patch_width % 4 == 0 && j.patch_ld % 4 == 0 && ((uintptr_t)j.patch_img & 15) == 0 &&
+            ((uintptr_t)j.patch_out & 15) == 0) {
+            a.patch_vec4 = 1;
+            a.n_patch = patch_ew_blocks((int64_t)j.patch_batch * (Np + 1) * (j.patch_ld / 4));
+        } else {
+            a.n_patch = patch_ew_blocks((int64_t)j.patch_batch * (Np + 1) * j.patch_ld);
+        }
+    }
+    a.n_pos = 0;
+    if (j.pos_pos != nullptr && j.pos_patches > 0) {
+        SPV_CHECK(j.pos_bias && j.pos_out && j.pos_embed > 0, "spv_step_prologue: bad position-row arguments");
+        a.n_pos = patch_ew_blocks((int64_t)(j.pos_patches + 1) * j.pos_embed);
+    }
+    const int64_t total = (int64_t)a.n_seed + a.n_shadow + a.n_fold + a.n_patch + a.n_pos;
+    if (total == 0) return 0;
+    SPV_CHECK(total < (1ll << 31), "spv_step_prologue: too many workgroups");
+    hipLaunchKernelGGL(step_prologue_kernel, dim3((unsigned)total), dim3(256), 0, static_cast<hipStream_t>(stream), a);
+    SPV_LAUNCH_CHECK("spv_step_prologue");
+    return 0;
+}
diff --git a/vit-spectre-experiments_amd/csrc/spv_patch.hip b/vit-spectre-experiments_amd/csrc/spv_patch.hip
--- a/vit-spectre-experiments_amd/csrc/spv_patch.hip
+++ b/vit-spectre-experiments_amd/csrc/spv_patch.hip
@@ -1,64 +1,22 @@
 #define SPV_USES_SEED
 #include "spv_common.h"
+#include "spv_prologue_core.h"
 
 namespace {
 
-__device__ __forceinline__ void st_any(void* base, size_t off, int bf, float v) {
-    if (bf) static_cast<bf16_t*>(base)[off] = f2bf(v);
-    else static_cast<float*>(base)[off] = v;
-}
 __device__ __forceinline__ float ld_any(const void* base, size_t off, int bf) {
     return bf ? bf2f(static_cast<const bf16_t*>(base)[off]) : static_cast<const float*>(base)[off];
 }
 
 __global__ __launch_bounds__(256) void patchify_kernel(const float* __restrict__ img, void* __restrict__ out, int B, int C, int H,
                                                        int W, int P, int ld, int transposed, int bf) {
-    const int nH = H / P, nW = W / P, Np = nH * nW, K = C * P * P;
-    const int64_t rows = (int64_t)B * Np;
-    const int64_t total = transposed == 1 ? (int64_t)K * ld : (transposed == 2 ? (int64_t)B * (Np + 1) * ld : rows * ld);
-    for (int64_t e = (int64_t)blockIdx.x * blockDim.x + threadIdx.x; e < total; e += (int64_t)gridDim.x * blockDim.x) {
-        int64_t row;
-        int k;
-        if (transposed == 1) { k = (int)(e / ld); row = e % ld; }
-        else { row = e / ld; k = (int)(e % ld); }
-        if (transposed == 2) {
-            const int64_t b2 = row / (Np + 1);
-            const int t2 = (int)(row % (Np + 1));
-            row = t2 == 0 ? rows : b2 * Np + t2 - 1;
-        }
-        float v = 0.0f;
-        if (row < rows && k < K) {
-            const int b = (int)(row / Np), n = (int)(row % Np);
-            const int ih = n / nW, iw = n % nW;
-            const int c = k / (P * P), p = (k / P) % P, q = k % P;
-            v = img[(((size_t)b * C + c) * H + ih * P + p) * W + iw * P + q];
-        }
-        st_any(out, (size_t)e, bf, v);
-    }
+    patchify_body(img, out, B, C, H, W, P, ld, transposed, bf, blockIdx.x, gridDim.x);
 }
 
 template <typename T>
 __global__ __launch_bounds__(256) void patchify_vec4_kernel(const float* __restrict__ img, T* __restrict__ out, int B, int C, int H, int W,
                                                             int P, int ld, int token_rows) {
-    const int nH = H / P, nW = W / P, Np = nH * nW, K = C * P * P;
-    const int T1 = token_rows ? Np + 1 : Np;
-    const int ld4 = ld >> 2, P4 = P >> 2;
-    const int64_t total = (int64_t)B * T1 * ld4;
-    for (int64_t e = (int64_t)blockIdx.x * blockDim.x + threadIdx.x; e < total; e += (int64_t)gridDim.x * blockDim.x) {
-        const int64_t row = e / ld4;
-        const int k = (int)(e - row * ld4) * 4;
-        const int b = (int)(row / T1), t = (int)(row - (int64_t)b * T1);
-        const int n = token_rows ? t - 1 : t;
-        float v[4] = {0.0f, 0.0f, 0.0f, 0.0f};
-        if (n >= 0 && k < K) {
-            const int ih = n / nW, iw = n - ih * nW;
-            const int c = k / (P * P), r = k - c * P * P, pr = r / P, q = r - pr * P;
-            const float4 px = *reinterpret_cast<const float4*>(img + (((size_t)b * C + c) * H + ih * P + pr) * W + iw * P + q);
-            v[0] = px.x; v[1] = px.y; v[2] = px.z; v[3] = px.w;
-        }
-        (void)P4;
-        io<T>::st4(out + (size_t)row * ld + k, v);
-    }
+    patchify_vec4_body<T>(img, out, B, C, H, W, P, ld, token_rows, blockIdx.x, gridDim.x);
 }
 
 __global__ __launch_bounds__(256) void patchify_u8_kernel(const unsigned char* __restrict__ img, const float* __restrict__ mean,
@@ -91,10 +49,7 @@
 
 __global__ __launch_bounds__(256) void posbias_kernel(const float* __restrict__ pos, const float* __restrict__ bias,
                                                       const float* __restrict__ cls, float* __restrict__ out, int Np, int E) {
-    const int lead = cls != nullptr ? E : 0;
-    const int total = Np * E + lead;
-    for (int i = blockIdx.x * blockDim.x + threadIdx.x; i < total; i += gridDim.x * blockDim.x)
-        out[i] = i < lead ? cls[i] + pos[i] : pos[E + i - lead] + bias[(i - lead) % E];
+    posbias_body(pos, bias, cls, out, Np, E, blockIdx.x, gridDim.x);
 }
 
 __global__ __launch_bounds__(256) void cls_rows_kernel(const float* __restrict__ cls, const float* __restrict__ pos,
@@ -137,24 +92,10 @@
                                      dropout_scale(dropout_row_key(live_seed(seed), (uint64_t)i >> 12), (unsigned)(i & 4095), p, inv_keep));
 }
 
-__device__ __forceinline__ float rcoef(int u, int v, int p, int q, int P) {
-    return cospif(2.0f * (float)((u * p + v * q) % P) / (float)P) / (float)P;
-}
-
 __global__ __launch_bounds__(256) void spectral_fold_kernel(const float* __restrict__ w, const float* __restrict__ fh,
                                                             const float* __restrict__ fw, float* __restrict__ wf, int E, int C, int P,
                                                             bf16_t* __restrict__ wf_bf = nullptr) {
-    const int Pv = P / 2 + 1;
-    const int total = E * C * P * P;
-    for (int i = blockIdx.x * blockDim.x + threadIdx.x; i < total; i += gridDim.x * blockDim.x) {
-        const int q = i % P, p = (i / P) % P, c = (i / (P * P)) % C, e = i / (P * P * C);
-        const float* wr = w + ((size_t)e * C + c) * P * Pv;
-        float a = 0.0f;
-        for (int u = 0; u < P; ++u)
-            for (int v = 0; v < Pv; ++v) a = fmaf(wr[u * Pv + v] * fh[u] * fw[v], rcoef(u, v, p, q, P), a);
-        wf[i] = a;
-        if (wf_bf != nullptr) wf_bf[i] = f2bf(a);
-    }
+    spectral_fold_body(w, fh, fw, wf, E, C, P, wf_bf, blockIdx.x, gridDim.x);
 }
 
 __global__ __launch_bounds__(256) void spectral_fold_bwd_kernel(const float* __restrict__ dwf, const float* __restrict__ w,
@@ -202,7 +143,7 @@
     }
 }
 
-inline int ew_blocks(int64_t n) { return (int)std::min<int64_t>((n + 255) / 256, 4096); }
+inline int ew_blocks(int64_t n) { return patch_ew_blocks(n); }
 
 }
 
diff --git a/vit-spectre-experiments_amd/csrc/spv_prologue_core.h b/vit-spectre-experiments_amd/csrc/spv_prologue_core.h
--- /dev/null
+++ b/vit-spectre-experiments_amd/csrc/spv_prologue_core.h
@@ -0,0 +1,135 @@
+#pragma once
+#include "spv_common.h"
+
+constexpr unsigned long long SEED_STEP = 0x9e3779b97f4a7c15ull;
+
+static __device__ __forceinline__ void st_any(void* base, size_t off, int bf, float v) {
+    if (bf) static_cast<bf16_t*>(base)[off] = f2bf(v);
+    else static_cast<float*>(base)[off] = v;
+}
+
+template <typename TO>
+static __device__ __forceinline__ void weight_shadow_tile(const float* __restrict__ src, TO* __restrict__ plain, TO* __restrict__ tr, int rows,
+                                                   int cols, int ld, int bx, int by, float (*tile)[65]) {
+    const int r0 = by * 32, c0 = bx * 64;
+    const int t = threadIdx.x;
+    const bool vec = (cols & 3) == 0;
+#pragma unroll
+    for (int pass = 0; pass < 2; ++pass) {
+        const int rl = pass * 16 + (t >> 4), c4 = (t & 15) * 4;
+        const int r = r0 + rl, c = c0 + c4;
+        float v[4] = {0.0f, 0.0f, 0.0f, 0.0f};
+        if (r < rows) {
+            if (vec && c + 3 < cols) {
+                const float4 f = *reinterpret_cast<const float4*>(src + (size_t)r * cols + c);
+                v[0] = f.x; v[1] = f.y; v[2] = f.z; v[3] = f.w;
+                if (plain != nullptr) io<TO>::st4(plain + (size_t)r * cols + c, v);
+            } else {
+                for (int u = 0; u < 4; ++u)
+                    if (c + u < cols) {
+                        v[u] = src[(size_t)r * cols + c + u];
+                        if (plain != nullptr) io<TO>::st(plain + (size_t)r * cols + c + u, v[u]);
+                    }
+            }
+        }
+#pragma unroll
+        for (int u = 0; u < 4; ++u) tile[rl][c4 + u] = v[u];
+    }
+    __syncthreads();
+    const int cl = t >> 2, r8 = (t & 3) * 8;
+    const int c = c0 + cl;
+    if (c < cols) {
+        TO* o = tr + (size_t)c * ld + r0 + r8;
+        if (r0 + r8 + 7 < ld && (ld & 7) == 0) {
+            float a[4], b[4];
+#pragma unroll
+            for (int u = 0; u < 4; ++u) { a[u] = tile[r8 + u][cl]; b[u] = tile[r8 + 4 + u][cl]; }
+            io<TO>::st4(o, a);
+            io<TO>::st4(o + 4, b);
+        } else {
+            for (int u = 0; u < 8; ++u)
+                if (r0 + r8 + u < ld) io<TO>::st(o + u, tile[r8 + u][cl]);
+        }
+    }
+}
+
+struct ShadowTensor { const float* src; void* plain; void* tr; int rows, cols, ld, pad; };
+
+static __device__ __forceinline__ void patchify_body(const float* __restrict__ img, void* __restrict__ out, int B, int C, int H, int W, int P,
+                                                     int ld, int transposed, int bf, int bid, int nb) {
+    const int nH = H / P, nW = W / P, Np = nH * nW, K = C * P * P;
+    const int64_t rows = (int64_t)B * Np;
+    const int64_t total = transposed == 1 ? (int64_t)K * ld : (transposed == 2 ? (int64_t)B * (Np + 1) * ld : rows * ld);
+    for (int64_t e = (int64_t)bid * blockDim.x + threadIdx.x; e < total; e += (int64_t)nb * blockDim.x) {
+        int64_t row;
+        int k;
+        if (transposed == 1) { k = (int)(e / ld); row = e % ld; }
+        else { row = e / ld; k = (int)(e % ld); }
+        if (transposed == 2) {
+            const int64_t b2 = row / (Np + 1);
+            const int t2 = (int)(row % (Np + 1));
+            row = t2 == 0 ? rows : b2 * Np + t2 - 1;
+        }
+        float v = 0.0f;
+        if (row < rows && k < K) {
+            const int b = (int)(row / Np), n = (int)(row % Np);
+            const int ih = n / nW, iw = n % nW;
+            const int c = k / (P * P), p = (k / P) % P, q = k % P;
+            v = img[(((size_t)b * C + c) * H + ih * P + p) * W + iw * P + q];
+        }
+        st_any(out, (size_t)e, bf, v);
+    }
+}
+
+template <typename T>
+static __device__ __forceinline__ void patchify_vec4_body(const float* __restrict__ img, T* __restrict__ out, int B, int C, int H, int W, int P,
+                                                          int ld, int token_rows, int bid, int nb) {
+    const int nH = H / P, nW = W / P, Np = nH * nW, K = C * P * P;
+    const int T1 = token_rows ? Np + 1 : Np;
+    const int ld4 = ld >> 2;
+    const int64_t total = (int64_t)B * T1 * ld4;
+    for (int64_t e = (int64_t)bid * blockDim.x + threadIdx.x; e < total; e += (int64_t)nb * blockDim.x) {
+        const int64_t row = e / ld4;
+        const int k = (int)(e - row * ld4) * 4;
+        const int b = (int)(row / T1), t = (int)(row - (int64_t)b * T1);
+        const int n = token_rows ? t - 1 : t;
+        float v[4] = {0.0f, 0.0f, 0.0f, 0.0f};
+        if (n >= 0 && k < K) {
+            const int ih = n / nW, iw = n - ih * nW;
+            const int c = k / (P * P), r = k - c * P * P, pr = r / P, q = r - pr * P;
+            const float4 px = *reinterpret_cast<const float4*>(img + (((size_t)b * C + c) * H + ih * P + pr) * W + iw * P + q);
+            v[0] = px.x; v[1] = px.y; v[2] = px.z; v[3] = px.w;
+        }
+        io<T>::st4(out + (size_t)row * ld + k, v);
+    }
+}
+
+static __device__ __forceinline__ void posbias_body(const float* __restrict__ pos, const float* __restrict__ bias, const float* __restrict__ cls,
+                                                    float* __restrict__ out, int Np, int E, int bid, int nb) {
+    const int lead = cls != nullptr ? E : 0;
+    const int total = Np * E + lead;
+    for (int i = bid * blockDim.x + threadIdx.x; i < total; i += nb * blockDim.x)
+        out[i] = i < lead ? cls[i] + pos[i] : pos[E + i - lead] + bias[(i - lead) % E];
+}
+
+static __device__ __forceinline__ float rcoef(int u, int v, int p, int q, int P) {
+    return cospif(2.0f * (float)((u * p + v * q) % P) / (float)P) / (float)P;
+}
+
+static __device__ __forceinline__ void spectral_fold_body(const float* __restrict__ w, const float* __restrict__ fh, const float* __restrict__ fw,
+                                                          float* __restrict__ wf, int E, int C, int P, bf16_t* __restrict__ wf_bf, int bid,
+                                                          int nb) {
+    const int Pv = P / 2 + 1;
+    const int total = E * C * P * P;
+    for (int i = bid * blockDim.x + threadIdx.x; i < total; i += nb * blockDim.x) {
+        const int q = i % P, p = (i / P) % P, c = (i / (P * P)) % C, e = i / (P * P * C);
+        const float* wr = w + ((size_t)e * C + c) * P * Pv;
+        float a = 0.0f;
+        for (int u = 0; u < P; ++u)
+            for (int v = 0; v < Pv; ++v) a = fmaf(wr[u * Pv + v] * fh[u] * fw[v], rcoef(u, v, p, q, P), a);
+        wf[i] = a;
+        if (wf_bf != nullptr) wf_bf[i] = f2bf(a);
+    }
+}
+
+inline int patch_ew_blocks(int64_t n) { return (int)std::min<int64_t>((n + 255) / 256, 4096); }
diff --git a/vit-spectre-experiments_amd/spectre_vit/_native.py b/vit-spectre-experiments_amd/spectre_vit/_native.py
--- a/vit-spectre-experiments_amd/spectre_vit/_native.py
+++ b/vit-spectre-experiments_amd/spectre_vit/_native.py
@@ -57,6 +57,8 @@
     "spv_small_sl_partial_floats": [c_i, c_i],
     "spv_small_sl_fwd": [c_vp, c_i64, c_vp, c_i64, c_vp, c_vp, c_vp, c_vp, c_vp, c_vp, c_vp, c_vp, c_vp, c_i, c_i, c_i, c_i, c_vp],
     "spv_small_sl_bwd": [c_vp] * 15 + [c_i, c_i, c_i, c_i, c_vp],
+    "spv_small_sl_bwd_rows": [c_vp] * 10 + [c_i, c_i, c_i, c_i, c_vp],
+    "spv_small_sl_bwd_w": [c_vp] * 7 + [c_i, c_i, c_i, c_vp],
     "spv_cross_entropy_workspace_floats": [],
     "spv_cross_entropy_fwd": [c_vp, c_vp, c_vp, c_vp, c_vp, c_i, c_i, c_vp],
     "spv_cross_entropy_bwd": [c_vp, c_vp, c_vp, c_vp, c_vp, c_i, c_i, c_vp],
@@ -92,6 +94,7 @@
     "spv_colsum": [c_vp, c_vp, c_vp, c_i, c_i, c_i, c_vp],
     "spv_set_seed_device_ptr": [c_vp],
     "spv_seed_advance": [c_vp, c_vp],
+    "spv_step_prologue": [c_vp, c_vp],
     "spv_adamw_multi": [c_vp, c_vp, c_vp, c_vp, c_i, c_f, c_f, c_f, c_f, c_f, c_f, c_f, c_f, c_f, c_vp, c_vp],
     "spv_adamw_multi_ema": [c_vp, c_vp, c_vp, c_vp, c_i, c_f, c_f, c_f, c_f, c_f, c_f, c_f, c_f, c_f, c_vp, c_vp, c_f, c_i, c_f, c_vp],
     "spv_grad_sumsq": [c_vp, c_vp, c_vp, c_vp, c_i, c_vp, c_vp],
@@ -147,6 +150,15 @@
                                    "ratio_hi")]
 
 
+class PrologueJobs(ctypes.Structure):
+    _fields_ = ([("seed_word", c_vp), ("shadow_table", c_vp), ("tile_tensor", c_vp), ("tile_x", c_vp), ("tile_y", c_vp), ("ntiles", c_i),
+                 ("shadow_dtype", c_i), ("fold_w", c_vp), ("fold_fh", c_vp), ("fold_fw", c_vp), ("fold_out", c_vp), ("fold_out_bf16", c_vp)]
+                + [(n, c_i) for n in ("fold_embed", "fold_chans", "fold_patch", "pad0")]
+                + [("patch_img", c_vp), ("patch_out", c_vp)]
+                + [(n, c_i) for n in ("patch_batch", "patch_chans", "patch_height", "patch_width", "patch_size", "patch_ld", "patch_dtype", "pad1")]
+                + [("pos_pos", c_vp), ("pos_bias", c_vp), ("pos_cls", c_vp), ("pos_out", c_vp), ("pos_patches", c_i), ("pos_embed", c_i)])
+
+
 class TnProblem(ctypes.Structure):
     _fields_ = [("a", c_vp), ("b", c_vp), ("c", c_vp), ("m", c_i), ("n", c_i), ("lda", c_i), ("ldb", c_i), ("ldc", c_i), ("k", c_i)]
 
diff --git a/vit-spectre-experiments_amd/spectre_vit/graph.py b/vit-spectre-experiments_amd/spectre_vit/graph.py
--- a/vit-spectre-experiments_amd/spectre_vit/graph.py
+++ b/vit-spectre-experiments_amd/spectre_vit/graph.py
@@ -63,7 +63,7 @@
             raise
 
     def _forward_backward(self):
-        _native.call("spv_seed_advance", self.seed_word.data_ptr(), torch.cuda.current_stream().cuda_stream)
+        hip_ops.step_prologue(self.model, self.img, self.seed_word, self.autocast_dtype)
         self.reducer.zero_grad()
         with torch.autocast("cuda", dtype=self.autocast_dtype, enabled=self.autocast_dtype is not None):
             out = self.model(self.img)
diff --git a/vit-spectre-experiments_amd/spectre_vit/hip_ops.py b/vit-spectre-experiments_amd/spectre_vit/hip_ops.py
--- a/vit-spectre-experiments_amd/spectre_vit/hip_ops.py
+++ b/vit-spectre-experiments_amd/spectre_vit/hip_ops.py
@@ -9,7 +9,7 @@
 
 import torch
 
-from . import _native, shadows
+from . import _native, prologue, shadows
 from ._launch import _DT, BF16, F32, _dt, _p, _require_gpu, _stream
 from .shadows import invalidate_weight_shadows
 from .timing import KernelTimer, _timing, set_kernel_timer
@@ -103,6 +103,8 @@
 WGRAD_BATCH = 8
 BATCH_FOLDS = 16
 _WGRAD_HOLD = True
+HEAD_WGRAD_HOLD = True
+_held_head = []
 FOLD_RIDE = True
 
 
@@ -133,6 +135,9 @@
 _T = torch.Tensor
 _Fold = NamedTuple("_Fold", [("partials", _T), ("outs", tuple), ("parts", int), ("n", int)])
 _HeldWgrad = NamedTuple("_HeldWgrad", [("dh", _T), ("x", _T), ("dw", int), ("rows", int), ("n", int), ("k", int), ("fold", object)])
+
+
+_HeldHead = NamedTuple("_HeldHead", [("dh", _T), ("xs", _T), ("partials", _T), ("outs", tuple), ("rows", int), ("n", int), ("k", int)])
 
 
 def _addrs(tensors):
@@ -219,6 +224,7 @@
     if _held_task != task:
         _held_folds.clear()
         _held_wgrads.clear()
+        _held_head.clear()
         _engine.queue_callback(flush_held_folds)
         _held_task = task
 
@@ -234,6 +240,27 @@
     return True
 
 
+def _hold_head_wgrad(dh, xs, partials, outs, sinks, rows, n, k):
+    if not (HEAD_WGRAD_HOLD and _hold_ok() and _sunk(outs, sinks)):
+        return False
+    task = _graph_task_id()
+    if task < 0:
+        return False
+    _begin_pass(task)
+    _held_head.append(_HeldHead(dh, xs, partials, _addrs(outs), rows, n, k))
+    return True
+
+
+def flush_held_head(end_of_pass=False):
+    if not _held_head:
+        return
+    if end_of_pass or _held_task == _graph_task_id():
+        for h in _held_head:
+            _native.call("spv_small_sl_bwd_w", _p(h.dh), _p(h.xs), _p(h.partials), *h.outs, h.rows, h.n, h.k, _stream())
+            PATH_COUNTS["head_wgrad_held"] += 1
+    _held_head.clear()
+
+
 def _in_sink(dw, sink):
     if sink is None:
         return False
@@ -244,6 +271,7 @@
 def flush_held_folds():
     global _held_task
     _flush_held_wgrads()
+    flush_held_head(True)
     if _held_folds:
         arr = _fold_array(_held_folds)
         _native.call("spv_fold_multi", ctypes.addressof(arr), len(_held_folds), _stream())
@@ -619,6 +647,13 @@
     def forward(ctx, proj_w, fh, fw, chans, patch):
         _require_gpu(proj_w)
         E = proj_w.shape[0]
+        ready = prologue.take("fold", (proj_w, fh, fw), (chans, patch)) if torch.is_autocast_enabled("cuda") else None
+        if ready is not None:
+            wf, wf._spv_bf16 = ready
+            ctx.save_for_backward(proj_w, fh, fw)
+            ctx.sinks = (_sink(proj_w), _sink(fh), _sink(fw))
+            ctx.meta = (E, chans, patch)
+            return wf
         wf = torch.empty((E, chans * patch * patch), dtype=torch.float32, device=proj_w.device)
         if torch.is_autocast_enabled("cuda"):
             wb = torch.empty(wf.shape, dtype=torch.bfloat16, device=proj_w.device)
@@ -671,16 +706,22 @@
         img = img.contiguous() if u8 else img.contiguous().float()
         _check_channels("patch embedding", E, K, dtype)
         st = _stream()
-        patches = torch.empty((B * T, K), dtype=dtype, device=dev)
-        if u8:
+        patches = None if u8 else prologue.take("patchify", (img,), (patch, dtype))
+        if patches is not None:
+            pass
+        elif u8:
+            patches = torch.empty((B * T, K), dtype=dtype, device=dev)
             _native.call("spv_patchify_u8", _p(img), _p(norm[0]), _p(norm[1]), _p(patches), B, C, H, W, patch, K, 2, _DT[dtype], st)
         else:
+            patches = torch.empty((B * T, K), dtype=dtype, device=dev)
             _native.call("spv_patchify", _p(img), _p(patches), B, C, H, W, patch, K, 2, _DT[dtype], st)
         wc = w_full if dtype == torch.float32 else (getattr(w_full, "_spv_bf16", None) if dtype == torch.bfloat16 else None)
         if wc is None:
             wc = _raw_cast(w_full, dtype)
-        posbias = torch.empty((T, E), dtype=torch.float32, device=dev)
-        _native.call("spv_embed_posbias", _p(pos), _p(bias), _p(cls), _p(posbias), Np, E, st)
+        posbias = prologue.take("posbias", (pos, bias, cls), (Np, E))
+        if posbias is None:
+            posbias = torch.empty((T, E), dtype=torch.float32, device=dev)
+            _native.call("spv_embed_posbias", _p(pos), _p(bias), _p(cls), _p(posbias), Np, E, st)
         tokens = torch.empty((B, T, E), dtype=dtype, device=dev)
         seed = _new_seed() if p_drop > 0.0 else 0
         _native.call("spv_gemm_nt_grouped_rows_drop", _p(patches), _p(wc), 0, _p(posbias), _p(tokens), B * T, E, K, K, K, E,
@@ -715,6 +756,7 @@
             dtok = masked
         if patches is not None and dtok.dtype == torch.bfloat16:
             dwf = _weight_grad(dtok.view(B * T, E), patches, B * T, E, K)
+            flush_held_head()
             if not early:
                 join_side_stream()
             return None, dwf, dbias, dcls, dpos_full, None, None, None, None
@@ -901,6 +943,64 @@
     def backward(ctx, g):
         shape, dtype = ctx.meta
         return _cls_row_gradient(shape, dtype, g.device, g), g
+
+
+STEP_PROLOGUE = True
+
+
+def step_prologue(model, img, seed_word, autocast_dtype):
+    prologue.clear()
+    if not STEP_PROLOGUE:
+        _native.call("spv_seed_advance", _p(seed_word), _stream())
+        return
+    jobs = _native.PrologueJobs()
+    jobs.seed_word = _p(seed_word)
+    work = 16.0
+    deposits = []
+    emb = getattr(model, "embeddings_block", None)
+    if autocast_dtype == torch.bfloat16 and torch.is_grad_enabled() and img.is_cuda:
+        weights_fn = getattr(model, "_shadow_weights", None)
+        weights = weights_fn() if callable(weights_fn) else None
+        ss = shadows.shadow_set(model, weights) if weights else None
+        if ss is not None and ss.dtype == torch.bfloat16:
+            table, tt, tx, ty, ntiles = ss._tables
+            jobs.shadow_table, jobs.tile_tensor, jobs.tile_x, jobs.tile_y = _p(table), _p(tt), _p(tx), _p(ty)
+            jobs.ntiles, jobs.shadow_dtype = ntiles, BF16
+            work += 2048.0 * ntiles * 8
+            deposits.append(("shadows", weights, (ss.dtype,), ss))
+        sources_fn = getattr(emb, "_prologue_sources", None)
+        sources = sources_fn(img) if callable(sources_fn) and img.dtype == torch.float32 and img.is_contiguous() else None
+        if sources is not None:
+            (w, fh, fw, C, P), (bias, cls, pos) = sources
+            B, _, H, W = img.shape
+            dev = img.device
+            E, K = w.shape[0], C * P * P
+            Np = (H // P) * (W // P)
+            fp32 = all(t.dtype == torch.float32 and t.is_contiguous() and t.is_cuda for t in (w, fh, fw, pos, bias, cls))
+            if fp32 and P > 0 and H >= P and W >= P and w.dim() == 2 and w.shape[1] == C * P * (P // 2 + 1) and pos.numel() == (Np + 1) * E:
+                wf = torch.empty((E, K), dtype=torch.float32, device=dev)
+                wb = torch.empty((E, K), dtype=torch.bfloat16, device=dev)
+                jobs.fold_w, jobs.fold_fh, jobs.fold_fw, jobs.fold_out, jobs.fold_out_bf16 = _p(w), _p(fh), _p(fw), _p(wf), _p(wb)
+                jobs.fold_embed, jobs.fold_chans, jobs.fold_patch = E, C, P
+                work += 4.0 * w.numel() + 6.0 * E * K
+                deposits.append(("fold", (w, fh, fw), (C, P), (wf, wb)))
+                patches = torch.empty((B * (Np + 1), K), dtype=torch.bfloat16, device=dev)
+                jobs.patch_img, jobs.patch_out = _p(img), _p(patches)
+                jobs.patch_batch, jobs.patch_chans, jobs.patch_height, jobs.patch_width = B, C, H, W
+                jobs.patch_size, jobs.patch_ld, jobs.patch_dtype = P, K, BF16
+                work += 4.0 * img.numel() + 2.0 * patches.numel()
+                deposits.append(("patchify", (img,), (P, torch.bfloat16), patches))
+                posbias = torch.empty((Np + 1, E), dtype=torch.float32, device=dev)
+                jobs.pos_pos, jobs.pos_bias, jobs.pos_cls, jobs.pos_out = _p(pos), _p(bias), _p(cls), _p(posbias)
+                jobs.pos_patches, jobs.pos_embed = Np, E
+                work += 8.0 * (Np + 1) * E
+                deposits.append(("posbias", (pos, bias, cls), (Np, E), posbias))
+    if _timing():
+        _native.hint = int(work)
+    _native.call("spv_step_prologue", ctypes.addressof(jobs), _stream())
+    PATH_COUNTS["step_prologue"] += 1
+    for role, sources, extra, value in deposits:
+        prologue.deposit(role, sources, extra, value)
 
 
 def small_head_ok(rows: int, n: int, k: int) -> bool:
@@ -951,8 +1051,10 @@
         dgamma = _grad_buf(s_g, (n,), dev)
         dbeta = _grad_buf(s_be, (n,), dev)
         partials = torch.empty((_native.call("spv_small_sl_partial_floats", B, n),), dtype=torch.float32, device=dev)
-        _native.call("spv_small_sl_bwd", _p(dlogits), _p(h), _p(xs), _p(mean), _p(rstd), _p(weight), _p(gamma), _p(beta), _p(dh), _p(dx),
-                     _p(dw), _p(dgamma), _p(dbeta), _p(dbias), _p(partials), B, n, E, _DT[dtype], _stream())
+        _native.call("spv_small_sl_bwd_rows", _p(dlogits), _p(h), _p(mean), _p(rstd), _p(weight), _p(gamma), _p(beta), _p(dh), _p(dx),
+                     _p(partials), B, n, E, _DT[dtype], _stream())
+        if not _hold_head_wgrad(dh, xs, partials, (dw, dgamma, dbeta, dbias), (s_w, s_g, s_be, s_b), B, n, E):
+            _native.call("spv_small_sl_bwd_w", _p(dh), _p(xs), _p(partials), _p(dw), _p(dgamma), _p(dbeta), _p(dbias), B, n, E, _stream())
         if dfeats is not None:
             dx = dx + dfeats.to(dx.dtype)
         return _cls_row_gradient(shape, dtype, dev, dx), dx, dw, dbias, dgamma, dbeta
diff --git a/vit-spectre-experiments_amd/spectre_vit/models/spectre/spectre.py b/vit-spectre-experiments_amd/spectre_vit/models/spectre/spectre.py
--- a/vit-spectre-experiments_amd/spectre_vit/models/spectre/spectre.py
+++ b/vit-spectre-experiments_amd/spectre_vit/models/spectre/spectre.py
@@ -162,6 +162,12 @@
         w_full = hip_ops.SpectralFoldFn.apply(self.proj.weight, self.freq_weight_h, self.freq_weight_w, C, self.P)
         return hip_ops.patch_embed(x, w_full, self.proj.bias, self.cls_token, self.position_embeddings, self.P, self.pixel_norm,
                                    self.dropout.p if self.training else 0.0)
+
+    def _prologue_sources(self, x):
+        if x.dtype == torch.uint8 or x.dim() != 4:
+            return None
+        return ((self.proj.weight, self.freq_weight_h, self.freq_weight_w, x.shape[1], self.P),
+                (self.proj.bias, self.cls_token, self.position_embeddings))
 
 
 class SpectreViT(nn.Module):
diff --git a/vit-spectre-experiments_amd/spectre_vit/prologue.py b/vit-spectre-experiments_amd/spectre_vit/prologue.py
--- /dev/null
+++ b/vit-spectre-experiments_amd/spectre_vit/prologue.py
@@ -0,0 +1,25 @@
+from __future__ import annotations
+
+_entries = {}
+
+
+def ident(*tensors):
+    return tuple((int(t.data_ptr()), tuple(t.shape), t.dtype) for t in tensors)
+
+
+def clear():
+    _entries.clear()
+
+
+def deposit(role, sources, extra, value):
+    _entries[(role, ident(*sources), tuple(extra))] = value
+
+
+def take(role, sources, extra=()):
+    if not _entries:
+        return None
+    return _entries.pop((role, ident(*sources), tuple(extra)), None)
+
+
+def pending():
+    return sorted(k[0] for k in _entries)
diff --git a/vit-spectre-experiments_amd/spectre_vit/shadows.py b/vit-spectre-experiments_amd/spectre_vit/shadows.py
--- a/vit-spectre-experiments_amd/spectre_vit/shadows.py
+++ b/vit-spectre-experiments_amd/spectre_vit/shadows.py
@@ -5,7 +5,7 @@
 
 import torch
 
-from . import _native
+from . import _native, prologue
 from ._launch import _DT, _p, _stream
 
 
@@ -91,6 +91,9 @@
 
     def refresh(self):
         _refresh_multi(self._tables, self.dtype)
+        self.mark_fresh()
+
+    def mark_fresh(self):
         for wr, (wc, wt) in zip(self.weights, self.bufs):
             w = wr()
             if w is not None:
@@ -137,18 +140,28 @@
         _pinned = prev
 
 
+def shadow_set(module, weights):
+    ss = getattr(module, "_spv_shadow_set", None)
+    key = tuple((w.data_ptr(), tuple(w.shape)) for w in weights)
+    if ss is None or ss.key != key:
+        if torch.cuda.is_current_stream_capturing():
+            return None
+        ss = ShadowSet(weights)
+        object.__setattr__(module, "_spv_shadow_set", ss)
+    return ss
+
+
 def refresh_weight_shadows(module, weights_fn):
     weights = weights_fn()
     if not weights:
         return
-    ss = getattr(module, "_spv_shadow_set", None)
-    key = tuple((w.data_ptr(), tuple(w.shape)) for w in weights)
-    if ss is None or ss.key != key:
-        if torch.cuda.is_current_stream_capturing():
-            return
-        ss = ShadowSet(weights)
-        object.__setattr__(module, "_spv_shadow_set", ss)
-    ss.refresh()
+    ss = shadow_set(module, weights)
+    if ss is None:
+        return
+    if prologue.take("shadows", weights, (ss.dtype,)) is ss:
+        ss.mark_fresh()
+    else:
+        ss.refresh()
 
 
 def invalidate_weight_shadows(*_args, **_kwargs):
diff --git a/vit-spectre-experiments_amd/spectre_vit/timing.py b/vit-spectre-experiments_amd/spectre_vit/timing.py
--- a/vit-spectre-experiments_amd/spectre_vit/timing.py
+++ b/vit-spectre-experiments_amd/spectre_vit/timing.py
@@ -16,6 +16,8 @@
 _WORK_MODELS = {
     "spv_small_sl_fwd": lambda i: ("head_fwd", i[2:5], i[5], "mfma", 2.0 * i[2] * i[3] * i[4]),
     "spv_small_sl_bwd": lambda i: ("head_bwd", i[0:3], i[3], "mfma", 4.0 * i[0] * i[1] * i[2]),
+    "spv_small_sl_bwd_rows": lambda i: ("head_bwd_rows", i[0:3], i[3], "mfma", 2.0 * i[0] * i[1] * i[2]),
+    "spv_small_sl_bwd_w": lambda i: ("head_bwd_w", i[0:3], F32, "mfma", 2.0 * i[0] * i[1] * i[2]),
     "spv_cross_entropy_fwd": lambda i: ("cross_entropy_fwd", i[0:2], F32, "hbm", i[0] * i[1] * 4.0),
     "spv_cross_entropy_bwd": lambda i: ("cross_entropy_bwd", i[0:2], F32, "hbm", i[0] * i[1] * 8.0),
     "spv_distill_loss_fwd": lambda i: ("distill_loss_fwd", i[0:2], F32, "hbm", i[0] * i[1] * 8.0),
@@ -66,6 +68,7 @@
     "spv_grad_sumsq": lambda i: ("grad_sumsq", i[0:1], F32, "hbm", 4.0 * 2048 * i[0]),
     "spv_step_control": lambda i: ("step_control", i[0:2], F32, "hbm", 8.0 * i[0] + 64),
     "spv_adamw_multi_ctl": lambda i: ("adamw_multi_ctl", i[0:1], F32, "hbm", 7.0 * 4 * 2048 * i[0]),
+    "spv_step_prologue": lambda i: ("step_prologue", (), BF16, "hbm", float(i[-1])),
     "spv_weight_shadows": lambda i: ("weight_shadows", i[0:2], i[3], "hbm", i[0] * i[1] * (4.0 + 2 * _es(i[3]))),
     "spv_dropout": lambda i: ("dropout", i[0:1], i[1], "hbm", 2.0 * i[0] * _es(i[1])),
     "spv_axpby": lambda i: ("axpby", i[0:1], i[1], "hbm", 3.0 * i[0] * _es(i[1])),
```
